# ThomasZiegler/RS-aware-differential-SfM

Measured on AMD Instinct MI355X. Metric: Mpixels/sec RS depth+pose solve, 1280x720 pair, higher is better.
Workload: dtype f64

## Files before the change

### include/rsdsfm.h

```cpp
#ifndef RSDSFM_H
#define RSDSFM_H

#include <stddef.h>
#include <stdint.h>

#ifdef __cplusplus
extern "C" {
#endif

#define RSDSFM_OK 0
#define RSDSFM_ERR_INVALID (-1)
#define RSDSFM_ERR_HIP (-2)
#define RSDSFM_ERR_NO_DEVICE (-3)
#define RSDSFM_ERR_NUMERIC (-4)
#define RSDSFM_ERR_PENDING (-5)
#define RSDSFM_ERR_PEER (-6)

#define RSDSFM_DEPTH_CLOSED_FORM 0
#define RSDSFM_DEPTH_CERES_LM 1

#define RSDSFM_K_COMPAT 0
#define RSDSFM_K_FIXED 1

#define RSDSFM_FLOW_COMPAT_RANK 0
// ... 111 lines not shown
int rsdsfm_flatten_dev(rsdsfm_ctx* ctx, const double* d_flow_img, int32_t rows, int32_t cols, double fx, double fy,
                       double cx, double cy, double gamma, double flow_threshold, double* d_q2n, double* d_u2n,
                       double* d_alpha_n, double* d_alpha_k_n, int64_t* n_out);
int rsdsfm_depth_map_dev(rsdsfm_ctx* ctx, double* d_inliers_3m_inout, int64_t m, double v_inout[3], double fx, double fy,
                         double cx, double cy, int32_t rows, int32_t cols, double* d_depth_map_colmajor,
                         int32_t* d_xs_or_null, int32_t* d_ys_or_null, int* flipped);
int rsdsfm_pose_table_dev(rsdsfm_ctx* ctx, const double v[3], const double w[3], double k, double gamma, int32_t rows,
                          double* d_R_rows9, double* d_t_rows3);
typedef struct rsdsfm_frame_params {
    int32_t ransac_trials;
    int32_t use_acceleration_mode;
    int32_t use_refinement;
    int32_t depth_mode;
    int32_t k_sign_mode;
    int32_t flow_index_mode;
    int32_t use_global_shutter_mode;
    int32_t struct_bytes;
    double ransac_tol;
    double flow_threshold;
    uint64_t seed;
} rsdsfm_frame_params;

void rsdsfm_frame_params_init(rsdsfm_frame_params* params);

typedef struct rsdsfm_frame_result {
    int64_t n_points, num_inliers;
    int32_t best_trial, flipped;
    double ransac_w[3], ransac_v[3], ransac_k;
    double w[3], v[3], k;
    rsdsfm_lm_summary refine_summary;
    const double* d_inliers;
    const int64_t* d_inlier_idx;
    const int32_t* d_scanline;
} rsdsfm_frame_result;

int rsdsfm_solve_frame_dev(rsdsfm_ctx* ctx, const double* d_flow_img, int32_t rows, int32_t cols, double fx, double fy,
                           double cx, double cy, double gamma, const rsdsfm_frame_params* params,
                           double* d_depth_map_colmajor, double* d_R_rows9_or_null, double* d_t_rows3_or_null,
                           rsdsfm_frame_result* result);
typedef struct rsdsfm_frame_job {
    const double* d_flow_img;
    int32_t rows, cols;
    double fx, fy, cx, cy, gamma;
    double* d_depth_map_colmajor;
    double* d_R_rows9_or_null;
    double* d_t_rows3_or_null;
    uint64_t seed;
} rsdsfm_frame_job;
int rsdsfm_solve_frames_dev(rsdsfm_ctx* ctx, const rsdsfm_frame_job* jobs, int32_t count, const rsdsfm_frame_params* params,
                            rsdsfm_frame_result* results);
int rsdsfm_set_sequence_lanes(rsdsfm_ctx* ctx, int32_t lanes);
int rsdsfm_set_frame_side_flatten(rsdsfm_ctx* ctx, int mode);
int rsdsfm_set_frame_tail(rsdsfm_ctx* ctx, int mode);
int rsdsfm_ransac_dev(rsdsfm_ctx* ctx, const double* d_q2n, const double* d_u2n, const double* d_alpha_n,
                      const double* d_alpha_k_n, int64_t n, int use_alpha_k, int32_t iterations, double tolerance,
                      const int32_t* samples_9xT_or_null, uint64_t seed, int depth_mode, int k_sign_mode,
                      rsdsfm_ransac_out* out);
int rsdsfm_refine_dev(rsdsfm_ctx* ctx, const double* d_flow2n, int64_t n_flow, int64_t m, const double* d_inliers_3m,
                      const double* d_alpha_m, const double* d_alpha_k_m, const int64_t* d_inlier_idx_or_null,
                      const double v_in[3], const double w_in[3], double k_in, int const_acceleration,
                      int flow_index_mode, double* d_inliers_out_3m, double v_out[3], double w_out[3], double* k_out,
                      rsdsfm_lm_summary* summary_or_null);
int rsdsfm_estimate_inverse_depths_batch_dev(rsdsfm_ctx* const* ctxs, int32_t count, const double* const* d_q2n,
                                             const double* const* d_u2n, const int64_t* n, const double* v_count_x3,
                                             const double* w_count_x3, const double* k_count, const double* const* d_alpha_n,
                                             const double* const* d_alpha_k_n, double* const* d_inv_depth_n);
int rsdsfm_depth_lm_batch_launch_dev(rsdsfm_ctx* const* ctxs, int32_t count, const double* const* d_q2n, const double* const* d_u2n,
                                     const int64_t* n, const double* v_count_x3, const double* w_count_x3, const double* k_count,
                                     const double* const* d_alpha_n, const double* const* d_alpha_k_n, double* const* d_inv_depth_n);
int rsdsfm_depth_lm_launch_dev(rsdsfm_ctx* ctx, const double* d_q2n, const double* d_u2n, int64_t n,
                               const double v[3], const double w[3], double k, const double* d_alpha_n,
                               const double* d_alpha_k_n, double* d_inv_depth_n, int launch_id);
int rsdsfm_depth_lm_sums_row_size(void);
int rsdsfm_depth_lm_reduce_dev(rsdsfm_ctx* ctx, int64_t n_shard, double* d_row_out);
int rsdsfm_depth_lm_decide_rows_dev(rsdsfm_ctx* ctx, const double* d_rows, int32_t nrows, int64_t n_total, int launch_id);
int rsdsfm_depth_lm_state(rsdsfm_ctx* ctx, int32_t* status, int32_t* next_launch, rsdsfm_lm_summary* summary_or_null);
int rsdsfm_depth_finish_dev(rsdsfm_ctx* ctx, const double* d_q2n, const double* d_u2n, int64_t n,
                            const double v[3], const double w[3], double k, const double* d_alpha_n,
                            const double* d_alpha_k_n, double* d_inv_depth_n, rsdsfm_lm_summary* summary_or_null,
                            int32_t* extra_launches);

int rsdsfm_flatten_slab_dev(rsdsfm_ctx* ctx, const double* d_img_slab, int32_t rows, int32_t slab_cols, int32_t col0,
                            double fx, double fy, double cx, double cy, double gamma, double thr, double* d_q2n,
                            double* d_u2n, double* d_alpha_n, double* d_alpha_k_n, int64_t* n_out);
int rsdsfm_sample_indices(int64_t n, int32_t iterations, uint64_t seed, int32_t* samples);
int rsdsfm_minimal9_dev(rsdsfm_ctx* ctx, const double* d_q9, const double* d_u9, const double* d_alpha9,
                        const double* d_alpha_k9, int32_t count, int use_alpha_k, int k_sign_mode, double* d_hyp);
int rsdsfm_minimal9_probe_dev(rsdsfm_ctx* ctx, const double* d_q9, const double* d_u9, const double* d_alpha9, const double* d_alpha_k9,
                              int32_t count, int use_alpha_k, int k_sign_mode, int use_cores, double* d_hyp, double* d_probe4);
size_t rsdsfm_tile_lm_state_bytes(void);
size_t rsdsfm_tile_best_bytes(void);
int32_t rsdsfm_tile_ransac_row_size(void);
int32_t rsdsfm_tile_ransac_batch(void);
int rsdsfm_tile_ransac_lm_rows_dev(rsdsfm_ctx* ctx, const double* d_q2n, const double* d_u2n, const double* d_alpha_n,
                                   const double* d_alpha_k_n, int64_t n_shard, const double* d_hyp, int32_t count,
                                   const void* d_states, int32_t round, double tolerance, double* d_rows);
int rsdsfm_tile_ransac_decide_dev(rsdsfm_ctx* ctx, const double* d_rows_all, int32_t nranks, int32_t count, void* d_states,
                                  int64_t n_total, int32_t round, int32_t* d_flags, int32_t* d_scored, double* d_trial_count,
                                  double* d_trial_err);
int rsdsfm_tile_ransac_score_rows_dev(rsdsfm_ctx* ctx, const double* d_q2n, const double* d_u2n, const double* d_alpha_n,
                                      const double* d_alpha_k_n, int64_t n_shard, const double* d_hyp, int32_t count,
                                      const void* d_states, int depth_mode, double tolerance, const int32_t* d_scored_or_null,
                                      double* d_rows);
int rsdsfm_tile_ransac_score_merge_dev(rsdsfm_ctx* ctx, const double* d_rows_all, int32_t nranks, int32_t count,
                                       const int32_t* d_scored_or_null, double* d_trial_count, double* d_trial_err);
int rsdsfm_tile_ransac_pick_dev(rsdsfm_ctx* ctx, const double* d_trial_count, const double* d_trial_err, int32_t iterations,
// ... 105 lines not shown
```

### rs-aware-differential-sfm_amd/__init__.py

```python
import ctypes as C
import os
import sys

import numpy as np

from . import dist, pipeline, synth

_HERE = os.path.dirname(os.path.abspath(__file__))
LIB_PATH = os.environ.get("RSDSFM_LIB") or os.path.join(_HERE, "librsdsfm_hip.so")
LIB_PATH_FUSED = os.path.join(_HERE, "librsdsfm_hip_fused.so")
HEADER_PATH = os.path.join(os.path.dirname(_HERE), "include", "rsdsfm.h")

OK = 0
ERR_PENDING = -5
DEPTH_CLOSED_FORM, DEPTH_CERES_LM = 0, 1
K_COMPAT, K_FIXED = 0, 1
FLOW_COMPAT_RANK, FLOW_GATHERED = 0, 1
REFINE_TRACE_COLS = 8
TRACE_REJECTED, TRACE_ACCEPTED, TRACE_INVALID, TRACE_PARAMETER_TOL, TRACE_FUNCTION_TOL, TRACE_ACCEPTED_GRADIENT_TOL = 0.0, 1.0, 2.0, 3.0, 4.0, 5.0
TERMINATION = {0: "gradient", 1: "parameter", 2: "function", 3: "max_iter", 4: "failure", 5: "min_radius"}

_libs = {}


# ... 442 lines not shown
                          int(flow_index_mode), int(use_global_shutter_mode), 0, float(tol), float(flow_threshold), int(seed))
        res, info = FrameResult(), TiledInfo()
        d = C.c_double
        self._check(self.lib.rsdsfm_solve_frame_tiled_dev(self._ctx, _dp(d_img_slab) if d_img_slab else None, C.c_int32(rows), C.c_int32(cols), d(K[0]), d(K[1]),
                                                          d(K[2]), d(K[3]), d(gamma), C.byref(prm), _dp(d_depth_map), _dp(d_R) if d_R else None,
                                                          _dp(d_t) if d_t else None, C.byref(res), C.byref(info)), "rsdsfm_solve_frame_tiled_dev")
        return dict(n=int(res.n_points), num_inliers=int(res.num_inliers), best_trial=int(res.best_trial), flipped=bool(res.flipped),
                    ransac_w=np.array(res.ransac_w[:]), ransac_v=np.array(res.ransac_v[:]), ransac_k=float(res.ransac_k),
                    w=np.array(res.w[:]), v=np.array(res.v[:]), k=float(res.k), refine_summary=res.refine_summary.as_dict(),
                    d_inliers=res.d_inliers, d_inlier_idx=res.d_inlier_idx, d_scanline=res.d_scanline, flow_index_mode=int(flow_index_mode),
                    info={k2: int(getattr(info, k2)) for k2, _ in TiledInfo._fields_ if k2 != "_pad"})

    def estimate_inverse_depths_tiled_dev(self, d_q_shard, d_u_shard, n_total, v, w, k, d_alpha_shard, d_alpha_k_shard, d_inv_depth,
                                          mode=DEPTH_CERES_LM):
        sm, info = LmSummary(), TiledInfo()
        opt = lambda p_: _dp(p_) if p_ else None
        self._check(self.lib.rsdsfm_estimate_inverse_depths_tiled_dev(self._ctx, opt(d_q_shard), opt(d_u_shard), C.c_int64(n_total), _v3(v), _v3(w),
                                                                      C.c_double(k), opt(d_alpha_shard), opt(d_alpha_k_shard), C.c_int(int(mode)),
                                                                      opt(d_inv_depth), C.byref(sm), C.byref(info)),
                    "rsdsfm_estimate_inverse_depths_tiled_dev")
        return (sm.as_dict() if int(mode) == DEPTH_CERES_LM else None,
                {k2: int(getattr(info, k2)) for k2, _ in TiledInfo._fields_ if k2 != "_pad"})

    def prepared_frame_solve(self, d_flow_img, rows, cols, K, gamma, d_depth_map, d_R=None, d_t=None, trials=50, tol=0.05,
                             use_acceleration_mode=False, use_refinement=True, depth_mode=DEPTH_CERES_LM, k_sign_mode=K_COMPAT,
                             flow_threshold=1e-10, flow_index_mode=FLOW_COMPAT_RANK, use_global_shutter_mode=False):
        prm = FrameParams(int(trials), int(use_acceleration_mode), int(use_refinement), int(depth_mode), int(k_sign_mode),
                          int(flow_index_mode), int(use_global_shutter_mode), 0, float(tol), float(flow_threshold), 0)
        res = FrameResult()
        d = C.c_double
        fn = self.lib.rsdsfm_solve_frame_dev
        args = (self._ctx, _dp(d_flow_img), C.c_int32(rows), C.c_int32(cols), d(K[0]), d(K[1]), d(K[2]), d(K[3]), d(gamma), C.byref(prm),
                _dp(d_depth_map), _dp(d_R) if d_R else None, _dp(d_t) if d_t else None, C.byref(res))
        check = self._check

        def call(seed):
            prm.seed = seed
            rc = fn(*args)
            if rc != OK:
                check(rc, "rsdsfm_solve_frame_dev")
            return res

        return call

    def set_sequence_lanes(self, lanes):
        self._check(self.lib.rsdsfm_set_sequence_lanes(self._ctx, C.c_int32(int(lanes))), "rsdsfm_set_sequence_lanes")

    def set_frame_side_flatten(self, on):
        self._check(self.lib.rsdsfm_set_frame_side_flatten(self._ctx, int(on)), "rsdsfm_set_frame_side_flatten")

    def set_frame_tail(self, mode):
        self._check(self.lib.rsdsfm_set_frame_tail(self._ctx, int(mode)), "rsdsfm_set_frame_tail")

    def prepared_frames_solve(self, jobs, trials=50, tol=0.05, use_acceleration_mode=False, use_refinement=True, depth_mode=DEPTH_CERES_LM,
                              k_sign_mode=K_COMPAT, flow_threshold=1e-10, flow_index_mode=FLOW_COMPAT_RANK, use_global_shutter_mode=False):
        n = len(jobs)
        arr = (FrameJob * n)()
        for a, j in zip(arr, jobs):
            K = j["K"]
            a.d_flow_img, a.rows, a.cols = int(j["d_flow_img"]), int(j["rows"]), int(j["cols"])
            a.fx, a.fy, a.cx, a.cy, a.gamma = float(K[0]), float(K[1]), float(K[2]), float(K[3]), float(j["gamma"])
            a.d_depth_map, a.d_R, a.d_t = int(j["d_depth_map"]), int(j.get("d_R") or 0) or None, int(j.get("d_t") or 0) or None
        prm = FrameParams(int(trials), int(use_acceleration_mode), int(use_refinement), int(depth_mode), int(k_sign_mode),
                          int(flow_index_mode), int(use_global_shutter_mode), 0, float(tol), float(flow_threshold), 0)
        res = (FrameResult * n)()
        fn, ctx, check = self.lib.rsdsfm_solve_frames_dev, self._ctx, self._check

        def call(seeds):
            for a, sd in zip(arr, seeds):
                a.seed = int(sd)
            rc = fn(ctx, arr, C.c_int32(n), C.byref(prm), res)
            if rc != OK:
                check(rc, "rsdsfm_solve_frames_dev")
            return res

        return call

    def solve_frames_dev(self, jobs, seeds, **kw):
        res = self.prepared_frames_solve(jobs, **kw)(seeds)
        return [dict(n=int(r.n_points), num_inliers=int(r.num_inliers), best_trial=int(r.best_trial), flipped=bool(r.flipped),
                     ransac_w=np.array(r.ransac_w[:]), ransac_v=np.array(r.ransac_v[:]), ransac_k=float(r.ransac_k),
                     w=np.array(r.w[:]), v=np.array(r.v[:]), k=float(r.k), refine_summary=r.refine_summary.as_dict(),
                     d_inliers=r.d_inliers, d_inlier_idx=r.d_inlier_idx, d_scanline=r.d_scanline) for r in res]

    def depth_lm_reduce_dev(self, n_shard, d_row):
        self._check(self.lib.rsdsfm_depth_lm_reduce_dev(self._ctx, C.c_int64(n_shard), _dp(d_row)), "rsdsfm_depth_lm_reduce_dev")

    def depth_lm_decide_rows_dev(self, d_rows, nrows, n_total, launch_id):
        self._check(self.lib.rsdsfm_depth_lm_decide_rows_dev(self._ctx, _dp(d_rows), C.c_int32(nrows), C.c_int64(n_total), int(launch_id)), "rsdsfm_depth_lm_decide_rows_dev")

    def depth_lm_state(self):
        status, nxt, sm = C.c_int32(), C.c_int32(), LmSummary()
        self._check(self.lib.rsdsfm_depth_lm_state(self._ctx, C.byref(status), C.byref(nxt), C.byref(sm)), "rsdsfm_depth_lm_state")
        return status.value, nxt.value, sm.as_dict()

    def depth_finish_dev(self, d_q, d_u, n, v, w, k, d_alpha, d_alpha_k, d_rho):
        sm = LmSummary()
        extra = C.c_int32()
        self._check(self.lib.rsdsfm_depth_finish_dev(self._ctx, _dp(d_q), _dp(d_u), C.c_int64(n), _v3(v), _v3(w), C.c_double(k), _dp(d_alpha), _dp(d_alpha_k), _dp(d_rho), C.byref(sm), C.byref(extra)), "rsdsfm_depth_finish_dev")
        return sm.as_dict(), extra.value


def _np0(ptr):
    return _dp(ptr) if ptr else None


# ... 386 lines not shown
```

### rs-aware-differential-sfm_amd/build.py

```python
import concurrent.futures
import glob
import os
import subprocess

HERE = os.path.dirname(os.path.abspath(__file__))
SO = os.path.join(HERE, "librsdsfm_hip.so")
SO_FUSED = os.path.join(HERE, "librsdsfm_hip_fused.so")
OBJ_DIR = os.path.join(HERE, "build")
CFLAGS = ["--offload-arch=gfx950", "-O3", "-std=c++17", "-ffp-contract=off", "-fPIC", "-Wall", "-Wno-unused-function"]
LDFLAGS = ["--offload-arch=gfx950", "-shared", "-fPIC", "-ldl"]
FUSED_UNITS = ("depth_kernels", "ransac_kernels", "ransac_lma_kernels", "depth_lma_kernels", "gtflow_kernels", "capi")


def sources():
    return sorted(glob.glob(os.path.join(HERE, "csrc", "*.hip")))


def _deps():
    return glob.glob(os.path.join(HERE, "csrc", "*.hpp")) + [os.path.join(HERE, "..", "include", "rsdsfm.h")]


def _stale(target, deps):
    return not os.path.exists(target) or os.path.getmtime(target) < max(os.path.getmtime(d) for d in deps)


def needs_build():
    return _stale(SO, sources() + _deps()) or _stale(SO_FUSED, sources() + _deps())


def _compile(job):
    src, obj, extra, verbose = job
    hipcc = os.environ.get("HIPCC", "/opt/rocm/bin/hipcc")
    cmd = [hipcc] + CFLAGS + extra + ["-c", src, "-o", obj]
    if verbose:
        print(" ".join(cmd), flush=True)
    subprocess.check_call(cmd)
    return obj


def build(force=False, verbose=False, jobs=None):
    if not force and not needs_build():
        return SO
    os.makedirs(OBJ_DIR, exist_ok=True)
    hdrs = _deps()
    todo, objs, objs_fused = [], [], []
    for src in sources():
        stem = os.path.splitext(os.path.basename(src))[0]
        obj = os.path.join(OBJ_DIR, stem + ".o")
        objs.append(obj)
        if force or _stale(obj, [src] + hdrs):
            todo.append((src, obj, [], verbose))
        if stem in FUSED_UNITS:
            objf = os.path.join(OBJ_DIR, stem + ".fused.o")
            objs_fused.append(objf)
            if force or _stale(objf, [src] + hdrs):
                todo.append((src, objf, ["-DRSDSFM_FUSED=1"], verbose))
        else:
            objs_fused.append(obj)
    jobs = jobs or max(1, min(len(todo), (os.cpu_count() or 4)))
    if todo:
        with concurrent.futures.ThreadPoolExecutor(max_workers=jobs) as ex:
            list(ex.map(_compile, todo))
    hipcc = os.environ.get("HIPCC", "/opt/rocm/bin/hipcc")
    for so, oo in ((SO, objs), (SO_FUSED, objs_fused)):
# ... 14 lines not shown
```

### rs-aware-differential-sfm_amd/csrc/frame_host.hip

```cpp
#include <stdlib.h>
#include <string.h>

#include <atomic>

#include <algorithm>
#include <new>

#include "rsdsfm_internal.hpp"

namespace rsdsfm {

static std::atomic<int> g_frames_in_flight[64];
int frames_in_flight(const Ctx* c) { return g_frames_in_flight[c->device & 63].load(std::memory_order_relaxed); }

int alpha_ones_launch(Ctx* c, double* d_alpha, int64_t n);
int flatten_device(Ctx* c, const double* d_img, int32_t rows, int32_t cols, int32_t col0, double fx, double fy, double cx, double cy, double gamma,
                   double thr, double* d_q, double* d_u, double* d_alpha, double* d_alpha_k, int64_t* n_out);

struct FrameRun {
    rsdsfm_frame_job job;
    rsdsfm_frame_params prm;
    size_t N = 0;
    int64_t n = 0;
    double *d_q = nullptr, *d_u = nullptr, *d_a = nullptr, *d_ak = nullptr, *d_in_a = nullptr, *d_in_ak = nullptr, *d_inl = nullptr, *d_inl_ref = nullptr;
    int64_t* d_idx = nullptr;
    uint8_t* d_mask = nullptr;
    int32_t* d_ys = nullptr;
    double *d_zpartials = nullptr, *d_zheader = nullptr;
    char* d_refine_ws = nullptr;
    rsdsfm_ransac_out ro;
    RansacRun ransac;
    RefineRun refine;
    Minimal9Direct direct;
    DenseFlatten dense;
    bool refinement_enqueued = false, ahead = false, side_flatten = false, dense_in_launch = false, open = false;
    bool counted = false;
    int rc_begin = RSDSFM_OK;
    int64_t m_known = -1;
    RefineTail tail;
    FinishClaim claim;
    RansacSpecTail spec_tail;
    std::function<int()> join;
};

namespace {

inline double* header_host(Ctx* c) { return reinterpret_cast<double*>(static_cast<char*>(c->h_pinned) + c->pinned_bytes - 64); }
inline RefineState* state_host(Ctx* c) { return reinterpret_cast<RefineState*>(static_cast<char*>(c->h_pinned) + c->pinned_bytes - kPinnedTail); }
inline int64_t* count_host(Ctx* c) { return reinterpret_cast<int64_t*>(static_cast<char*>(c->h_pinned) + c->pinned_bytes - kPinnedTail / 2); }
static_assert(sizeof(RefineState) + sizeof(int) <= kPinnedTail / 2, "reserved tail: state read-back | point count ... depth-map header");

struct StreamSwap {
    Ctx* c;
    hipStream_t main;
    StreamSwap(Ctx* ctx, hipStream_t other) : c(ctx), main(ctx->stream) { c->stream = other; }
    ~StreamSwap() { c->stream = main; }
};

int ensure_side_stream(Ctx* c) {
    if (c->aux_stream) return RSDSFM_OK;
    RSDSFM_HIP_CHECK(c, hipStreamCreateWithFlags(&c->aux_stream, hipStreamNonBlocking));
    RSDSFM_HIP_CHECK(c, hipEventCreateWithFlags(&c->ev_fork, hipEventDisableTiming));
    RSDSFM_HIP_CHECK(c, hipEventCreateWithFlags(&c->ev_join, hipEventDisableTiming));
    return RSDSFM_OK;
}

static void frame_uncount(const Ctx* c, FrameRun* F) {
    if (F && F->counted) {
        F->counted = false;
        g_frames_in_flight[c->device & 63].fetch_sub(1, std::memory_order_relaxed);
    }
}
struct FrameInFlightEnd {
    const Ctx* c;
    FrameRun* F;
    ~FrameInFlightEnd() { frame_uncount(c, F); }
};

int frame_begin(Ctx* c, FrameRun* F) {
    const rsdsfm_frame_job& J = F->job;
    const rsdsfm_frame_params* prm = &F->prm;
    frame_uncount(c, F);
    F->open = false;
    F->rc_begin = RSDSFM_OK;
    if (J.rows <= 0 || J.cols <= 0 || !J.d_flow_img || !J.d_depth_map_colmajor) return fail(c, RSDSFM_ERR_INVALID, "bad arguments");
    if (prm->flow_index_mode != RSDSFM_FLOW_COMPAT_RANK && prm->flow_index_mode != RSDSFM_FLOW_GATHERED) return fail(c, RSDSFM_ERR_INVALID, "unknown flow_index_mode");
    if (prm->struct_bytes != 0 && prm->struct_bytes != (int32_t)sizeof(rsdsfm_frame_params))
        return fail(c, RSDSFM_ERR_INVALID, "rsdsfm_frame_params: struct_bytes is neither 0 nor sizeof(rsdsfm_frame_params) -- caller built against another header (use rsdsfm_frame_params_init)");
// ... 74 lines not shown
                StreamSwap on_side(c, c->aux_stream);
                rc = flatten_launch(c, J.d_flow_img, rows, cols, 0, fx, fy, cx, cy, gamma, prm->flow_threshold, F->d_q, F->d_u, F->d_a, F->d_ak,
                                    d_flat_counts, d_flat_offsets, count_host(c), nullptr);
                if (rc == RSDSFM_OK && prm->use_global_shutter_mode) rc = alpha_ones_launch(c, F->d_a, n);
            }
            if (rc != RSDSFM_OK) return rc;
            RSDSFM_HIP_CHECK(c, hipEventRecord(c->ev_join, c->aux_stream));
            F->join = [c]() -> int {
                RSDSFM_HIP_CHECK(c, hipStreamWaitEvent(c->stream, c->ev_join, 0));
                return RSDSFM_OK;
            };
        } else {
            rc = flatten_enqueue(c, J.d_flow_img, rows, cols, fx, fy, cx, cy, gamma, prm->flow_threshold, F->d_q, F->d_u, F->d_a, F->d_ak, count_host(c));
            if (rc != RSDSFM_OK) return rc;
        }
    } else {
        rc = flatten_device(c, J.d_flow_img, rows, cols, 0, fx, fy, cx, cy, gamma, prm->flow_threshold, F->d_q, F->d_u, F->d_a, F->d_ak, &n);
        if (rc != RSDSFM_OK) return rc;
        *count_host(c) = n;
    }
    if (prm->use_global_shutter_mode && !F->side_flatten) {
        rc = alpha_ones_launch(c, F->d_a, n);
        if (rc != RSDSFM_OK) return rc;
    }
    F->n = n;
    memset(&F->ro, 0, sizeof(F->ro));
    F->ro.inlier_idx = F->d_idx;
    F->ro.inliers = F->d_inl;
    F->ro.alpha = F->d_in_a;
    F->ro.alpha_k = F->d_in_ak;
    F->ro.mask = F->d_mask;
    F->m_known = -1;
    F->tail = [c, F](const RefineBuffers& B) -> int {
        const rsdsfm_frame_job& J2 = F->job;
        const RefineState* st = B.state;
        const int64_t m_arg = F->m_known >= 0 ? F->m_known : F->n;
        const int64_t* m_dev = F->m_known >= 0 ? nullptr : &st->m;
        PoseTableOut pt;
        if (J2.d_R_rows9_or_null && J2.d_t_rows3_or_null)
            pt.R = J2.d_R_rows9_or_null, pt.t = J2.d_t_rows3_or_null, pt.rows = J2.rows, pt.gamma = J2.gamma, pt.wk_dev = st->p + 3;
        if (B.claim.on)
            return depth_map_decided_launch(c, F->d_inl_ref, m_arg, F->d_zpartials, refine_finish_grid(c, B), B, J2.d_depth_map_colmajor, F->d_zheader,
                                            header_host(c), st->p, m_dev, &pt);
        return depth_map_slab_launch(c, F->d_inl_ref, m_arg, F->d_zpartials, refine_finish_grid(c, B), m_arg, nullptr, J2.fx, J2.fy, J2.cx, J2.cy, J2.rows,
                                     0, J2.cols, J2.d_depth_map_colmajor, nullptr, F->d_ys, F->d_zheader, header_host(c), st->p, m_dev, &pt);
    };
    F->claim = FinishClaim();
    if (c->frame_tail == 0) {
        F->claim.on = true;
        F->claim.fx = J.fx, F->claim.fy = J.fy, F->claim.cx = J.cx, F->claim.cy = J.cy;
        F->claim.rows = rows, F->claim.cols = cols;
        F->claim.ys = F->d_ys;
    }
    F->spec_tail = [c, F](const RansacBest* d_best) -> int {
        return refine_begin(c, F->d_u, F->n, F->n, F->d_inl, F->d_in_a, F->d_in_ak, F->d_idx, nullptr, nullptr, 0.0, F->prm.use_acceleration_mode,
                            F->prm.flow_index_mode, F->d_inl_ref, &F->tail, d_best, F->d_refine_ws, &F->refine, state_host(c), F->d_zpartials, false,
                            &F->claim);
    };
    F->refinement_enqueued = false;
    F->ahead = prm->use_refinement && c->ransac_spec_miss < 2;
    F->open = true;
    g_frames_in_flight[c->device & 63].fetch_add(1, std::memory_order_relaxed);
    F->counted = true;
    F->rc_begin = ransac_begin(c, F->d_q, F->d_u, F->d_a, F->d_ak, n, prm->use_acceleration_mode, prm->ransac_trials, prm->ransac_tol, nullptr, J.seed,
                               prm->depth_mode, prm->k_sign_mode, &F->ro, prm->use_refinement ? &F->spec_tail : nullptr, &F->refinement_enqueued, &F->ransac,
                               F->side_flatten ? &F->direct : nullptr, F->side_flatten && !F->dense_in_launch ? &F->join : nullptr,
                               F->dense_in_launch ? &F->dense : nullptr, F->ahead, true,
                               F->claim.on && prm->use_refinement ? refine_flag_words(F->d_refine_ws) : nullptr);
    return RSDSFM_OK;
}

int frame_finish(Ctx* c, FrameRun* F, rsdsfm_frame_result* res) {
    if (!F->open) return fail(c, RSDSFM_ERR_INVALID, "no frame solve in flight");
    F->open = false;
    FrameInFlightEnd in_flight_end_{c, F};
    const rsdsfm_frame_job& J = F->job;
    const rsdsfm_frame_params* prm = &F->prm;
    memset(res, 0, sizeof(*res));
    int rc = F->rc_begin;
    if (rc == RSDSFM_OK) rc = ransac_finish(c, &F->ransac);
    if (rc != RSDSFM_OK) RSDSFM_HIP_CHECK(c, hipStreamSynchronize(c->stream));
    if (F->side_flatten && c->aux_stream) RSDSFM_HIP_CHECK(c, hipStreamSynchronize(c->aux_stream));
    int64_t n = F->n;
    if (*count_host(c) < 0) {
        c->frame_dense_hint = 1;
        return rc != RSDSFM_OK ? rc : fail(c, RSDSFM_ERR_NUMERIC, "frame solve: the point count did not arrive");
    }
    bool counted = true;
    if (*count_host(c) != n) {
        if (F->dense_in_launch) {
            int64_t n_real = 0;
            rc = flatten_device(c, J.d_flow_img, J.rows, J.cols, 0, J.fx, J.fy, J.cx, J.cy, J.gamma, prm->flow_threshold, F->d_q, F->d_u, F->d_a, F->d_ak, &n_real);
            if (rc == RSDSFM_OK && prm->use_global_shutter_mode) rc = alpha_ones_launch(c, F->d_a, n_real);
            if (rc != RSDSFM_OK) return rc;
            *count_host(c) = n_real;
        }
        n = *count_host(c);
        F->n = n;
        F->refinement_enqueued = false;
        counted = false;
        rc = ransac_begin(c, F->d_q, F->d_u, F->d_a, F->d_ak, n, prm->use_acceleration_mode, prm->ransac_trials, prm->ransac_tol, nullptr, J.seed,
                          prm->depth_mode, prm->k_sign_mode, &F->ro, prm->use_refinement ? &F->spec_tail : nullptr, &F->refinement_enqueued, &F->ransac, nullptr, nullptr,
                          nullptr, F->ahead, true,
                               F->claim.on && prm->use_refinement ? refine_flag_words(F->d_refine_ws) : nullptr);
        if (rc == RSDSFM_OK) rc = ransac_finish(c, &F->ransac);
        counted = rc == RSDSFM_OK;
    }
    c->frame_dense_hint = n == (int64_t)F->N ? 1 : 0;
    if (rc != RSDSFM_OK) return rc;
    if (counted) ransac_commit_hints(c, F->ransac);
    const rsdsfm_ransac_out& ro = F->ro;
    res->n_points = n;
    res->num_inliers = ro.num_inliers;
    res->best_trial = ro.best_trial;
    memcpy(res->ransac_w, ro.w, sizeof(ro.w));
    memcpy(res->ransac_v, ro.v, sizeof(ro.v));
    res->ransac_k = ro.k;
    double v[3], w[3], k = ro.k;
    for (int i = 0; i < 3; ++i) v[i] = ro.v[i], w[i] = ro.w[i];
    double* d_final = F->d_inl;
    int flipped = 0;
    F->m_known = ro.num_inliers;
    if (prm->use_refinement) {
        bool exact = false;
        if (F->refinement_enqueued) {
            rc = refine_poll(c, &F->refine, v, w, &k, &res->refine_summary);
            exact = rc == kRcRefineRestartExact;
        }
        if (!F->refinement_enqueued || exact)
            rc = refine_device(c, F->d_u, n, ro.num_inliers, F->d_inl, F->d_in_a, F->d_in_ak, F->d_idx, v, w, k, prm->use_acceleration_mode,
                               prm->flow_index_mode, F->d_inl_ref, v, w, &k, &res->refine_summary, &F->tail, F->d_zpartials, exact, &F->claim);
        if (rc != RSDSFM_OK) return rc;
        d_final = F->d_inl_ref;
        const double* h_header = header_host(c);
        flipped = h_header[0] != 0.0;
        v[0] = h_header[1], v[1] = h_header[2], v[2] = h_header[3];
    } else {
        rc = depth_map_device(c, d_final, ro.num_inliers, v, J.fx, J.fy, J.cx, J.cy, J.rows, J.cols, J.d_depth_map_colmajor, nullptr, F->d_ys, &flipped, w,
                              k, J.gamma, J.d_R_rows9_or_null, J.d_t_rows3_or_null);
        if (rc != RSDSFM_OK) return rc;
    }
    res->flipped = flipped;
    memcpy(res->v, v, sizeof(v));
    memcpy(res->w, w, sizeof(w));
    res->k = k;
    res->d_inliers = d_final;
    res->d_inlier_idx = F->d_idx;
    res->d_scanline = F->d_ys;
    return RSDSFM_OK;
}

FrameRun* frame_run_of(Ctx* c) {
    if (!c->frame_run) c->frame_run = new (std::nothrow) FrameRun();
    return static_cast<FrameRun*>(c->frame_run);
}

}

void frame_release(Ctx* c) {
    frame_uncount(c, static_cast<FrameRun*>(c->frame_run));
    delete static_cast<FrameRun*>(c->frame_run);
    c->frame_run = nullptr;
    for (rsdsfm_ctx* lane : c->lanes) rsdsfm_destroy(lane);
    c->lanes.clear();
    if (c->ev_fork) (void)hipEventDestroy(c->ev_fork);
    if (c->ev_join) (void)hipEventDestroy(c->ev_join);
    if (c->ev_seq) (void)hipEventDestroy(c->ev_seq);
    if (c->aux_stream) (void)hipStreamDestroy(c->aux_stream);
    if (c->d_flat_counters) (void)hipFree(c->d_flat_counters);
    c->d_flat_counters = nullptr;
    c->ev_fork = c->ev_join = c->ev_seq = nullptr;
    c->aux_stream = nullptr;
}

}

using namespace rsdsfm;

extern "C" {

void rsdsfm_frame_params_init(rsdsfm_frame_params* p) {
    if (!p) return;
    memset(p, 0, sizeof(*p));
    p->ransac_trials = 5;
    p->use_acceleration_mode = 0;
    p->use_refinement = 1;
    p->depth_mode = RSDSFM_DEPTH_CERES_LM;
    p->k_sign_mode = RSDSFM_K_COMPAT;
    p->flow_index_mode = RSDSFM_FLOW_COMPAT_RANK;
    p->use_global_shutter_mode = 0;
    p->struct_bytes = (int32_t)sizeof(rsdsfm_frame_params);
    p->ransac_tol = 0.05;
    p->flow_threshold = 1e-10;
    p->seed = 1;
}

int rsdsfm_solve_frame_dev(rsdsfm_ctx* ctx, const double* d_flow_img, int32_t rows, int32_t cols, double fx, double fy, double cx,
                           double cy, double gamma, const rsdsfm_frame_params* prm, double* d_depth_map, double* d_R_rows9,
                           double* d_t_rows3, rsdsfm_frame_result* res) {
    if (!ctx) return RSDSFM_ERR_INVALID;
    Ctx* c = &ctx->c;
    DeviceGuard device_guard_(c);
    if (!prm || !res) return fail(c, RSDSFM_ERR_INVALID, "bad arguments");
    FrameRun* F = frame_run_of(c);
    if (!F) return fail(c, RSDSFM_ERR_INVALID, "out of host memory");
    F->prm = *prm;
    F->job = rsdsfm_frame_job{d_flow_img, rows, cols, fx, fy, cx, cy, gamma, d_depth_map, d_R_rows9, d_t_rows3, prm->seed};
    int rc = frame_begin(c, F);
    if (rc != RSDSFM_OK) return rc;
    return frame_finish(c, F, res);
}

int rsdsfm_set_sequence_lanes(rsdsfm_ctx* ctx, int32_t lanes) {
    if (!ctx) return RSDSFM_ERR_INVALID;
    Ctx* c = &ctx->c;
    DeviceGuard device_guard_(c);
    if (lanes < 0 || lanes > 16) return fail(c, RSDSFM_ERR_INVALID, "lanes must be 0 (default) .. 16");
    c->seq_lanes = lanes;
    return RSDSFM_OK;
}

int rsdsfm_set_frame_tail(rsdsfm_ctx* ctx, int mode) {
    if (!ctx) return RSDSFM_ERR_INVALID;
    if (mode < 0 || mode > 1) return fail(&ctx->c, RSDSFM_ERR_INVALID, "mode must be 0 (short launch tail) or 1 (stage-by-stage launches)");
    ctx->c.frame_tail = mode;
    return RSDSFM_OK;
}

int rsdsfm_set_frame_side_flatten(rsdsfm_ctx* ctx, int mode) {
    if (!ctx) return RSDSFM_ERR_INVALID;
    if (mode < 0 || mode > 3) return fail(&ctx->c, RSDSFM_ERR_INVALID, "mode must be 0 (flatten first), 1 (flatten on a second stream), 2 (flatten behind the minimal solver) or 3 (flatten inside the solver's launch)");
    ctx->c.frame_side_flatten = mode;
    return RSDSFM_OK;
}

int rsdsfm_solve_frames_dev(rsdsfm_ctx* ctx, const rsdsfm_frame_job* jobs, int32_t count, const rsdsfm_frame_params* prm, rsdsfm_frame_result* results) {
    if (!ctx) return RSDSFM_ERR_INVALID;
    Ctx* c = &ctx->c;
    DeviceGuard device_guard_(c);
    if (count < 0 || !prm || (count > 0 && (!jobs || !results))) return fail(c, RSDSFM_ERR_INVALID, "bad arguments");
    if (count == 0) return RSDSFM_OK;
    const int L = std::max(1, std::min<int>(count, c->seq_lanes > 0 ? c->seq_lanes : kSequenceLanesDefault));
    while ((int)c->lanes.size() < L - 1) {
        rsdsfm_ctx* lane = nullptr;
        int rc = rsdsfm_create(&lane, c->device, nullptr);
        if (rc != RSDSFM_OK) return fail(c, rc, "could not create a sequence lane");
        c->lanes.push_back(lane);
    }
    auto lane_ctx = [&](int l) -> Ctx* { return l == 0 ? c : &c->lanes[(size_t)l - 1]->c; };
    if (L > 1) {
        if (!c->ev_seq) RSDSFM_HIP_CHECK(c, hipEventCreateWithFlags(&c->ev_seq, hipEventDisableTiming));
        RSDSFM_HIP_CHECK(c, hipEventRecord(c->ev_seq, c->stream));
    }
    for (int l = 1; l < L; ++l) {
        Ctx* lc = lane_ctx(l);
        RSDSFM_HIP_CHECK(c, hipStreamWaitEvent(lc->stream, c->ev_seq, 0));
        lc->ransac_k0 = c->ransac_k0;
        lc->ransac_math_mode = c->ransac_math_mode;
        lc->lm_arithmetic = c->lm_arithmetic;
        lc->refine_arithmetic = c->refine_arithmetic;
        lc->lma_count_only_force = c->lma_count_only_force;
        lc->frame_side_flatten = c->frame_side_flatten;
        lc->frame_tail = c->frame_tail;
        lc->refine_stage_mode = c->refine_stage_mode;
    }
    for (int l = 0; l < L; ++l) lane_ctx(l)->refine_stage_separate = L > 1;
    int first_error = RSDSFM_OK;
    int in_flight[16];
    for (int l = 0; l < 16; ++l) in_flight[l] = -1;
    auto finish_lane = [&](int l) {
        const int i = in_flight[l];
        if (i < 0) return;
        in_flight[l] = -1;
        Ctx* lc = lane_ctx(l);
        int rc = frame_finish(lc, static_cast<FrameRun*>(lc->frame_run), &results[i]);
        if (rc != RSDSFM_OK && first_error == RSDSFM_OK) {
            first_error = rc;
            if (lc != c) c->err = "pair " + std::to_string(i) + ": " + lc->err;
        }
    };
    for (int i = 0; i < count && first_error == RSDSFM_OK; ++i) {
        const int l = i % L;
        finish_lane(l);
        if (first_error != RSDSFM_OK) break;
        Ctx* lc = lane_ctx(l);
        FrameRun* F = frame_run_of(lc);
        if (!F) {
            first_error = fail(c, RSDSFM_ERR_INVALID, "out of host memory");
            break;
        }
        F->prm = *prm;
        F->job = jobs[i];
        int rc = frame_begin(lc, F);
        if (rc != RSDSFM_OK) {
            first_error = rc;
            if (lc != c) c->err = "pair " + std::to_string(i) + ": " + lc->err;
            break;
        }
        in_flight[l] = i;
    }
    for (;;) {
        int best = -1;
        for (int l = 0; l < L; ++l)
            if (in_flight[l] >= 0 && (best < 0 || in_flight[l] < in_flight[best])) best = l;
        if (best < 0) break;
        finish_lane(best);
    }
    for (int l = 0; l < L; ++l) lane_ctx(l)->refine_stage_separate = false;
    return first_error;
}

int rsdsfm_set_refine_stage(rsdsfm_ctx* ctx, int mode) {
    if (!ctx) return RSDSFM_ERR_INVALID;
    Ctx* c = &ctx->c;
    if (mode < 0 || mode > 2) return fail(c, RSDSFM_ERR_INVALID, "refine stage: 0 (automatic), 1 (in the next pass's prologue) or 2 (a launch of its own)");
    c->refine_stage_mode = mode;
// ... 5 lines not shown
```

### rs-aware-differential-sfm_amd/csrc/lm_common.hpp

```cpp
#pragma once

#include "device_math.hpp"
#include "rsdsfm_internal.hpp"

namespace rsdsfm {

__device__ __forceinline__ double closed_form_rho(double x, double y, double ux, double uy, double al, double ak,
                                                  const Pose& pose, double two_over) {
    PixelModel m;
    m.init(x, y, ux, uy, al, ak, pose, two_over);
    double r0, r1;
    m.residual(1.0, r0, r1);
    double h = m.J0 * m.J0 + m.J1 * m.J1;
    double g = m.J0 * r0 + m.J1 * r1;
    return (h > 0.0) ? 1.0 - g / h : 1.0;
}


__device__ __forceinline__ void lm_advance(LmScal& st, double* hist, const double* sums, int64_t n, int first, int used_K,
                                           int used_write, int launch_id) {
    if (first) {
        st.status = 0;
        st.restart = 0;
        st.n_hist = 0;
// ... 61 lines not shown
        if (rel > kMinRelDecrease) {
            hist[st.n_hist] = st.radius;
            st.n_hist += 1;
            accepted_in_batch = j + 1;
            cost = ccost;
            x_norm = sqrt(s[3]);
            st.radius = radius_accept(st.radius, rel);
            st.decrease_factor = 2.0;
            st.num_successful += 1;
            if (s[4] <= kGradientTol) {
                st.termination = RSDSFM_TERM_GRADIENT;
                break;
            }
        } else {
            st.num_unsuccessful += 1;
            st.radius = st.radius / st.decrease_factor;
            st.decrease_factor *= 2.0;
            break;
        }
    }
    st.cost = cost;
    if (used_write <= accepted_in_batch) st.rho_holds = base_hist + used_write;
    else st.rho_holds = -1;
    if (st.termination < 0 && st.iteration >= kMaxIter) st.termination = RSDSFM_TERM_MAX_ITER;
    if (st.termination < 0 && st.radius <= kMinRadius) st.termination = RSDSFM_TERM_MIN_RADIUS;
    st.next_launch = launch_id + 1;
    if (st.termination >= 0) {
        st.predict = st.n_hist < KMAX ? st.n_hist : KMAX;
        if (st.rho_holds == st.n_hist) {
            st.status = 1;
        } else {
            st.status = 2;
            st.K = 0;
            st.write_which = 0;
        }
    } else {
        st.status = 0;
        st.K = KMAX;
        st.write_which = 0;
        double r = st.radius;
#pragma unroll
        for (int j = 0; j < KMAX; ++j) {
            st.cand[j] = r;
            r = radius_accept(r, 1.0);
        }
    }
}

struct LmPlanLds {
    int n_hist, K, write_which;
    double inv_hist[kMaxIter];
    double inv_cand[KMAX];
    __device__ __forceinline__ double inv_hist_at(int h) const { return inv_hist[h]; }
};

struct LmPlanReg {
    int n_hist, K, write_which;
    double inv_cand[KMAX];
    double h0, h1, h2, h3;
    const double* hist_lds;
    __device__ __forceinline__ double inv_hist_at(int h) const {
        return h == 0 ? h0 : (h == 1 ? h1 : (h == 2 ? h2 : (h == 3 ? h3 : hist_lds[h])));
    }
};

template <int K0>
struct LmPlanFirstK {
    static constexpr int n_hist = 0;
    static constexpr int K = K0;
    int write_which;
    double inv_cand[KMAX];
    __device__ __forceinline__ double inv_hist_at(int) const { return 0.0; }
    __device__ __forceinline__ void load(const LmPlanLds& l) {
        write_which = l.write_which;
#pragma unroll
        for (int j = 0; j < KMAX; ++j) inv_cand[j] = l.inv_cand[j];
    }
};
using LmPlanFirst = LmPlanFirstK<KMAX>;

template <int NH>
struct LmPlanReplay {
    static constexpr int n_hist = NH;
    static constexpr int K = 0;
    static constexpr int write_which = 0;
    double ih[NH > 0 ? NH : 1];
    double inv_cand[KMAX];
    __device__ __forceinline__ double inv_hist_at(int h) const { return ih[h]; }
};

__device__ __forceinline__ double lm_denominator(double ht, double diag, double inv_radius) {
#if RSDSFM_FUSED
    return __builtin_fma(diag, inv_radius, ht);
#else
    const double lam = diag * inv_radius;
    return ht + lam;
#endif
}

struct NoHook {
    __device__ __forceinline__ void operator()(int, double, const PixelModel&) const {}
};

template <bool CORE, class Plan, class Hook = NoHook>
__device__ __forceinline__ double lm_pixel_t(double x, double y, double ux, double uy, double al, double ak,
                                             const Pose& pose, double two_over, const Plan& plan,
// ... 9 lines not shown
        s = 1.0 / (1.0 + sqrt(dot2(m.J0, m.J0, m.J1, m.J1)));
    }
    const double jt0 = m.J0 * s, jt1 = m.J1 * s;
    const double ht = dot2(jt0, jt0, jt1, jt1);
    const double diag = clampd(ht, kMinLmDiag, kMaxLmDiag);
    double rho = 1.0;
    double r0, r1;
    m.residual(rho, r0, r1);
    for (int h = 0; h < plan.n_hist; ++h) {
        const double gt = dot2(jt0, r0, jt1, r1);
        const double step = -(gt / lm_denominator(ht, diag, plan.inv_hist_at(h)));
        rho = mad(step, s, rho);
        m.residual(rho, r0, r1);
    }
    double out = rho;
    if (plan.K > 0) {
        acc[0] = acc_sq2(acc[0], r0, r1);
        acc[1] = acc_sq(acc[1], rho);
        acc[2] = fmax(acc[2], fabs(dot2(m.J0, r0, m.J1, r1)));
    }
#pragma unroll
    for (int j = 0; j < KMAX; ++j) {
        if (j < plan.K) {
            const double gt = dot2(jt0, r0, jt1, r1);
            const double step = -(gt / lm_denominator(ht, diag, plan.inv_cand[j]));
            const double m0 = jt0 * step, m1 = jt1 * step;
#if RSDSFM_FUSED
            acc[3 + 5 * j + 1] = __builtin_fma(-m0, __builtin_fma(m0, 0.5, r0), __builtin_fma(-m1, __builtin_fma(m1, 0.5, r1), acc[3 + 5 * j + 1]));
#else
            acc[3 + 5 * j + 1] -= m0 * (r0 + m0 / 2.0) + m1 * (r1 + m1 / 2.0);
#endif
            const double cand = mad(step, s, rho);
            const double dx = rho - cand;
            acc[3 + 5 * j + 2] = acc_sq(acc[3 + 5 * j + 2], dx);
            m.residual(cand, r0, r1);
            acc[3 + 5 * j + 0] = acc_sq2(acc[3 + 5 * j + 0], r0, r1);
            acc[3 + 5 * j + 3] = acc_sq(acc[3 + 5 * j + 3], cand);
            acc[3 + 5 * j + 4] = fmax(acc[3 + 5 * j + 4], fabs(dot2(m.J0, r0, m.J1, r1)));
            rho = cand;
            hook(j, cand, m);
            if (plan.write_which == j + 1) out = cand;
        }
    }
    return out;
}

template <class Plan, class Hook = NoHook>
__device__ __forceinline__ double lm_pixel(double x, double y, double ux, double uy, double al, double ak,
                                           const Pose& pose, double two_over, const Plan& plan,
                                           double (&acc)[NS], const Hook& hook = Hook(), PixelModel* model_out = nullptr) {
    return lm_pixel_t<false>(x, y, ux, uy, al, ak, pose, two_over, plan, acc, hook, model_out);
}

__device__ __forceinline__ bool is_max_slot(int s) { return s == 2 || (s >= 3 && ((s - 3) % 5) == 4); }


}
```

### rs-aware-differential-sfm_amd/csrc/ransac_host.hip

```cpp
#include <stdio.h>
#include <stdlib.h>
#include <string.h>

#include <algorithm>
#include <vector>

#include "rsdsfm_internal.hpp"

namespace rsdsfm {

namespace {


inline uint64_t splitmix64(uint64_t& state) {
    uint64_t z = (state += 0x9E3779B97F4A7C15ULL);
    z = (z ^ (z >> 30)) * 0xBF58476D1CE4E5B9ULL;
    z = (z ^ (z >> 27)) * 0x94D049BB133111EBULL;
    return z ^ (z >> 31);
}

void sample_indices(int64_t n, int T, uint64_t seed, std::vector<int32_t>& out) {
    struct Slot {
        int64_t key;
        int32_t val;
// ... 105 lines not shown
                    }
                }
                R.b0 = 0;
                R.pc = kPcBatchBegin;
                break;
            }
            case kPcBatchBegin: {
                if (R.b0 >= T) {
                    R.pc = kPcFinal;
                    break;
                }
                R.B = std::min(batch, T - R.b0);
                R.need_score = true;
                if (depth_mode == RSDSFM_DEPTH_CERES_LM) {
                    if (R.b0 > 0)
                        RSDSFM_HIP_CHECK(c, hipMemsetAsync(R.d_flags, 0, (size_t)(reinterpret_cast<char*>(R.d_irr_count + R.batch) - reinterpret_cast<char*>(R.d_flags)), c->stream));
                    R.round = 0;
                    R.pc = kPcRoundEnqueue;
                } else {
                    R.pc = kPcScore;
                }
                break;
            }
            case kPcRoundEnqueue: {
                const int b0 = R.b0, B = R.B, round = R.round;
                bool flags_via_pick = false;
                if (round > 4 * kMaxIter) return fail(c, RSDSFM_ERR_NUMERIC, "LM state machines did not terminate");
                if (R.analytic && round == 0) {
                    rc = ransac_lma_launch(c, R.d_q, R.d_u, R.d_a, R.d_ak, n, R.d_hyp + (size_t)b0 * 8, B, R.d_states + b0, R.d_partials, R.d_flags,
                                           R.d_scored + b0, R.d_tcount + b0, R.d_terr + b0, tol, R.lma_cand, 2, R.d_irr_count, R.d_irr_list, R.d_unscored,
                                           nullptr, R.core_epoch ? c->d_core_flag : nullptr, R.core_epoch, R.count_only);
                } else {
                    rc = ransac_lm_round_launch(c, R.d_q, R.d_u, R.d_a, R.d_ak, n, R.d_hyp + (size_t)b0 * 8, B, R.d_states + b0, R.d_partials, R.d_flags,
                                                R.d_scored + b0, R.d_tcount + b0, R.d_terr + b0, round, tol, R.k0, R.fused_base, R.core_math,
                                                R.core_epoch ? c->d_core_flag : nullptr, R.core_epoch, R.d_unscored);
                }
                if (rc != RSDSFM_OK) return rc;
                if (round == 0 && B == T) {
                    const PickLazy lazy = R.count_only ? PickLazy{R.d_scored, R.d_unscored, R.d_flags + 1} : PickLazy();
                    if (c->ransac_score_idle < kScoreIdleLimit) {
                        if (R.count_only) {
                            rc = ransac_pick_launch(c, R.d_tcount, R.d_terr, T, R.d_hyp, R.d_best, nullptr, R.d_flags, nullptr, 0, nullptr, 0, 0, nullptr, 0.0, lazy);
                            if (rc != RSDSFM_OK) return rc;
                        }
                        rc = ransac_score_launch(c, R.d_q, R.d_u, R.d_a, R.d_ak, n, R.d_hyp, T, R.d_states, depth_mode, tol, R.d_scored, R.d_partials,
                                                 R.d_tcount, R.d_terr, R.d_unscored, R.d_flags + 1);
                        if (rc != RSDSFM_OK) return rc;
                        R.spec_scored = true;
                    }
                    rc = ransac_pick_launch(c, R.d_tcount, R.d_terr, T, R.d_hyp, R.d_best, R.h_best, R.d_flags, R.h_running, R.spec_scored ? 1 : 0,
                                            nullptr, 0, 0, nullptr, R.tie_margin, lazy);
                    if (rc != RSDSFM_OK) return rc;
                    flags_via_pick = true;
                    rc = ransac_final_launch(c, R.d_q, R.d_u, R.d_a, R.d_ak, n, R.d_best, R.d_states, depth_mode, tol, R.d_rho, R.d_mask, R.d_bcounts,
                                             R.d_boffs, out->inlier_idx, out->inliers, out->alpha, out->alpha_k, R.h_best, R.refine_flag_words);
                    if (rc != RSDSFM_OK) return rc;
                    R.final_done = true;
                    R.spec_final = true;
                    if (R.spec_tail && R.tail_ahead) {
                        rc = (*R.spec_tail)(R.d_best);
                        if (rc != RSDSFM_OK) return rc;
                        R.tail_enqueued = true;
                    }
                }
                if (!flags_via_pick) RSDSFM_HIP_CHECK(c, hipMemcpyAsync(R.h_running, R.d_flags, sizeof(int) * 8, hipMemcpyDeviceToHost, c->stream));
                R.pc = kPcRoundWait;
                if (yield_at_wait) return RSDSFM_OK;
                break;
            }
            case kPcRoundWait: {
                yield_at_wait = false;
                if (int rcs = sync_stream(c, "ransac_finish line 244")) return rcs;
                const int* h_running = R.h_running;
                if (R.round == 0 && R.analytic && (h_running[3] & 16) != 0) R.lma_guard |= h_running[3] >> 8;
                if (R.round == 0 && R.analytic && (h_running[3] & 6) != 0 && !((h_running[3] & 1) && R.core_math)) {
                    rc = lma_start_over(c, R, (h_running[3] >> 8) | ((h_running[3] & 4) ? (1 << 7) : 0));
                    if (rc != RSDSFM_OK) return rc;
                    break;
                }
                if (R.round == 0 && R.core_math && (h_running[3] & 1) != 0) {
                    R.core_math = false;
                    R.restarted = true;
                    R.not_one_step = 0;
                    R.final_done = R.spec_scored = R.tail_enqueued = R.spec_final = false;
                    R.dense = nullptr;
                    R.after_minimal9 = nullptr;
                    R.pc = kPcStart;
                    break;
                }
                if (R.round == 0) {
                    R.not_one_step += h_running[2];
                    if (R.b0 == 0) {
                        int best = 0;
                        for (int a2 = 1; a2 <= 3; ++a2)
                            if (h_running[4 + a2] > (best ? h_running[4 + best] : 0)) best = a2;
                        if (best) R.fused_base_next = best;
                        int second = 0;
                        for (int a2 = 1; a2 <= 3; ++a2)
                            if (a2 != best && h_running[4 + a2] > (second ? h_running[4 + second] : 0)) second = a2;
                        if (best) {
                            R.lma_cand_next[0] = best;
                            R.lma_cand_next[1] = second ? second : (best > 1 ? best - 1 : 2);
                        }
                    }
                }
                if (h_running[0] == 0) {
                    R.pc = kPcAfterRounds;
                } else {
                    R.final_done = false;
                    R.round += 1;
                    R.pc = kPcRoundEnqueue;
                }
                break;
            }
            case kPcAfterRounds: {
                R.need_score = R.h_running[1] > 0;
                if (R.B == T) R.score_hint_next = R.need_score ? 1 : 0;
                if (R.need_score && R.final_done && R.spec_scored && !R.h_best->lazy_pending) R.need_score = false;
                if (R.need_score) R.final_done = false;
                R.pc = kPcScore;
                break;
            }
            case kPcScore: {
                if (R.need_score) {
                    rc = ransac_score_launch(c, R.d_q, R.d_u, R.d_a, R.d_ak, n, R.d_hyp + (size_t)R.b0 * 8, R.B, R.d_states + R.b0, depth_mode, tol,
                                             depth_mode == RSDSFM_DEPTH_CERES_LM ? R.d_scored + R.b0 : nullptr, R.d_partials, R.d_tcount + R.b0,
                                             R.d_terr + R.b0, depth_mode == RSDSFM_DEPTH_CERES_LM ? R.d_unscored : nullptr, R.d_flags + 1);
                    if (rc != RSDSFM_OK) return rc;
                }
                R.b0 += batch;
                R.pc = kPcBatchBegin;
                break;
            }
            case kPcFinal: {
                if (!R.final_done) {
                    R.tail_enqueued = false;
                    R.spec_final = false;
                    rc = ransac_pick_launch(c, R.d_tcount, R.d_terr, T, R.d_hyp, R.d_best, R.h_best, nullptr, nullptr, 0, nullptr, 0, 0, nullptr, R.tie_margin,
                                            R.count_only ? PickLazy{R.d_scored, R.d_unscored, R.d_flags + 1} : PickLazy());
                    if (rc != RSDSFM_OK) return rc;
                    rc = ransac_final_launch(c, R.d_q, R.d_u, R.d_a, R.d_ak, n, R.d_best, R.d_states, depth_mode, tol, R.d_rho, R.d_mask, R.d_bcounts,
                                             R.d_boffs, out->inlier_idx, out->inliers, out->alpha, out->alpha_k, R.h_best, R.refine_flag_words);
                    if (rc != RSDSFM_OK) return rc;
                }
                if (R.spec_tail && !R.tail_enqueued) {
                    rc = (*R.spec_tail)(R.d_best);
                    if (rc != RSDSFM_OK) return rc;
                    R.tail_enqueued = true;
                }
                if (T > 0 && out->trial_count) RSDSFM_HIP_CHECK(c, hipMemcpyAsync(R.h_tcount, R.d_tcount, sizeof(double) * T, hipMemcpyDeviceToHost, c->stream));
                if (T > 0 && out->trial_err) RSDSFM_HIP_CHECK(c, hipMemcpyAsync(R.h_terr, R.d_terr, sizeof(double) * T, hipMemcpyDeviceToHost, c->stream));
                if (T > 0 && out->trial_vel) RSDSFM_HIP_CHECK(c, hipMemcpyAsync(R.h_hyp, R.d_hyp, sizeof(double) * 8 * T, hipMemcpyDeviceToHost, c->stream));
                if (T > 0 && out->trial_steps && depth_mode == RSDSFM_DEPTH_CERES_LM)
                    RSDSFM_HIP_CHECK(c, hipMemcpyAsync(R.h_states, R.d_states, sizeof(LmState) * T, hipMemcpyDeviceToHost, c->stream));
                R.pc = kPcFinalWait;
                if (yield_at_wait) return RSDSFM_OK;
                break;
            }
            case kPcFinalWait: {
                if (int rcs = sync_stream(c, "ransac_finish line 345")) return rcs;
                const RansacBest* h_best = R.h_best;
#ifdef RSDSFM_DEBUG_HOOKS
                if (getenv("RSDSFM_RANSAC_DEBUG")) fprintf(stderr, "[ransac] final wait: lazy_pending %d undecided %d flags %d %d %d %d hist %d %d %d %d spec_scored %d spec_final %d tail %d idle %d\n", h_best->lazy_pending, h_best->undecided, R.h_running[0], R.h_running[1], R.h_running[2], R.h_running[3], R.h_running[4], R.h_running[5], R.h_running[6], R.h_running[7], (int)R.spec_scored, (int)R.spec_final, (int)R.tail_enqueued, c->ransac_score_idle);
#endif
                if (R.count_only && h_best->lazy_pending) {
                    if (++R.lazy_rounds > T + 2) return fail(c, RSDSFM_ERR_NUMERIC, "lazy error sums did not settle");
                    R.final_done = R.tail_enqueued = R.spec_final = false;
                    R.need_score = true;
                    R.score_hint_next = 1;
                    R.b0 = 0;
                    R.B = T;
                    R.pc = kPcScore;
                    break;
                }
                if (R.analytic && h_best->lma_tie) {
                    rc = lma_start_over(c, R, 1 << 7);
                    if (rc != RSDSFM_OK) return rc;
                    break;
                }
                R.lma_tie_seen = h_best->lma_tie != 0;
                R.shared_best = h_best->shared_best;
                if (h_best->num_inliers != h_best->num_inliers_scan) {
                    if (R.analytic) {
                        rc = lma_start_over(c, R, 1 << 10);
                        if (rc != RSDSFM_OK) return rc;
                        break;
                    }
                    return fail(c, RSDSFM_ERR_NUMERIC, "inlier count mismatch between scoring and compaction");
                }
                out->num_inliers = h_best->num_inliers;
                out->best_trial = h_best->best_trial;
                memcpy(out->w, &h_best->hyp[0], 3 * sizeof(double));
                memcpy(out->v, &h_best->hyp[3], 3 * sizeof(double));
                out->k = h_best->hyp[6];
                out->inlier_error = h_best->inlier_error;
                for (int t = 0; t < T; ++t) {
                    if (out->trial_count) out->trial_count[t] = (int64_t)R.h_tcount[t];
                    if (out->trial_err) out->trial_err[t] = R.h_terr[t];
                    if (out->trial_vel) memcpy(out->trial_vel + (size_t)7 * t, R.h_hyp + (size_t)8 * t, 7 * sizeof(double));
                    if (out->trial_steps) out->trial_steps[t] = depth_mode == RSDSFM_DEPTH_CERES_LM ? R.h_states[t].num_successful : 1;
                }
                if (R.spec_tail_held) *R.spec_tail_held = R.tail_enqueued;
                R.hints_ready = true;
                R.pc = kPcDone;
                (void)Tn;
                return RSDSFM_OK;
            }
            default:
                return RSDSFM_OK;
        }
    }
}

}

void ransac_commit_hints(Ctx* c, const RansacRun& R) {
    if (!R.hints_ready || R.depth_mode != RSDSFM_DEPTH_CERES_LM || R.T <= 0) return;
    if (R.fused_base_next) c->ransac_fused_base = R.fused_base_next;
    if (R.score_hint_next >= 0) c->ransac_score_idle = R.score_hint_next ? 0 : std::min(c->ransac_score_idle + 1, kScoreIdleLimit);
    c->ransac_not_one_step = R.not_one_step;
    c->ransac_spec_miss = R.spec_final ? 0 : std::min(c->ransac_spec_miss + 1, 2);
    if (R.count_only) c->lma_count_only_runs += 1, c->lma_lazy_runs += (R.lazy_rounds > 0 || R.shared_best > 1) ? 1 : 0;
    if (R.lazy_rounds > 0 || R.shared_best > 1) c->lma_unique_run = 0;
    else if (R.shared_best == 1) c->lma_unique_run = std::min(c->lma_unique_run + 1, 2);
    if (R.lma_guard) c->lma_last_guard = R.lma_guard, c->lma_handed_over += 1;
    if (R.lma_restarted) {
        c->lma_hold = 16;
        c->lma_restarts += 1;
        c->lma_last_guard = R.lma_guard;
    } else if (c->lma_hold > 0 && !R.analytic) {
        c->lma_hold = R.lma_tie_seen ? 16 : c->lma_hold - 1;
    }
    if (R.restarted) {
        c->ransac_standard_math = 16;
        c->ransac_restarts += 1;
    } else if (c->ransac_standard_math > 0) {
        c->ransac_standard_math -= 1;
    }
}

int ransac_begin(Ctx* c, const double* d_q, const double* d_u, const double* d_a, const double* d_ak, int64_t n, int use_alpha_k, int T,
                 double tol, const int32_t* h_samples, uint64_t seed, int depth_mode, int k_sign_mode, rsdsfm_ransac_out* out,
                 const RansacSpecTail* spec_tail, bool* spec_tail_held, RansacRun* run, const Minimal9Direct* direct,
                 const std::function<int()>* after_minimal9, const DenseFlatten* dense, bool tail_ahead, bool count_only, int* refine_flag_words) {
    RansacRun& R = *run;
    R = RansacRun();
    R.tail_ahead = tail_ahead;
    R.core_math = c->ransac_math_mode == 0 && c->ransac_standard_math == 0;
    R.analytic = depth_mode == RSDSFM_DEPTH_CERES_LM && T > 0 && c->lm_arithmetic == 0 && c->lma_hold == 0;
    R.tie_margin = depth_mode != RSDSFM_DEPTH_CERES_LM || c->lm_arithmetic != 0 ? 0.0 : (R.analytic ? kLmaTie : -kLmaTie);
    R.lma_cand[0] = c->lma_cand[0], R.lma_cand[1] = c->lma_cand[1];
    R.count_only = count_only && R.analytic && T <= kRansacBatch && (c->lma_unique_run >= 2 || c->lma_count_only_force);
    if (R.count_only) R.tie_margin = 0.0;
    R.refine_flag_words = refine_flag_words;
    if (spec_tail_held) *spec_tail_held = false;
    if (!out) return fail(c, RSDSFM_ERR_INVALID, "null out");
    if (n < 9) return fail(c, RSDSFM_ERR_INVALID, "ransac needs at least 9 points (the reference would compute rand() % 0)");
    if (T < 0) return fail(c, RSDSFM_ERR_INVALID, "negative iterations");
    if (depth_mode != RSDSFM_DEPTH_CLOSED_FORM && depth_mode != RSDSFM_DEPTH_CERES_LM) return fail(c, RSDSFM_ERR_INVALID, "unknown depth_mode");
    if (n > (int64_t)INT32_MAX) return fail(c, RSDSFM_ERR_INVALID, "n exceeds the int32 sample index range");
    if (T > 0) {
        if (h_samples) {
            R.samples.assign(h_samples, h_samples + (size_t)T * 9);
            for (int32_t s : R.samples)
                if (s < 0 || s >= n) return fail(c, RSDSFM_ERR_INVALID, "sample index out of range");
        } else {
            sample_indices(n, T, seed, R.samples);
        }
    }
    const int Tn = std::max(T, 1);
    const int batch = std::min(Tn, kRansacBatch);
    const size_t partials_doubles = std::max<size_t>((size_t)ransac_lm_partials_doubles(c, n, batch), (size_t)ransac_lma_partials_doubles(c, n, batch));
    size_t need = Arena::need(sizeof(double) * Tn * 8) + Arena::need(sizeof(int) * batch) + Arena::need(sizeof(int) * ransac_lma_list_ints(batch)) +
                  Arena::need(sizeof(LmState) * Tn) + Arena::need(sizeof(double) * partials_doubles) +
                  Arena::need(sizeof(int) * 8) + 2 * Arena::need(sizeof(int) * Tn) + 2 * Arena::need(sizeof(double) * Tn) + Arena::need(sizeof(RansacBest)) +
                  2 * Arena::need(sizeof(int64_t) * 2048) + Arena::need(sizeof(double) * (size_t)n) + Arena::need((size_t)n) + 4096;
    int rc = ensure_ws(c, need);
    if (rc != RSDSFM_OK) return rc;
    Arena ws(c->d_ws);
    R.d_hyp = ws.take<double>((size_t)Tn * 8);
    R.zero_begin = ws.base + ws.off;
    R.d_states = ws.take<LmState>(Tn);
    R.d_scored = ws.take<int>(Tn);
    R.d_flags = ws.take<int>(8);
    R.d_irr_count = ws.take<int>(batch);
    R.zero_bytes = (size_t)((ws.base + ws.off) - R.zero_begin);
    R.d_irr_list = ws.take<int>(ransac_lma_list_ints(batch));
    R.d_unscored = ws.take<int>(batch);
    R.d_partials = ws.take<double>(partials_doubles);
    R.d_tcount = ws.take<double>(Tn);
    R.d_terr = ws.take<double>(Tn);
    R.d_best = ws.take<RansacBest>(1);
    R.d_bcounts = ws.take<int64_t>(2048);
    R.d_boffs = ws.take<int64_t>(2048);
    R.d_rho = out->inv_depth ? out->inv_depth : ws.take<double>((size_t)n);
    R.d_mask = out->mask ? out->mask : ws.take<uint8_t>((size_t)n);

    rc = ensure_pinned(c, ransac_pinned_bytes(T));
    if (rc != RSDSFM_OK) return rc;
    if (!c->d_core_flag) {
        RSDSFM_HIP_CHECK(c, hipMalloc(reinterpret_cast<void**>(&c->d_core_flag), 64));
        RSDSFM_HIP_CHECK(c, hipMemsetAsync(c->d_core_flag, 0, 64, c->stream));
    }
    char* hp = static_cast<char*>(c->h_pinned);
    R.h_best = reinterpret_cast<RansacBest*>(hp);
    R.h_running = reinterpret_cast<int*>(hp + sizeof(RansacBest));
    R.h_tcount = reinterpret_cast<double*>(hp + sizeof(RansacBest) + 32);
    R.h_terr = R.h_tcount + Tn;
    R.h_hyp = R.h_terr + Tn;
    R.h_states = reinterpret_cast<LmState*>(R.h_hyp + (size_t)8 * Tn);
    R.h_samples_pinned = reinterpret_cast<int32_t*>(R.h_states + Tn);

    R.d_q = d_q, R.d_u = d_u, R.d_a = d_a, R.d_ak = d_ak;
    R.n = n, R.T = T, R.Tn = Tn, R.batch = batch, R.tol = tol, R.depth_mode = depth_mode, R.use_alpha_k = use_alpha_k, R.k_sign_mode = k_sign_mode;
    R.out = out, R.spec_tail = spec_tail, R.spec_tail_held = spec_tail_held;
    R.direct = direct, R.after_minimal9 = after_minimal9, R.dense = dense;
    R.k0 = c->ransac_k0 != 0 ? c->ransac_k0 : (c->ransac_not_one_step == 0 ? 2 : (int)KMAX);
    R.fused_base = R.k0 == 2 ? 1 : std::min(std::max(c->ransac_fused_base, 1), (int)KMAX);
    R.pc = kPcStart;
    return ransac_advance(c, R, true);
}

int ransac_finish(Ctx* c, RansacRun* run) { return ransac_advance(c, *run, false); }

int ransac_device(Ctx* c, const double* d_q, const double* d_u, const double* d_a, const double* d_ak, int64_t n,
                  int use_alpha_k, int T, double tol, const int32_t* h_samples, uint64_t seed, int depth_mode,
                  int k_sign_mode, rsdsfm_ransac_out* out, const RansacSpecTail* spec_tail, bool* spec_tail_held) {
    RansacRun run;
    int rc = ransac_begin(c, d_q, d_u, d_a, d_ak, n, use_alpha_k, T, tol, h_samples, seed, depth_mode, k_sign_mode, out, spec_tail, spec_tail_held,
                          &run, nullptr, nullptr);
    if (rc == RSDSFM_OK) rc = ransac_finish(c, &run);
    if (rc == RSDSFM_OK) ransac_commit_hints(c, run);
    return rc;
}

}

using namespace rsdsfm;

extern "C" {

int rsdsfm_calculate_velocities(rsdsfm_ctx* ctx, const double* q, const double* u, const double* alpha, const double* alpha_k,
                                int32_t count, int use_alpha_k, int k_sign_mode, double* w, double* v, double* k) {
    if (!ctx) return RSDSFM_ERR_INVALID;
    Ctx* c = &ctx->c;
    DeviceGuard device_guard_(c);
    if (count < 0 || (count > 0 && (!q || !u || !alpha || !alpha_k || !w || !v || !k))) return fail(c, RSDSFM_ERR_INVALID, "bad arguments");
    if (count == 0) return RSDSFM_OK;
    const size_t T = (size_t)count;
    int rc = ensure_stage(c, 2 * Arena::need(144 * T) + 2 * Arena::need(72 * T) + Arena::need(64 * T));
    if (rc != RSDSFM_OK) return rc;
    Arena sa(c->d_stage);
    double* d_q = sa.take<double>(18 * T);
    double* d_u = sa.take<double>(18 * T);
    double* d_a = sa.take<double>(9 * T);
    double* d_ak = sa.take<double>(9 * T);
    double* d_h = sa.take<double>(8 * T);
    RSDSFM_HIP_CHECK(c, hipMemcpyAsync(d_q, q, 144 * T, hipMemcpyHostToDevice, c->stream));
    RSDSFM_HIP_CHECK(c, hipMemcpyAsync(d_u, u, 144 * T, hipMemcpyHostToDevice, c->stream));
    RSDSFM_HIP_CHECK(c, hipMemcpyAsync(d_a, alpha, 72 * T, hipMemcpyHostToDevice, c->stream));
    RSDSFM_HIP_CHECK(c, hipMemcpyAsync(d_ak, alpha_k, 72 * T, hipMemcpyHostToDevice, c->stream));
    rc = minimal9_launch(c, d_q, d_u, d_a, d_ak, nullptr, count, use_alpha_k, k_sign_mode, d_h);
    if (rc != RSDSFM_OK) return rc;
    std::vector<double> h(8 * T);
    RSDSFM_HIP_CHECK(c, hipMemcpyAsync(h.data(), d_h, 64 * T, hipMemcpyDeviceToHost, c->stream));
    RSDSFM_HIP_CHECK(c, hipStreamSynchronize(c->stream));
    int worst = 0;
    for (size_t t = 0; t < T; ++t) {
        memcpy(w + 3 * t, &h[8 * t], 3 * sizeof(double));
        memcpy(v + 3 * t, &h[8 * t + 3], 3 * sizeof(double));
        k[t] = h[8 * t + 6];
        if (h[8 * t + 7] != 0.0) worst = (int)h[8 * t + 7];
    }
    if (worst != 0) return fail(c, RSDSFM_ERR_NUMERIC, worst == -1 ? "no real eigenvalue k for at least one hypothesis" : "singular system in the k estimation");
    return RSDSFM_OK;
}
// ... 79 lines not shown
```

### rs-aware-differential-sfm_amd/csrc/ransac_kernels.hip

```cpp
#include <algorithm>

#include "device_math.hpp"
#include "lm_common.hpp"
#include "rsdsfm_internal.hpp"

namespace rsdsfm {

namespace {

constexpr int kRB = 256;
constexpr int kRP = RSDSFM_FUSED ? 5 : 6;
constexpr int kFused = 1;
constexpr int kTiledFusedBase = 2;
constexpr int NSR = NS + 2 * kFused;
constexpr int kNSum = NSR - (KMAX + 1);
constexpr int kTStride = 65;

template <int K0>
struct R0Shape {
    static constexpr int NSk = 3 + 5 * K0;
    static constexpr int F = kFused;
    static constexpr int nsum = NSk - (K0 + 1) + 2 * F;
};
static_assert(R0Shape<KMAX>::nsum == kNSum, "full shape uses every sum slot");
// ... 287 lines not shown
    if (core_flags && t == 0 && threadIdx.x < 2) rows[(int64_t)T * NSR + threadIdx.x] = (threadIdx.x == 0 && core_flags[3] != 0) ? 1.0 : 0.0;
    const LmState* state = states + t;
    if (round > 0 && (state->status != 0 || state->next_launch != round)) {
        if (threadIdx.x < NSR) rows[(int64_t)t * NSR + threadIdx.x] = 0.0;
        return;
    }
    reduce_hyp_sums(partials, nblocks, T, t, true, s_red, s_sums);
    if (threadIdx.x < NSR) rows[(int64_t)t * NSR + threadIdx.x] = s_sums[threadIdx.x];
}

__global__ __launch_bounds__(256) void ransac_decide_kernel(const double* __restrict__ partials, int nblocks, int T, int hyp_major,
                                                           LmState* states, int64_t n, int round, int k0, int* flags, int* pred_flag,
                                                           int* __restrict__ scored, double* __restrict__ trial_count,
                                                           double* __restrict__ trial_err, int fused_base, int* steps_hist,
                                                           int* __restrict__ unscored_list, int rank_stride2 = 0,
                                                           double* __restrict__ cnt_rt = nullptr, int cnt_stride = 0) {
    __shared__ double s_red[4][NSR];
    __shared__ double s_sums[NSR];
    __shared__ int s_fused_score;
    const int t = blockIdx.x;
    const int tid = threadIdx.x;
    LmState* state = states + t;
    if (tid == 0) s_fused_score = 0;
    if (rank_stride2 && t == 0 && tid < nblocks) {
        if (partials[(int64_t)tid * rank_stride2 * 2 + (int64_t)T * NSR] != 0.0) flags[3] = 1;
    }
    if (round > 0 && (state->status != 0 || state->next_launch != round)) return;
    reduce_hyp_sums(partials, nblocks, T, t, hyp_major != 0, s_red, s_sums, rank_stride2);
    if (tid == 0) {
        LmScal st = *static_cast<const LmScal*>(state);
        const bool first = round == 0 || st.launches == 0;
        const int used_K = (round == 0) ? k0 : st.K;
        lm_advance(st, state->hist, s_sums, n, first, used_K, 0, round);
        if (pred_flag && round == 0 && (st.status == 0 || st.n_hist >= 2)) atomicAdd(pred_flag, 1);
        if (steps_hist && round == 0) atomicAdd(&steps_hist[st.status == 0 ? 3 : (st.n_hist < 1 ? 0 : (st.n_hist > 3 ? 3 : st.n_hist))], 1);
        if (st.status == 0) {
            atomicAdd(&flags[0], 1);
        } else if (round == 0 && st.n_hist == fused_base) {
            trial_count[t] = s_sums[NS];
            trial_err[t] = s_sums[NS + 1];
            scored[t] = 1;
            s_fused_score = 1;
        } else {
            const int pos = atomicAdd(&flags[1], 1);
            if (unscored_list) unscored_list[pos] = t;
        }
        *static_cast<LmScal*>(state) = st;
    }
    if (cnt_rt) {
        __syncthreads();
        if (s_fused_score && tid < nblocks)
            cnt_rt[(int64_t)tid * cnt_stride + t] = partials[((int64_t)tid * (rank_stride2 ? rank_stride2 : T * (NSR / 2)) + (int64_t)t * (NSR / 2)) * 2 + NS];
    }
}

__device__ __forceinline__ double hyp_rho(double x, double y, double ux, double uy, double al, double ak, const Pose& pose,
                                          double two_over, int depth_mode, const LmPlanLds& plan) {
    if (depth_mode == RSDSFM_DEPTH_CLOSED_FORM) return closed_form_rho(x, y, ux, uy, al, ak, pose, two_over);
    double dummy[NS];
    return lm_pixel(x, y, ux, uy, al, ak, pose, two_over, plan, dummy);
}

__device__ __forceinline__ double score_error(const PixelModel& m, double x, double y, double ux, double uy, double al, double ak,
                                              const Pose& pose, double two_over, double rho) {
#if RSDSFM_FUSED
    (void)m;
    return point_error(x, y, ux, uy, al, ak, pose, two_over, rho);
#else
    (void)x, (void)y, (void)ux, (void)uy, (void)al, (void)ak, (void)pose, (void)two_over;
    return point_error_from_model(m, rho);
#endif
}

template <int NH>
__device__ __forceinline__ void score_pixels(const Tile& px, bool full_tile, const Pose& pose, double two_over, const LmState& st, double tol,
                                             double& cnt, double& es) {
    LmPlanReplay<NH> plan;
#pragma unroll
    for (int h = 0; h < NH; ++h) plan.ih[h] = 1.0 / st.hist[h];
    double dummy[NS];
#pragma unroll
    for (int j = 0; j < kRP; ++j) {
        if (full_tile || px.ok[j]) {
            PixelModel m;
            const double rho = lm_pixel(px.x[j], px.y[j], px.ux[j], px.uy[j], px.al[j], px.ak[j], pose, two_over, plan, dummy, NoHook(), &m);
            const double err = score_error(m, px.x[j], px.y[j], px.ux[j], px.uy[j], px.al[j], px.ak[j], pose, two_over, rho);
            if (err < tol) {
                cnt += 1.0;
                es += err;
            }
        }
    }
}

__device__ __forceinline__ void tile_group_of_block(int bid, int ntile_blocks, int ngroups, int& tb, int& grp) {
    const int tiles8 = ((ntile_blocks + 7) / 8) * 8;
    const int nfull = ngroups - 1;
    if (nfull > 0 && bid < tiles8 * nfull) {
        const int window = 8 * nfull;
        tb = (bid / window) * 8 + (bid % 8);
        grp = (bid % window) / 8;
    } else {
        tb = bid - tiles8 * nfull;
        grp = nfull;
    }
}

__global__ __launch_bounds__(kRB) void ransac_score_kernel(const double2* __restrict__ q, const double2* __restrict__ u,
                                                          const double* __restrict__ alpha,
                                                          const double* __restrict__ alpha_k, int64_t n,
                                                          const double* __restrict__ hyp, int T,
                                                          const LmState* __restrict__ states, int depth_mode, double tol,
                                                          const int* __restrict__ scored, double* __restrict__ partials, int ntile_blocks,
// ... 229 lines not shown
            ns += __builtin_popcountll(__builtin_amdgcn_ballot_w64(hit));
            nco += __builtin_popcountll(__builtin_amdgcn_ballot_w64(hit && lazy.scored && lazy.scored[t] == 2));
        }
        if (ns > 1 && nco > 0) {
            int base = 0;
            for (int t0 = 0; t0 < T; t0 += 64) {
                const int t = t0 + lane;
                const bool co = t < T && trial_count[t] == best_count && lazy.scored[t] == 2;
                const unsigned long long mk = __builtin_amdgcn_ballot_w64(co);
                if (co) {
                    lazy.list[base + __builtin_popcountll(mk & ((1ull << lane) - 1ull))] = t;
                    lazy.scored[t] = 0;
                }
                base += __builtin_popcountll(mk);
            }
            if (lane == 0) *lazy.list_count = nco;
            pending = 1;
            list_n = nco;
            undecided = 1;
        }
    }
    if (flags_host && lane < 8) flags_host[lane] = (lane == 1 && pending) ? list_n : (flags[lane] | ((lane == 3 && tie && tie_margin > 0.0) ? 4 : 0));
    if (m_all)
        for (int r = lane; r < nranks; r += 64) m_all[r] = bi >= 0 ? (int64_t)cnt_rt[(int64_t)r * cnt_stride + bi] : 0;
    const double h = (lane < 8 && bi >= 0) ? hyp[(int64_t)bi * 8 + lane] : 0.0;
    if (lane < 8) best->hyp[lane] = h;
    if (lane < 8 && best_host) best_host->hyp[lane] = h;
    if (lane == 0) {
        best->best_trial = bi;
        best->undecided = undecided;
        best->lma_tie = tie;
        best->lazy_pending = pending;
        best->shared_best = ns;
        best->num_inliers = bi >= 0 ? (int64_t)best_count : 0;
        best->inlier_error = best_err;
        if (best_host) {
            best_host->best_trial = bi;
            best_host->undecided = undecided;
            best_host->lma_tie = tie;
            best_host->lazy_pending = pending;
            best_host->shared_best = ns;
            best_host->num_inliers = bi >= 0 ? (int64_t)best_count : 0;
            best_host->inlier_error = best_err;
        }
    }
}

__global__ __launch_bounds__(kRB) void ransac_final_kernel(const double2* __restrict__ q, const double2* __restrict__ u,
                                                          const double* __restrict__ alpha,
                                                          const double* __restrict__ alpha_k, int64_t n, int64_t chunk,
                                                          const RansacBest* __restrict__ best,
                                                          const LmState* __restrict__ states, int depth_mode, double tol,
                                                          double* __restrict__ rho_out, uint8_t* __restrict__ mask_out,
                                                          int64_t* __restrict__ block_counts) {
    __shared__ LmPlanLds plan;
    __shared__ int s_cnt[kRB / 64];
    const int tid = threadIdx.x, lane = tid & 63, wv = tid >> 6;
    if (best->undecided) return;
    const int bt = best->best_trial;
    Pose pose;
    pose.w[0] = best->hyp[0], pose.w[1] = best->hyp[1], pose.w[2] = best->hyp[2];
    pose.v[0] = best->hyp[3], pose.v[1] = best->hyp[4], pose.v[2] = best->hyp[5];
    pose.k = best->hyp[6];
    if (depth_mode == RSDSFM_DEPTH_CERES_LM && bt >= 0) {
        if (tid == 0) {
            plan.n_hist = states[bt].n_hist;
            plan.K = 0;
            plan.write_which = 0;
        }
        if (tid < kMaxIter) plan.inv_hist[tid] = 1.0 / states[bt].hist[tid];
    }
    __syncthreads();
    const double two_over = 2.0 / (2.0 + pose.k);
    const int64_t i0 = (int64_t)blockIdx.x * chunk;
    const int64_t i1 = (i0 + chunk < n) ? i0 + chunk : n;
    int count = 0;
    for (int64_t i = i0 + tid; i < i1; i += kRB) {
        double2 qq = q[i], uu = u[i];
        const double al = alpha[i], ak = alpha_k[i];
        bool in = false;
        double rho = 0.0;
        if (bt >= 0) {
            rho = hyp_rho(qq.x, qq.y, uu.x, uu.y, al, ak, pose, two_over, depth_mode, plan);
            in = point_error(qq.x, qq.y, uu.x, uu.y, al, ak, pose, two_over, rho) < tol;
        }
        rho_out[i] = rho;
        mask_out[i] = in ? 1 : 0;
        count += in ? 1 : 0;
    }
    for (int off = 32; off >= 1; off >>= 1) count += __shfl_xor(count, off, 64);
    if (lane == 0) s_cnt[wv] = count;
    __syncthreads();
    if (tid == 0) {
        int c = 0;
        for (int w2 = 0; w2 < kRB / 64; ++w2) c += s_cnt[w2];
        block_counts[blockIdx.x] = c;
    }
}

__global__ __launch_bounds__(256) void ransac_scan_kernel(const int64_t* __restrict__ block_counts, int nblocks,
                                                         int64_t* __restrict__ block_offsets, RansacBest* best, RansacBest* best_host) {
    __shared__ int64_t s_part[256];
    const int tid = threadIdx.x;
    const int per = (nblocks + 255) / 256;
    int64_t sum = 0;
    for (int j = 0; j < per; ++j) {
        const int b = tid * per + j;
        if (b < nblocks) sum += block_counts[b];
    }
    s_part[tid] = sum;
    __syncthreads();
    if (tid == 0) {
        int64_t run = 0;
        for (int i = 0; i < 256; ++i) {
            int64_t v = s_part[i];
            s_part[i] = run;
            run += v;
        }
        best->num_inliers_scan = run;
        if (best_host) best_host->num_inliers_scan = run;
    }
    __syncthreads();
    int64_t run = s_part[tid];
    for (int j = 0; j < per; ++j) {
        const int b = tid * per + j;
        if (b < nblocks) {
            block_offsets[b] = run;
            run += block_counts[b];
        }
    }
}

__global__ __launch_bounds__(kRB) void ransac_scatter_kernel(const double2* __restrict__ q, const double* __restrict__ alpha,
                                                            const double* __restrict__ alpha_k, int64_t n, int64_t chunk,
                                                            const double* __restrict__ rho, const uint8_t* __restrict__ mask,
                                                            const int64_t* __restrict__ block_counts, RansacBest* best,
                                                            RansacBest* best_host, int64_t* __restrict__ inlier_idx, double* __restrict__ inliers,
                                                            double* __restrict__ out_alpha, double* __restrict__ out_alpha_k,
                                                            int* __restrict__ zero_words = nullptr) {
    __shared__ int s_wave[kRB / 64];
    __shared__ int64_t s_base;
    if (zero_words && blockIdx.x == 0 && threadIdx.x < (int)(kRefineStateBlockTail / sizeof(int))) zero_words[threadIdx.x] = 0;
    __shared__ int64_t s_pre[kRB / 64], s_all[kRB / 64];
    const int tid = threadIdx.x, lane = tid & 63, wv = tid >> 6;
    const int undecided = best->undecided;
    const int64_t i0 = (int64_t)blockIdx.x * chunk;
    const int64_t i1 = (i0 + chunk < n) ? i0 + chunk : n;
    {
        int64_t pre = 0, all = 0;
        for (int b = tid; b < (int)gridDim.x; b += kRB) {
            const int64_t cnt = block_counts[b];
            all += cnt;
            if (b < (int)blockIdx.x) pre += cnt;
        }
#pragma unroll
        for (int off = 32; off > 0; off >>= 1) {
            pre += __shfl_down(pre, off);
            all += __shfl_down(all, off);
        }
        if (lane == 0) s_pre[wv] = pre, s_all[wv] = all;
        __syncthreads();
        if (tid == 0) {
            int64_t p2 = 0, a2 = 0;
            for (int w2 = 0; w2 < kRB / 64; ++w2) p2 += s_pre[w2], a2 += s_all[w2];
            s_base = p2;
            if (blockIdx.x == 0 && !undecided) {
                best->num_inliers_scan = a2;
                if (best_host) best_host->num_inliers_scan = a2;
            }
        }
    }
    if (undecided) return;
    __syncthreads();
    for (int64_t start = i0; start < i1; start += kRB) {
        const int64_t i = start + tid;
        const bool in = (i < i1) && mask[i] != 0;
        const unsigned long long bal = __ballot(in);
        const int prefix = __popcll(bal & ((1ull << lane) - 1ull));
        if (lane == 0) s_wave[wv] = __popcll(bal);
        __syncthreads();
        int woff = 0, total = 0;
#pragma unroll
        for (int w2 = 0; w2 < kRB / 64; ++w2) {
            const int c = s_wave[w2];
            if (w2 < wv) woff += c;
            total += c;
        }
        if (in) {
            const int64_t o = s_base + woff + prefix;
            double2 qq = q[i];
            if (inlier_idx) inlier_idx[o] = i;
            if (inliers) {
                inliers[3 * o + 0] = qq.x;
                inliers[3 * o + 1] = qq.y;
                inliers[3 * o + 2] = 1.0 / rho[i];
// ... 119 lines not shown
    return RSDSFM_OK;
}

int ransac_rows_payload_doubles(int T, bool core_trailer) { return T * NSR + (core_trailer ? 2 : 0); }

int ransac_decide_rows_launch(Ctx* c, const double* rows_all, int nranks, int T, LmState* states, int64_t n_total, int round,
                              int* flags, int* scored, double* trial_count, double* trial_err, bool core_trailer, double* cnt_rt, int cnt_stride) {
    if (cnt_rt && nranks > 256) return fail(c, RSDSFM_ERR_INVALID, "more than 256 ranks");
    RSDSFM_HIP_CHECK(c, hipMemsetAsync(flags, 0, sizeof(int), c->stream));
    hipLaunchKernelGGL(ransac_decide_kernel, dim3(T), dim3(256), 0, c->stream, rows_all, nranks, T, 0, states, n_total, round, (int)KMAX, flags,
                       static_cast<int*>(nullptr), scored, trial_count, trial_err, kTiledFusedBase, static_cast<int*>(nullptr),
                       static_cast<int*>(nullptr), core_trailer ? T * NSR / 2 + 1 : 0, cnt_rt, cnt_stride);
    RSDSFM_HIP_CHECK(c, hipGetLastError());
    return RSDSFM_OK;
}

int ransac_score_rows_launch(Ctx* c, const double* q, const double* u, const double* a, const double* ak, int64_t n,
                             const double* hyp, int T, const LmState* states, int depth_mode, double tol, const int* scored,
                             double* partials, double* rows) {
    const int grid = ransac_pixel_grid(c, n);
    const int groups = ransac_lm_groups(c, grid, T);
    hipLaunchKernelGGL(ransac_score_kernel, dim3(((grid + 7) / 8) * 8 * groups), dim3(kRB), sizeof(double) * T * 2, c->stream,
                       reinterpret_cast<const double2*>(q), reinterpret_cast<const double2*>(u), a, ak, n, hyp, T, states,
                       depth_mode, tol, scored, partials, grid, groups, static_cast<const int*>(nullptr), static_cast<const int*>(nullptr));
    RSDSFM_HIP_CHECK(c, hipGetLastError());
    hipLaunchKernelGGL(ransac_score_rows_kernel, dim3(T), dim3(256), 0, c->stream, partials, grid, T, scored, rows);
    RSDSFM_HIP_CHECK(c, hipGetLastError());
    return RSDSFM_OK;
}

int ransac_score_merge_launch(Ctx* c, const double* rows_all, int nranks, int T, const int* scored, double* trial_count,
                              double* trial_err, double* cnt_rt, int cnt_stride) {
    if (cnt_rt && nranks > 256) return fail(c, RSDSFM_ERR_INVALID, "more than 256 ranks");
    hipLaunchKernelGGL(ransac_reduce_scores_kernel, dim3(T), dim3(256), 0, c->stream, rows_all, nranks, T, scored, trial_count,
                       trial_err, cnt_rt, cnt_stride);
    RSDSFM_HIP_CHECK(c, hipGetLastError());
    return RSDSFM_OK;
}

int ransac_rows_doubles() { return NSR; }

int ransac_pick_launch(Ctx* c, const double* trial_count, const double* trial_err, int T, const double* hyp, RansacBest* best,
                       RansacBest* best_host, const int* d_flags, int* h_flags, int scored_ahead, const double* cnt_rt, int cnt_stride,
                       int nranks, int64_t* m_all, double tie_margin, PickLazy lazy) {
    hipLaunchKernelGGL(ransac_pick_kernel, dim3(1), dim3(64), 0, c->stream, trial_count, trial_err, T, hyp, best, best_host, d_flags, h_flags, scored_ahead,
                       cnt_rt, cnt_stride, nranks, m_all, tie_margin, lazy);
    RSDSFM_HIP_CHECK(c, hipGetLastError());
    return RSDSFM_OK;
}

int ransac_final_launch(Ctx* c, const double* q, const double* u, const double* a, const double* ak, int64_t n,
                        RansacBest* best, const LmState* states, int depth_mode, double tol, double* rho, uint8_t* mask,
                        int64_t* block_counts, int64_t* block_offsets, int64_t* inlier_idx, double* inliers,
                        double* out_alpha, double* out_alpha_k, RansacBest* best_host, int* zero_words) {
    int64_t blocks = (n + kRB - 1) / kRB;
    if (blocks < 1) blocks = 1;
    const int64_t cap = 2048;
    int64_t chunk = kRB;
    if (blocks > cap) {
        chunk = ((blocks + cap - 1) / cap) * kRB;
        blocks = (n + chunk - 1) / chunk;
    }
    hipLaunchKernelGGL(ransac_final_kernel, dim3((int)blocks), dim3(kRB), 0, c->stream, reinterpret_cast<const double2*>(q),
                       reinterpret_cast<const double2*>(u), a, ak, n, chunk, best, states, depth_mode, tol, rho, mask,
                       block_counts);
    RSDSFM_HIP_CHECK(c, hipGetLastError());
    if (inlier_idx || inliers || out_alpha || out_alpha_k) {
        hipLaunchKernelGGL(ransac_scatter_kernel, dim3((int)blocks), dim3(kRB), 0, c->stream, reinterpret_cast<const double2*>(q),
                           a, ak, n, chunk, rho, mask, block_counts, best, best_host, inlier_idx, inliers, out_alpha, out_alpha_k, zero_words);
    } else {
        if (zero_words) RSDSFM_HIP_CHECK(c, hipMemsetAsync(zero_words, 0, kRefineStateBlockTail, c->stream));
        hipLaunchKernelGGL(ransac_scan_kernel, dim3(1), dim3(256), 0, c->stream, block_counts, (int)blocks, block_offsets, best, best_host);
    }
    RSDSFM_HIP_CHECK(c, hipGetLastError());
    return RSDSFM_OK;
}

}
```

### rs-aware-differential-sfm_amd/csrc/refine_host.hip

```cpp
#include <string.h>

#include <algorithm>

#include "rsdsfm_internal.hpp"

namespace rsdsfm {

int refine_begin(Ctx* c, const double* d_flow, int64_t n_flow, int64_t m, const double* d_inl, const double* d_alpha,
                 const double* d_alpha_k, const int64_t* d_inlier_idx, const double v_in[3], const double w_in[3], double k_in,
                 int const_acceleration, int flow_index_mode, double* d_inl_out, const RefineTail* tail, const RansacBest* d_best,
                 void* ws_base, RefineRun* run, RefineState* hs_prefetch, double* d_zpartials, bool exact, const FinishClaim* claim) {
    if (m < 0 || n_flow < 0 || (!d_best && (!v_in || !w_in))) return fail(c, RSDSFM_ERR_INVALID, "bad arguments");
    if (flow_index_mode != RSDSFM_FLOW_COMPAT_RANK && flow_index_mode != RSDSFM_FLOW_GATHERED) return fail(c, RSDSFM_ERR_INVALID, "unknown flow_index_mode");
    if (flow_index_mode == RSDSFM_FLOW_GATHERED && m > 0 && !d_inlier_idx) return fail(c, RSDSFM_ERR_INVALID, "gathered mode needs inlier_idx");
    if (m > 0 && (!d_flow || !d_inl || !d_alpha || !d_alpha_k || !d_inl_out)) return fail(c, RSDSFM_ERR_INVALID, "null device pointer");
    const int np = const_acceleration ? 7 : 6;
    const size_t M = (size_t)std::max<int64_t>(m, 1);
    const size_t npart = (size_t)(d_best ? refine_partials_doubles_cap(c) : refine_partials_doubles(c, m));
    int rc = RSDSFM_OK;
    if (!ws_base) {
        rc = ensure_ws(c, refine_workspace_bytes(c, m, d_best != nullptr));
        if (rc != RSDSFM_OK) return rc;
        ws_base = c->d_ws;
    }
    rc = ensure_pinned(c, sizeof(RefineState) + 64);
    if (rc != RSDSFM_OK) return rc;
    Arena ws(ws_base);
    RefineBuffers& B = run->B;
    B = RefineBuffers();
    B.flow = d_flow;
    B.n_flow = n_flow;
    B.m = m;
    B.m_on_device = d_best != nullptr;
    B.inl = d_inl;
    B.alpha = d_alpha;
    B.alpha_k = d_alpha_k;
    B.inlier_idx = d_inlier_idx;
    B.flow_index_mode = flow_index_mode;
    static_assert(sizeof(RefineState) % sizeof(int) == 0, "flag follows the state");
    char* state_block = ws.take<char>(sizeof(RefineState) + 64);
    B.state = reinterpret_cast<RefineState*>(state_block);
    B.uu = ws.take<double>(4 * M);
    B.beta = ws.take<double>(M);
    B.rho_a = ws.take<double>(M);
    B.rho_b = ws.take<double>(M);
    B.srho = ws.take<double>(M);
    B.partials = ws.take<double>(npart);
    B.bad_index = reinterpret_cast<int*>(state_block + sizeof(RefineState));
    B.zpartials = d_zpartials;
    if (claim && claim->on && d_zpartials) B.claim = *claim;
    run->np = np;
    run->rf = !exact && c->lm_arithmetic == 0 && c->refine_arithmetic == 0;
    if (run->rf) c->refine_rf_runs += 1;
    run->d_inl_out = d_inl_out;
    run->tail = tail;
    run->launched = 0;
    run->hint_prev = c->refine_iters_hint;
    run->hs = hs_prefetch ? hs_prefetch : static_cast<RefineState*>(c->h_pinned);
    run->prefetch = hs_prefetch != nullptr;
    run->prefetched = false;
    B.state_host = hs_prefetch;
    if (d_best && claim && claim->on && run->rf && !c->refine_stage_separate) {
        B.best_dev = d_best;
    } else if (d_best) {
        rc = refine_state_from_best_launch(c, d_best, B, np);
        if (rc != RSDSFM_OK) return rc;
    } else {
        RefineState* hs = static_cast<RefineState*>(c->h_pinned);
        int* h_bad = reinterpret_cast<int*>(static_cast<char*>(c->h_pinned) + sizeof(RefineState));
        memset(hs, 0, sizeof(RefineState));
        hs->np = np;
        for (int i = 0; i < 3; ++i) {
            hs->p[i] = v_in[i];
            hs->p[3 + i] = w_in[i];
        }
        hs->p[6] = k_in;
        hs->termination = -1;
        hs->radius = kInitialRadius;
        hs->need_schur = 1;
        memset(h_bad, 0, kRefineStateBlockTail);
        RSDSFM_HIP_CHECK(c, hipMemcpyAsync(B.state, hs, sizeof(RefineState) + kRefineStateBlockTail, hipMemcpyHostToDevice, c->stream));
    }
    rc = refine_trace_reset(c);
    if (rc != RSDSFM_OK) return rc;
    if (!run->rf) {
        rc = refine_init_launch(c, B, np);
        if (rc != RSDSFM_OK) return rc;
    }
    const int hp = run->hint_prev;
    run->chunk = (hp >= 0 && hp <= 3) ? hp + 1 : (hp > 8 ? std::min(hp + 1, 28) : 7);
    return refine_enqueue_chunk(c, run);
}

int refine_enqueue_chunk(Ctx* c, RefineRun* run) {
    static const bool watch = getenv("RSDSFM_SYNC_WATCHDOG_S") != nullptr;
    if (watch) {
        const RefineBuffers B = run->B;
        const int launched = run->launched, chunk = run->chunk, rf = run->rf ? 1 : 0;
        set_sync_dumper([B, launched, chunk, rf](Ctx* cc) {
            fprintf(stderr, "[rsdsfm] last refinement chunk enqueued: slots [%d, %d), radius-factorised %d\n", launched, launched + chunk, rf);
            refine_rf_debug_dump(cc, B);
        });
    }
    if (run->rf) {
        for (int i = 0; i <= run->chunk; ++i) {
            const int g = run->launched + i;
// ... 204 lines not shown
```

### rs-aware-differential-sfm_amd/csrc/refine_kernels.hip

```cpp
#include "refine_common.hpp"

namespace rsdsfm {


template <int NP>
__global__ __launch_bounds__(kFB) void refine_init_kernel(const double2* __restrict__ flow, int64_t n_flow, int64_t m,
                                                         const double* __restrict__ inl, const double* __restrict__ alpha,
                                                         const double* __restrict__ alpha_k,
                                                         const int64_t* __restrict__ inlier_idx, int flow_index_mode,
                                                         const RefineState* __restrict__ st, double4* __restrict__ xyuv,
                                                         double* __restrict__ beta_out, double* __restrict__ rho0,
                                                         double* __restrict__ srho, double* __restrict__ partials,
                                                         int* __restrict__ bad_index, int want_zsum) {
    using CT = Counts<NP>;
    __shared__ double s_red[kFB / 64][CT::NINIT];
    const PassShape ps = pass_shape(st, m);
    if (!ps.live) return;
    m = ps.m;
    double p[7];
#pragma unroll
    for (int c = 0; c < 7; ++c) p[c] = st->p[c];
    double acc[CT::NINIT];
#pragma unroll
    for (int s = 0; s < CT::NINIT; ++s) acc[s] = 0.0;
// ... 386 lines not shown
template <int NP>
__global__ __launch_bounds__(kFB) void refine_decide_kernel(const double* __restrict__ partials, int nblocks,
                                                           RefineState* st, double* __restrict__ trace, int trace_rows) {
    using CT = Counts<NP>;
    __shared__ double s_red[kFB / 64][CT::NBACK];
    __shared__ double s[CT::NBACK];
    if (st->termination >= 0) return;
    const int solve_ok = st->solve_ok;
    if (solve_ok) reduce_partials<CT::NBACK>(partials, nblocks >= 0 ? nblocks : st->grid, CT::BACK_MAX, s_red, s);
    if (threadIdx.x != 0) return;
    (void)decide_serial<NP>(st, s, solve_ok, trace, trace_rows);
}

__global__ __launch_bounds__(kFB) void refine_finish_kernel(int64_t m, const double* __restrict__ inl,
                                                           const double* __restrict__ rho_a, const double* __restrict__ rho_b,
                                                           const RefineState* __restrict__ st, double* __restrict__ inl_out,
                                                           double* __restrict__ zpartials, RefineState* __restrict__ state_host,
                                                           const int* __restrict__ bad_index) {
    __shared__ double s_red[kFB / 64];
    if (state_host && blockIdx.x == 0) {
        static_assert(sizeof(RefineState) % 8 == 0, "copied as 8-byte words");
        for (int i = threadIdx.x; i < (int)(sizeof(RefineState) / 8); i += kFB)
            reinterpret_cast<double*>(state_host)[i] = reinterpret_cast<const double*>(st)[i];
        if (threadIdx.x == 0) *reinterpret_cast<int*>(reinterpret_cast<char*>(state_host) + sizeof(RefineState)) = *bad_index;
    }
    const double* __restrict__ rho = st->cur ? rho_b : rho_a;
    if (m < 0) m = st->m;
    const int64_t stride = (int64_t)gridDim.x * kFB;
    double acc = 0.0;
    for (int64_t i = (int64_t)blockIdx.x * kFB + threadIdx.x; i < m; i += stride) {
        inl_out[3 * i] = inl[3 * i];
        inl_out[3 * i + 1] = inl[3 * i + 1];
        const double z = 1.0 / rho[i];
        inl_out[3 * i + 2] = z;
        acc += z;
    }
    if (zpartials) {
        const double r = wave_sum(acc);
        if ((threadIdx.x & 63) == 0) s_red[threadIdx.x >> 6] = r;
        __syncthreads();
        if (threadIdx.x == 0) {
            double t = s_red[0];
            for (int w2 = 1; w2 < kFB / 64; ++w2) t += s_red[w2];
            zpartials[blockIdx.x] = t;
        }
    }
}

__global__ __launch_bounds__(kFB) void refine_finish_claim_kernel(int64_t m, const double* __restrict__ inl, const double* __restrict__ rho_a,
                                                                 const double* __restrict__ rho_b, const RefineState* __restrict__ st,
                                                                 double* __restrict__ inl_out, double* __restrict__ zpartials,
                                                                 RefineState* __restrict__ state_host, const int* __restrict__ bad_index,
                                                                 double fx, double fy, double cx, double cy, int rows, int ncols,
                                                                 unsigned* __restrict__ owner, unsigned tag, int32_t* __restrict__ ys) {
    __shared__ double s_red[kFB / 64];
    if (state_host && blockIdx.x == 0) {
        for (int i = threadIdx.x; i < (int)(sizeof(RefineState) / 8); i += kFB)
            reinterpret_cast<double*>(state_host)[i] = reinterpret_cast<const double*>(st)[i];
        if (threadIdx.x == 0) *reinterpret_cast<int*>(reinterpret_cast<char*>(state_host) + sizeof(RefineState)) = *bad_index;
    }
    const double* __restrict__ rho = st->cur ? rho_b : rho_a;
    if (m < 0) m = st->m;
    const int64_t stride = (int64_t)gridDim.x * kFB;
    double acc = 0.0;
    for (int64_t i = (int64_t)blockIdx.x * kFB + threadIdx.x; i < m; i += stride) {
        const double xn = inl[3 * i], yn = inl[3 * i + 1];
        inl_out[3 * i] = xn;
        inl_out[3 * i + 1] = yn;
        const double z = 1.0 / rho[i];
        inl_out[3 * i + 2] = z;
        acc += z;
        const int x = (int)(fx * xn + cx + 0.5);
        const int y = (int)(fy * yn + cy + 0.5);
        ys[i] = y;
        if (x >= 0 && x < ncols && y >= 0 && y < rows) atomicMax(&owner[(int64_t)x * rows + y], tag | (unsigned)i);
    }
    const double r = wave_sum(acc);
    if ((threadIdx.x & 63) == 0) s_red[threadIdx.x >> 6] = r;
    __syncthreads();
    if (threadIdx.x == 0) {
        double t = s_red[0];
        for (int w2 = 1; w2 < kFB / 64; ++w2) t += s_red[w2];
        zpartials[blockIdx.x] = t;
    }
}

__global__ void refine_state_from_best_kernel(const RansacBest* __restrict__ best, RefineState* __restrict__ st, int np, int cap,
                                              int* __restrict__ bad_index) {
    if (threadIdx.x != 0 || blockIdx.x != 0) return;
    RefineState z;
    memset(&z, 0, sizeof(z));
    z.np = np;
    for (int i = 0; i < 3; ++i) {
        z.p[i] = best->hyp[3 + i];
        z.p[3 + i] = best->hyp[i];
    }
    z.p[6] = best->hyp[6];
    z.termination = -1;
    z.radius = kInitialRadius;
    z.need_schur = 1;
    const int64_t m = best->undecided ? 0 : best->num_inliers_scan;
    z.m = m;
    int64_t b = (m + kFB - 1) / kFB;
    if (b < 1) b = 1;
    if (b > cap) {
        const int64_t iters = (b + cap - 1) / cap;
        b = (b + iters - 1) / iters;
    }
    z.grid = (int)b;
    *st = z;
    bad_index[0] = 0;
    bad_index[4] = bad_index[5] = bad_index[6] = 0;
}

static inline int refine_grid_cap(const Ctx* c) { return c->num_cus * kWorkgroupsPerCu; }
static inline int refine_grid(const Ctx* c, int64_t m) {
    int64_t b = (m + kFB - 1) / kFB;
    const int64_t cap = (int64_t)c->num_cus * kWorkgroupsPerCu;
    if (b < 1) b = 1;
    if (b > cap) {
        const int64_t iters = (b + cap - 1) / cap;
        b = (b + iters - 1) / iters;
    }
    return (int)b;
}

static inline int refine_partials_half(const Ctx* c) { return refine_grid_cap(c) * SlotRow<7>::NW; }
constexpr int kStateDoubles = (int)((sizeof(RefineState) + 63) / 64 * 8);
int refine_partials_doubles_cap(const Ctx* c) { return 2 * refine_partials_half(c) + 2 * kStateDoubles + 8 + refine_rf_extra_doubles(); }
int refine_partials_half_doubles(const Ctx* c) { return refine_partials_half(c); }
int refine_state_doubles() { return kStateDoubles; }
int refine_partials_doubles(const Ctx* c, int64_t m) { (void)m; return refine_partials_doubles_cap(c); }
static inline double* rows_buffer(const Ctx* c, const RefineBuffers& B, int which) { return B.partials + (size_t)(which & 1) * refine_partials_half(c); }
static inline RefineState* chunk_state(const Ctx* c, const RefineBuffers& B, int which) {
    return reinterpret_cast<RefineState*>(B.partials + 2 * (size_t)refine_partials_half(c) + (size_t)(which & 1) * kStateDoubles);
}
static inline const RefineState* slot_state_in(const Ctx* c, const RefineBuffers& B, int j) { return j == 0 ? B.state : chunk_state(c, B, j - 1); }

int refine_state_from_best_launch(Ctx* c, const RansacBest* d_best, const RefineBuffers& B, int np) {
    hipLaunchKernelGGL(refine_state_from_best_kernel, dim3(1), dim3(64), 0, c->stream, d_best, B.state, np, refine_grid_cap(c), B.bad_index);
    RSDSFM_HIP_CHECK(c, hipGetLastError());
    return RSDSFM_OK;
}

template <int NP>
static int refine_init_t(Ctx* c, const RefineBuffers& B) {
    const int grid = B.m_on_device ? refine_grid_cap(c) : refine_grid(c, B.m);
    const int64_t m_arg = B.m_on_device ? -1 : B.m;
    hipLaunchKernelGGL(refine_init_kernel<NP>, dim3(grid), dim3(kFB), 0, c->stream, reinterpret_cast<const double2*>(B.flow), B.n_flow,
                       m_arg, B.inl, B.alpha, B.alpha_k, B.inlier_idx, B.flow_index_mode, B.state, reinterpret_cast<double4*>(B.uu),
                       B.beta, B.rho_a, B.srho, B.partials, B.bad_index, B.want_zsum ? 1 : 0);
    RSDSFM_HIP_CHECK(c, hipGetLastError());
    hipLaunchKernelGGL(refine_init_decide_kernel<NP>, dim3(1), dim3(kFB), 0, c->stream, B.partials, B.m_on_device ? -1 : grid, B.state, m_arg);
    RSDSFM_HIP_CHECK(c, hipGetLastError());
    return RSDSFM_OK;
}

template <int NV>
__global__ __launch_bounds__(kFB) void refine_row_kernel(const double* __restrict__ partials, int nblocks, int max_slot,
                                                        double* __restrict__ row, const RefineState* __restrict__ st = nullptr) {
    __shared__ double s_red[kFB / 64][NV];
    __shared__ double s[NV];
    if (nblocks < 0) nblocks = st->grid;
    reduce_partials<NV>(partials, nblocks, max_slot, s_red, s);
    if (threadIdx.x < NV) row[threadIdx.x] = s[threadIdx.x];
}

template <int NP>
static int refine_stage_rows_t(Ctx* c, const RefineBuffers& B, int stage, double* row) {
    using CT = Counts<NP>;
    const int grid = B.m_on_device ? refine_grid_cap(c) : refine_grid(c, B.m);
    if (stage == 0) {
        hipLaunchKernelGGL(refine_init_kernel<NP>, dim3(grid), dim3(kFB), 0, c->stream, reinterpret_cast<const double2*>(B.flow),
                           B.n_flow, B.m_on_device ? (int64_t)-1 : B.m, B.inl, B.alpha, B.alpha_k, B.inlier_idx, B.flow_index_mode, B.state,
                           reinterpret_cast<double4*>(B.uu), B.beta, B.rho_a, B.srho, B.partials, B.bad_index, B.want_zsum ? 1 : 0);
        RSDSFM_HIP_CHECK(c, hipGetLastError());
        hipLaunchKernelGGL(refine_row_kernel<CT::NINIT>, dim3(1), dim3(kFB), 0, c->stream, B.partials, B.m_on_device ? -1 : grid, CT::INIT_MAX, row,
                           static_cast<const RefineState*>(B.state));
    } else if (B.m_on_device) {
        return fail(c, RSDSFM_ERR_INVALID, "two-stage refinement protocol: the inlier count must be known on the host");
    } else if (stage == 1) {
        hipLaunchKernelGGL(refine_schur_kernel<NP>, dim3(grid), dim3(kFB), 0, c->stream, B.m,
                           reinterpret_cast<const double4*>(B.uu), B.beta, B.alpha, B.alpha_k, B.rho_a, B.rho_b, B.srho, B.state, B.partials);
        RSDSFM_HIP_CHECK(c, hipGetLastError());
        hipLaunchKernelGGL(refine_row_kernel<CT::NSCHUR>, dim3(1), dim3(kFB), 0, c->stream, B.partials, grid, -1, row);
    } else {
        hipLaunchKernelGGL(refine_backsub_kernel<NP>, dim3(grid), dim3(kFB), 0, c->stream, B.m,
                           reinterpret_cast<const double4*>(B.uu), B.beta, B.alpha, B.alpha_k, B.rho_a, B.rho_b, B.srho, B.state, B.partials, B.want_zsum ? 1 : 0);
        RSDSFM_HIP_CHECK(c, hipGetLastError());
        hipLaunchKernelGGL(refine_row_kernel<CT::NBACK>, dim3(1), dim3(kFB), 0, c->stream, B.partials, grid, CT::BACK_MAX, row);
    }
    RSDSFM_HIP_CHECK(c, hipGetLastError());
    return RSDSFM_OK;
// ... 243 lines not shown
    return RSDSFM_OK;
}

template <int NP>
static int refine_slot_rows_t(Ctx* c, const RefineBuffers& B, double* row, int j, const double* rows_all_prev, int nranks) {
    const int grid = B.m_on_device ? refine_grid_cap(c) : refine_grid(c, B.m);
    hipLaunchKernelGGL(refine_slot_pass_kernel<NP>, dim3(grid), dim3(kFB), 0, c->stream, B.m_on_device ? (int64_t)-1 : B.m, reinterpret_cast<const double4*>(B.uu), B.beta, B.alpha,
                       B.alpha_k, B.rho_a, B.rho_b, B.srho, slot_state_in(c, B, j), chunk_state(c, B, j), rows_all_prev, nranks, rows_buffer(c, B, 0),
                       B.want_zsum ? 1 : 0, c->d_refine_trace, c->refine_trace_rows);
    RSDSFM_HIP_CHECK(c, hipGetLastError());
    hipLaunchKernelGGL(refine_slot_row_kernel<NP>, dim3(1), dim3(kFB), 0, c->stream, rows_buffer(c, B, 0), B.m_on_device ? -1 : grid, row,
                       static_cast<const RefineState*>(B.state));
    RSDSFM_HIP_CHECK(c, hipGetLastError());
    return RSDSFM_OK;
}
int refine_slot_row_doubles(int np) { return np == 7 ? SlotRow<7>::NW : SlotRow<6>::NW; }
int refine_slot_partials_doubles(const Ctx* c, int64_t m) { return refine_partials_doubles(c, m); }
int refine_slot_rows_launch(Ctx* c, const RefineBuffers& B, int np, double* row, int j, const double* rows_all_prev, int nranks) {
    return np == 7 ? refine_slot_rows_t<7>(c, B, row, j, rows_all_prev, nranks) : refine_slot_rows_t<6>(c, B, row, j, rows_all_prev, nranks);
}
int refine_slot_apply_launch(Ctx* c, const RefineBuffers& B, int np, const double* rows_all, int nranks, int chunk) {
    if (np == 7)
        hipLaunchKernelGGL(refine_slot_apply_kernel<7>, dim3(1), dim3(kFB), 0, c->stream, rows_all, nranks, chunk_state(c, B, chunk - 1), B.state,
                           c->d_refine_trace, c->refine_trace_rows);
    else
        hipLaunchKernelGGL(refine_slot_apply_kernel<6>, dim3(1), dim3(kFB), 0, c->stream, rows_all, nranks, chunk_state(c, B, chunk - 1), B.state,
                           c->d_refine_trace, c->refine_trace_rows);
    RSDSFM_HIP_CHECK(c, hipGetLastError());
    return RSDSFM_OK;
}

int refine_stage_row_doubles(int np, int stage) {
    if (np == 7) return stage == 0 ? Counts<7>::NINIT : stage == 1 ? Counts<7>::NSCHUR : Counts<7>::NBACK;
    return stage == 0 ? Counts<6>::NINIT : stage == 1 ? Counts<6>::NSCHUR : Counts<6>::NBACK;
}
int refine_stage_rows_launch(Ctx* c, const RefineBuffers& B, int np, int stage, double* row) {
    return np == 7 ? refine_stage_rows_t<7>(c, B, stage, row) : refine_stage_rows_t<6>(c, B, stage, row);
}
int refine_stage_apply_launch(Ctx* c, const RefineBuffers& B, int np, int stage, const double* rows_all, int nranks, int64_t m_total, const int64_t* m_total_dev) {
    return np == 7 ? refine_stage_apply_t<7>(c, B, stage, rows_all, nranks, m_total, m_total_dev)
                   : refine_stage_apply_t<6>(c, B, stage, rows_all, nranks, m_total, m_total_dev);
}

int refine_init_launch(Ctx* c, const RefineBuffers& B, int np) { return np == 7 ? refine_init_t<7>(c, B) : refine_init_t<6>(c, B); }
int refine_iter_launch(Ctx* c, const RefineBuffers& B, int np, int j, int chunk) { return np == 7 ? refine_iter_t<7>(c, B, j, chunk) : refine_iter_t<6>(c, B, j, chunk); }

int refine_finish_grid(const Ctx* c, const RefineBuffers& B) { return B.m_on_device ? refine_grid_cap(c) : refine_grid(c, B.m); }

int refine_finish_launch(Ctx* c, const RefineBuffers& B, double* inl_out) {
    if (!B.m_on_device && B.m == 0 && !B.zpartials && !B.state_host) return RSDSFM_OK;
    if (B.claim.on) {
        hipLaunchKernelGGL(refine_finish_claim_kernel, dim3(refine_finish_grid(c, B)), dim3(kFB), 0, c->stream, B.m_on_device ? (int64_t)-1 : B.m, B.inl,
                           B.rho_a, B.rho_b, B.state, inl_out, B.zpartials, B.state_host, B.bad_index, B.claim.fx, B.claim.fy, B.claim.cx, B.claim.cy,
                           B.claim.rows, B.claim.cols, B.claim.owner, B.claim.tag, B.claim.ys);
        RSDSFM_HIP_CHECK(c, hipGetLastError());
        return RSDSFM_OK;
    }
    hipLaunchKernelGGL(refine_finish_kernel, dim3(refine_finish_grid(c, B)), dim3(kFB), 0, c->stream,
                       B.m_on_device ? (int64_t)-1 : B.m, B.inl, B.rho_a, B.rho_b, B.state, inl_out, B.zpartials, B.state_host, B.bad_index);
    RSDSFM_HIP_CHECK(c, hipGetLastError());
    return RSDSFM_OK;
}

}
```

### rs-aware-differential-sfm_amd/csrc/refine_rf_kernels.hip

```cpp
#include "refine_common.hpp"

#ifndef RF_LOADS_ONLY
#define RF_LOADS_ONLY 0
#endif
#ifndef RF_NP7_PREFETCH
#define RF_NP7_PREFETCH 0
#endif

namespace rsdsfm {

namespace {

constexpr int kRfListCap = 64;
constexpr int kRfEntry = 8;

template <int NP>
struct RfRow {
    static constexpr int TRI = NP * (NP + 1) / 2;
    static constexpr int OFF_JTJ = 0, OFF_B = TRI, OFF_JTB = 2 * TRI, OFF_C = 2 * TRI + NP;
    static constexpr int NSCHUR = 2 * TRI + 2 * NP;
    static constexpr int MODEL = NSCHUR, STEPSQ = NSCHUR + 1, COST2 = NSCHUR + 2, XSQ = NSCHUR + 3, ZSUM = NSCHUR + 4, GMAX = NSCHUR + 5;
    static constexpr int NW = NSCHUR + 6;
    static constexpr int NF = TRI + NP;
    static_assert(NW % 2 == 0, "rows are read as double2");
};

struct RfExt {
    double sums[RfRow<7>::NSCHUR];
    double nlist;
    double list[kRfListCap * kRfEntry];
};
constexpr int kRfExtDoubles = (int)((sizeof(RfExt) + 63) / 64 * 8);
constexpr int kRfListDoubles = 2 + kRfListCap * kRfEntry;

enum RfGuard : int {
    kRfGuardNonFinite = 1, kRfGuardGradient = 2, kRfGuardModel = 3, kRfGuardParameter = 4, kRfGuardFunction = 5, kRfGuardQuality = 6,
    kRfGuardPivot = 7, kRfGuardList = 8, kRfGuardRadius = 9
};
constexpr double kBandGradient = 1e-4, kBandParameter = 1e-2, kBandFunction = 1e-4, kBandQuality = 1e-4, kBandModel = 1e-12, kBandPivot = 1e-9;

struct RfPoint {
    double v0, v1, v2, w0, w1, w2, k, c1, c2;
};
__device__ __forceinline__ RfPoint rf_point(const double* p) {
    RfPoint P;
    P.v0 = p[0], P.v1 = p[1], P.v2 = p[2], P.w0 = p[3], P.w1 = p[4], P.w2 = p[5], P.k = p[6];
    const double t = 2.0 + p[6];
    P.c1 = 2.0 / t;
    P.c2 = 2.0 / (t * t);
    return P;
}
__device__ __forceinline__ RfPoint rf_point_uniform(const RfPoint& Q) {
    RfPoint P;
    P.v0 = uniform_d(Q.v0), P.v1 = uniform_d(Q.v1), P.v2 = uniform_d(Q.v2), P.w0 = uniform_d(Q.w0), P.w1 = uniform_d(Q.w1), P.w2 = uniform_d(Q.w2);
    P.k = uniform_d(Q.k), P.c1 = uniform_d(Q.c1), P.c2 = uniform_d(Q.c2);
    return P;
}

struct RfGeom {
    double x, y, xy, xx1, yy1;
};
__device__ __forceinline__ RfGeom rf_geom(double x, double y) {
    RfGeom g;
    g.x = x, g.y = y, g.xy = x * y, g.xx1 = __builtin_fma(x, x, 1.0), g.yy1 = __builtin_fma(y, y, 1.0);
    return g;
}
__device__ __forceinline__ void rf_av(const RfGeom& g, double v0, double v1, double v2, double& a0, double& a1) {
    a0 = __builtin_fma(g.x, v2, -v0);
    a1 = __builtin_fma(g.y, v2, -v1);
}
__device__ __forceinline__ void rf_bw(const RfGeom& g, double w0, double w1, double w2, double& b0, double& b1) {
    b0 = __builtin_fma(g.y, w2, __builtin_fma(-g.xx1, w1, g.xy * w0));
    b1 = __builtin_fma(-g.x, w2, __builtin_fma(-g.xy, w1, g.yy1 * w0));
}
template <int NP>
__device__ __forceinline__ void rf_beta(double ab, double ak, const RfPoint& P, double& be, double& dbe) {
    if (NP == 6) {
        be = ab, dbe = 0.0;
    } else {
        be = P.c1 * __builtin_fma(P.k, ak, ab);
        dbe = P.c2 * __builtin_fma(2.0, ak, -ab);
    }
}
__device__ __forceinline__ bool rf_flagged(double h, double h0) { return !(h >= __builtin_fma(2.02e-6, h0, 2.02e-6) && h <= 1e30); }

template <int NP>
struct RfEval {
    double r0, r1, J0, J1, h, in0, in1;
    double P0[NP], P1[NP];
};
// ... 477 lines not shown
        RF_BEAT(21);
        const int again = L.loop;
        __syncthreads();
        if (!again) break;
        resolve = true;
    }
    RF_BEAT(30);
    if (ext_out) {
        if (tid < RR::NSCHUR) ext_out->sums[tid] = L.cur[tid];
        const int n = L.nlist;
        for (int q = tid; q < n * kRfEntry; q += kFB) ext_out->list[q] = L.list[q];
        if (tid == 0) ext_out->nlist = (double)n;
    }
    RF_BEAT(31);
#undef RF_BEAT
}

struct RfPassArgs {
    int64_t m;
    const double4* xyuv_in;
    double4* xyuv_out;
    double* beta;
    const double* alpha;
    const double* alpha_k;
    double* rho_a;
    double* rho_b;
    const RefineState* st_in;
    RefineState* st_out;
    const double* rows_prev;
    int nrows_prev, row_stride;
    RfLists lists_prev;
    int* list_count;
    double* list_entries;
    int* list_count_zero;
    const RfExt* ext_in;
    RfExt* ext_out;
    double* partials;
    double* trace;
    int trace_rows;
    int64_t m_total;
    const int64_t* m_total_dev;
    const double2* flow;
    int64_t n_flow;
    const double* inl;
    const int64_t* inlier_idx;
    int flow_index_mode;
    int* bad_index;
    unsigned long long* beat;
    int slot;
    const RansacBest* best;
    int grid_cap;
    unsigned long long* stamps;
};

struct RfLoad {
    double4 c4;
    double rho, ab, ak;
};
template <int NP>
__device__ __forceinline__ RfLoad rf_load(const RfPassArgs& A, const double* __restrict__ rho, int64_t i, bool live) {
    RfLoad l;
    l.c4 = make_double4(0.0, 0.0, 0.0, 0.0), l.rho = 0.0, l.ab = 0.0, l.ak = 0.0;
    if (live) {
        l.c4 = A.xyuv_in[i];
        l.rho = rho[i];
        if (NP == 6) {
            l.ab = A.beta[i];
        } else {
            l.ab = A.alpha[i], l.ak = A.alpha_k[i];
        }
    }
    return l;
}

}

template <int NP, bool FIRST, bool ZSUM>
__global__ __launch_bounds__(kFB) void refine_rf_pass_kernel(const RfPassArgs A) {
    using RR = RfRow<NP>;
    __shared__ RfStageLds<NP> s_stage;
    __shared__ double s_red[kFB / 64][RR::NW];
    __shared__ RefineState s_state;
    const bool stamp = A.stamps && blockIdx.x == 0 && threadIdx.x == 0;
    if (A.beat && threadIdx.x == 0) {
        if (A.beat[7]) atomicAdd(&A.beat[2], 1ull);
        if (blockIdx.x == 0) A.beat[0] = ((unsigned long long)A.slot << 8) | 1;
        if (blockIdx.x < 512) A.beat[8 + blockIdx.x] = ((unsigned long long)A.slot << 8) | 1;
    }
    __shared__ unsigned long long tk[8];
    if (stamp) {
#pragma unroll
        for (int i = 0; i < 8; ++i) tk[i] = 0;
    }
    if (stamp) tk[0] = wall_clock64();
    if (FIRST && A.best) {
        if (threadIdx.x < sizeof(RefineState) / 8) reinterpret_cast<unsigned long long*>(&s_state)[threadIdx.x] = 0ull;
        __syncthreads();
        if (threadIdx.x == 0) {
            RefineState& z = s_state;
            z.np = NP;
            for (int i = 0; i < 3; ++i) {
                z.p[i] = A.best->hyp[3 + i];
                z.p[3 + i] = A.best->hyp[i];
            }
            z.p[6] = A.best->hyp[6];
            z.termination = -1;
            z.radius = kInitialRadius;
            z.need_schur = 1;
            const int64_t mb = A.best->undecided ? 0 : A.best->num_inliers_scan;
            z.m = mb;
            int64_t b = (mb + kFB - 1) / kFB;
            if (b < 1) b = 1;
            if (b > A.grid_cap) {
                const int64_t iters = (b + A.grid_cap - 1) / A.grid_cap;
                b = (b + iters - 1) / iters;
            }
            z.grid = (int)b;
        }
        __syncthreads();
    } else {
        state_to_lds(&s_state, A.st_in);
    }
    RefineState* st = &s_state;
    if (stamp) tk[1] = wall_clock64();
    if (FIRST) {
        if (threadIdx.x < 7) st->p0[threadIdx.x] = st->p[threadIdx.x];
        if (threadIdx.x == 0) st->rf = 1, st->rf_guard = 0, st->rf_resolves = 0, st->pending_apply = 0;
        __syncthreads();
    } else if (st->termination < 0 && st->pending_apply) {
        int64_t mt = A.m_total_dev ? *A.m_total_dev : (A.m_total >= 0 ? A.m_total : (A.m >= 0 ? A.m : st->m));
        rf_apply_body<NP>(st, s_stage, A.rows_prev, A.nrows_prev >= 0 ? A.nrows_prev : st->grid, A.row_stride, A.lists_prev, A.ext_in,
                          blockIdx.x == 0 ? A.ext_out : nullptr, mt, blockIdx.x == 0 ? A.trace : nullptr, A.trace_rows, stamp ? tk + 4 : nullptr);
        __syncthreads();
    }
    if (threadIdx.x == 0) st->pending_apply = st->termination < 0 ? 1 : 0;
    __syncthreads();
    if (stamp) tk[2] = wall_clock64();
    if (A.beat && threadIdx.x == 0) {
        if (blockIdx.x == 0) A.beat[0] = ((unsigned long long)A.slot << 8) | 2;
        if (blockIdx.x < 512) A.beat[8 + blockIdx.x] = ((unsigned long long)A.slot << 8) | ((st->termination >= 0 || (A.m < 0 && (int)blockIdx.x >= st->grid)) ? 9 : 2);
        if (A.beat[7] && (st->termination >= 0 || (A.m < 0 && (int)blockIdx.x >= st->grid))) atomicAdd(&A.beat[3], 1ull);
    }
    if (blockIdx.x == 0) {
        state_from_lds(A.st_out, st);
        if (threadIdx.x == 0) *A.list_count_zero = 0;
    }
    if (st->termination >= 0) return;
    const PassShape ps = pass_shape(st, A.m);
    if (!ps.live) return;
    const int64_t m = ps.m;
    double acc[RR::NW];
#pragma unroll
    for (int s = 0; s < RR::NW; ++s) acc[s] = 0.0;
    constexpr bool kLdsC = NP == 7 && !FIRST;
    __shared__ double s_cacc[kLdsC ? 3 * NP : 1][kLdsC ? kFB : 1];
    double* const lds_c = kLdsC ? &s_cacc[0][threadIdx.x] : nullptr;
    if (kLdsC) {
#pragma unroll
        for (int a = 0; a < 3 * NP; ++a) lds_c[a * kFB] = 0.0;
    }
    const int64_t stride = (int64_t)ps.grid * kFB;
    const int64_t i0 = (int64_t)blockIdx.x * kFB + threadIdx.x;
    RfPoint P0q = rf_point(st->p0);
    const RfPoint P0 = rf_point_uniform(P0q);
    if (FIRST) {
        RfPoint Pq = rf_point(st->p);
        const RfPoint P = rf_point_uniform(Pq);
        for (int64_t i = i0; i < m; i += stride) {
            int64_t fi = (A.flow_index_mode == RSDSFM_FLOW_GATHERED) ? A.inlier_idx[i] : i;
            if (fi < 0 || fi >= A.n_flow) {
                *A.bad_index = 1;
                fi = 0;
            }
            const double2 f = A.flow[fi];
            const double x = A.inl[3 * i], y = A.inl[3 * i + 1];
            const double rho = 1.0 / A.inl[3 * i + 2];
            const double al = A.alpha[i], ak = A.alpha_k[i];
            A.xyuv_out[i] = make_double4(x, y, f.x, f.y);
            const double ab = NP == 6 ? P.c1 * __builtin_fma(P.k, ak, al) : al;
            if (NP == 6) A.beta[i] = ab;
            A.rho_a[i] = rho;
            const RfGeom g = rf_geom(x, y);
            double be, dbe;
            rf_beta<NP>(ab, ak, P, be, dbe);
            RfEval<NP> o;
            rf_resid<NP>(g, f.x, f.y, be, P, rho, o);
            rf_jac<NP>(g, be, dbe, rho, o);
            acc[RR::COST2] = __builtin_fma(o.r0, o.r0, __builtin_fma(o.r1, o.r1, acc[RR::COST2]));
            acc[RR::GMAX] = fmax(acc[RR::GMAX], fabs(__builtin_fma(o.J0, o.r0, o.J1 * o.r1)));
            acc[RR::XSQ] = __builtin_fma(rho, rho, acc[RR::XSQ]);
            if (ZSUM) acc[RR::ZSUM] += 1.0 / rho;
            const bool flagged = rf_flagged(o.h, o.h);
            const double ihm = flagged ? 0.0 : rcp_core(flagged ? 1.0 : o.h);
            rf_schur_accumulate<NP>(o, ihm, acc);
            if (flagged) rf_list_append(A.list_count, A.list_entries, x, y, f.x, f.y, ab, ak, rho, i);
        }
    } else {
        RfPoint Pq = rf_point(st->p), Pcq = rf_point(st->pc);
        const RfPoint P = rf_point_uniform(Pq), Pc = rf_point_uniform(Pcq);
        double dp[7];
#pragma unroll
        for (int c = 0; c < 7; ++c) dp[c] = uniform_d(st->dp[c]);
        const double inv_radius = uniform_d(1.0 / st->radius);
        const double psi = uniform_d(1.0 / (1.0 + 1.0 / st->radius));
        const double* __restrict__ rho = st->cur ? A.rho_b : A.rho_a;
        double* __restrict__ cand = st->cur ? A.rho_a : A.rho_b;
        auto body = [&](const RfLoad& l0, int64_t i) {
            const double x = l0.c4.x, y = l0.c4.y, ux = l0.c4.z, uy = l0.c4.w, rh = l0.rho;
            const RfGeom g = rf_geom(x, y);
            double be, dbe, bec, dbec, be0, dbe0;
            rf_beta<NP>(l0.ab, l0.ak, P, be, dbe);
            rf_beta<NP>(l0.ab, l0.ak, Pc, bec, dbec);
            rf_beta<NP>(l0.ab, l0.ak, P0, be0, dbe0);
            RfEval<NP> o;
            rf_resid<NP>(g, ux, uy, be, P, rh, o);
            double da0, da1, db0, db1;
            rf_av(g, dp[0], dp[1], dp[2], da0, da1);
            rf_bw(g, dp[3], dp[4], dp[5], db0, db1);
            double t0 = be * __builtin_fma(rh, da0, db0), t1 = be * __builtin_fma(rh, da1, db1);
            if (NP == 7) {
                const double dk = dbe * dp[6];
                t0 = __builtin_fma(dk, o.in0, t0);
                t1 = __builtin_fma(dk, o.in1, t1);
            }
            double a00, a10;
            rf_av(g, P0.v0, P0.v1, P0.v2, a00, a10);
            const double h0 = (be0 * be0) * __builtin_fma(a00, a00, a10 * a10);
            const double gJ = __builtin_fma(o.J0, o.r0, o.J1 * o.r1), tJ = __builtin_fma(o.J0, t0, o.J1 * t1);
            const bool flagged = rf_flagged(o.h, h0);
            double drho = -((psi * (gJ + tJ)) * rcp_core(flagged ? 1.0 : o.h));
            if (__builtin_amdgcn_ballot_w64(flagged) != 0) {
                if (flagged) {
                    asm volatile("; listed inlier: exact e-block inverse" ::: "memory");
                    double sr, E0, E1;
                    const double ete_inv = rf_ete_inv_exact(o.J0, o.J1, h0, inv_radius, sr, E0, E1);
                    drho = -((ete_inv * (sr * (gJ + tJ))) * sr);
                }
            }
            const double m0 = __builtin_fma(o.J0, drho, t0), m1 = __builtin_fma(o.J1, drho, t1);
            acc[RR::MODEL] -= __builtin_fma(m0, __builtin_fma(0.5, m0, o.r0), m1 * __builtin_fma(0.5, m1, o.r1));
            const double cd = rh + drho;
            cand[i] = cd;
            acc[RR::STEPSQ] = __builtin_fma(drho, drho, acc[RR::STEPSQ]);
            RfEval<NP> oc;
            rf_resid<NP>(g, ux, uy, bec, Pc, cd, oc);
            rf_jac<NP>(g, bec, dbec, cd, oc);
            acc[RR::COST2] = __builtin_fma(oc.r0, oc.r0, __builtin_fma(oc.r1, oc.r1, acc[RR::COST2]));
            acc[RR::GMAX] = fmax(acc[RR::GMAX], fabs(__builtin_fma(oc.J0, oc.r0, oc.J1 * oc.r1)));
// ... 13 lines not shown
                const RfLoad l2 = rf_load<NP>(A, rho, i2, i2 <= last);
#if RF_LOADS_ONLY
                acc[0] += l0.c4.x + l0.c4.y + l0.c4.z + l0.c4.w + l0.rho + l0.ab;
                cand[i] = l0.rho;
#else
                body(l0, i);
#endif
                l0 = l1;
                l1 = l2;
            }
        } else {
#if RF_NP7_PREFETCH == 1
            RfLoad l0 = rf_load<NP>(A, rho, i0, i0 <= last);
            for (int64_t i = i0; i < m; i += stride) {
                const RfLoad l1 = rf_load<NP>(A, rho, i + stride, i + stride <= last);
                body(l0, i);
                l0 = l1;
            }
#else
            for (int64_t i = i0; i < m; i += stride) body(rf_load<NP>(A, rho, i, true), i);
#endif
        }
    }
    if (kLdsC) {
        int tri = 0;
#pragma unroll
        for (int a = 0; a < NP; ++a) {
            acc[RR::OFF_C + a] = lds_c[a * kFB];
            tri += NP - 1 - a;
            acc[RR::OFF_JTJ + tri] = lds_c[(NP + a) * kFB];
            acc[RR::OFF_B + tri] = lds_c[(2 * NP + a) * kFB];
            tri += 1;
        }
    }
    if (A.beat && threadIdx.x == 0 && blockIdx.x < 512) A.beat[8 + blockIdx.x] = ((unsigned long long)A.slot << 8) | 3;
    if (A.beat && (threadIdx.x & 63) == 0 && blockIdx.x < 64) A.beat[8 + 256 + blockIdx.x * 4 + 0] |= 1ull << (threadIdx.x >> 6);
    if (A.beat && blockIdx.x == 0 && threadIdx.x == 0) A.beat[0] = ((unsigned long long)A.slot << 8) | 3;
    if (stamp) tk[3] = wall_clock64();
    if (A.stamps && blockIdx.x == 0 && (threadIdx.x & 63) == 0) A.stamps[8 + (threadIdx.x >> 6)] += wall_clock64();
    static_assert(RR::GMAX == RR::NW - 1, "the max slot is the row's last");
    block_reduce_store_halving<RR::NW>(acc, s_red, A.partials + (int64_t)blockIdx.x * RR::NW);
    if (A.beat && threadIdx.x == 0) {
        if (A.beat[7]) atomicAdd(&A.beat[3], 1ull);
        if (blockIdx.x == 0) A.beat[0] = ((unsigned long long)A.slot << 8) | 4;
        if (blockIdx.x < 512) A.beat[8 + blockIdx.x] = ((unsigned long long)A.slot << 8) | 4;
    }
    if (stamp) {
        tk[4] = wall_clock64();
        A.stamps[0] += tk[1] - tk[0], A.stamps[1] += tk[2] - tk[1], A.stamps[2] += tk[3] - tk[2], A.stamps[3] += tk[4] - tk[3], A.stamps[4] += 1;
        if (tk[4 + 0]) A.stamps[5] += tk[4 + 0] - tk[1], A.stamps[6] += tk[4 + 1] - tk[4 + 0], A.stamps[7] += tk[2] - tk[4 + 1];
    }
}

template <int NP>
__global__ __launch_bounds__(kFB) void refine_rf_apply_kernel(const double* __restrict__ rows, int nrows, int row_stride, RfLists lists,
                                                             const RefineState* __restrict__ st_in, RefineState* __restrict__ st_out,
                                                             const RfExt* __restrict__ ext_in, RfExt* __restrict__ ext_out, int64_t m_total,
                                                             const int64_t* __restrict__ m_total_dev, double* __restrict__ trace, int trace_rows,
                                                             unsigned long long* __restrict__ beat, int slot) {
    __shared__ RfStageLds<NP> s_stage;
    __shared__ RefineState s_state;
    if (beat && threadIdx.x == 0) beat[1] = ((unsigned long long)slot << 8) | 1;
    state_to_lds(&s_state, st_in);
    RefineState* st = &s_state;
    if (st->termination < 0 && st->pending_apply) {
        const int64_t mt = m_total_dev ? *m_total_dev : (m_total >= 0 ? m_total : st->m);
        rf_apply_body<NP>(st, s_stage, rows, nrows >= 0 ? nrows : st->grid, row_stride, lists, ext_in, ext_out, mt, trace, trace_rows, nullptr, beat);
    }
    __syncthreads();
    if (beat && threadIdx.x == 0) beat[1] = ((unsigned long long)slot << 8) | 40;
    if (threadIdx.x == 0) st->pending_apply = 0;
    __syncthreads();
    state_from_lds(st_out, st);
}

template <int NP>
__global__ __launch_bounds__(kFB) void refine_rf_row_kernel(const double* __restrict__ partials, int nblocks, const RefineState* __restrict__ st,
                                                           const int* __restrict__ list_count, const double* __restrict__ list_entries,
                                                           double* __restrict__ row) {
    using RR = RfRow<NP>;
    __shared__ double s_grp[ReduceShape<RR::NW>::G][RR::NW];
    __shared__ double s[RR::NW];
    if (nblocks < 0) nblocks = st->grid;
    reduce_partials_groups<RR::NW>(partials, nblocks, RR::GMAX, s_grp, threadIdx.x, RR::NW, 0);
    __syncthreads();
    reduce_partials_slots<RR::NW>(s_grp, RR::GMAX, s, threadIdx.x);
    __syncthreads();
    if (threadIdx.x < RR::NW) row[threadIdx.x] = s[threadIdx.x];
    const int n = *list_count;
    double* lr = row + RR::NW;
    if (threadIdx.x == 0) {
        reinterpret_cast<int*>(lr)[0] = n;
        reinterpret_cast<int*>(lr)[1] = 0;
        lr[1] = 0.0;
    }
    if ((int)threadIdx.x < n && n <= kRfListCap) {
        const double* e = list_entries + (size_t)threadIdx.x * kRfEntry;
        int rank = 0;
        for (int j = 0; j < n; ++j) rank += (list_entries[(size_t)j * kRfEntry + 7] < e[7]) ? 1 : 0;
#pragma unroll
        for (int q = 0; q < kRfEntry; ++q) lr[2 + (size_t)rank * kRfEntry + q] = e[q];
    }
}


int refine_rf_extra_doubles() { return 3 * kRfListCap * kRfEntry + 2 * kRfExtDoubles + 8; }
// ... 29 lines not shown
    Lo.cs[0] = reinterpret_cast<RefineState*>(p), Lo.cs[1] = reinterpret_cast<RefineState*>(p + sd);
    p += 2 * sd + 8;
    for (int i = 0; i < 3; ++i) Lo.list[i] = p + (size_t)i * kRfListCap * kRfEntry;
    p += 3 * kRfListCap * kRfEntry;
    Lo.ext[0] = reinterpret_cast<RfExt*>(p), Lo.ext[1] = reinterpret_cast<RfExt*>(p + kRfExtDoubles);
    return Lo;
}
inline int rf_mod3(int g) { return ((g % 3) + 3) % 3; }
inline int* rf_list_count(const RefineBuffers& B, int g) { return refine_rf_counters(B) + rf_mod3(g); }
inline double* rf_list_entries(const RfLayout& Lo, int g) { return Lo.list[rf_mod3(g)]; }
inline RfLists rf_lists_of(const RfLayout& Lo, const RefineBuffers& B, int g, const double* rows_all, int nranks, int nw) {
    RfLists l;
    if (rows_all) {
        l.counts = reinterpret_cast<const int*>(rows_all + nw), l.count_stride = 2 * (nw + kRfListDoubles);
        l.entries = rows_all + nw + 2, l.entry_stride = nw + kRfListDoubles, l.nlists = nranks;
    } else {
        l.counts = rf_list_count(B, g), l.count_stride = 0, l.entries = rf_list_entries(Lo, g), l.entry_stride = 0, l.nlists = 1;
    }
    return l;
}

struct RfBeat {
    const Ctx* c;
    unsigned long long* words;
};
RfBeat g_beats[32];
int g_nbeats = 0;
unsigned long long* rf_beat(Ctx* c) {
    static const bool on = getenv("RSDSFM_SYNC_WATCHDOG_S") != nullptr && getenv("RSDSFM_NO_BEAT") == nullptr;
    if (!on) return nullptr;
    for (int i = 0; i < g_nbeats; ++i)
        if (g_beats[i].c == c) return g_beats[i].words;
    if (g_nbeats >= 32) return nullptr;
    unsigned long long* w = nullptr;
    if (hipHostMalloc((void**)&w, 64 + 8 * 512, hipHostMallocDefault) != hipSuccess) return nullptr;
    for (int i = 0; i < 8 + 512; ++i) w[i] = 0;
    w[7] = getenv("RSDSFM_BEAT_COUNT_WORKGROUPS") ? 1 : 0;
    g_beats[g_nbeats].c = c, g_beats[g_nbeats].words = w;
    ++g_nbeats;
    return w;
}
unsigned long long* rf_stamps(Ctx* c) {
    static int on = -1;
    static unsigned long long* buf = nullptr;
    if (on < 0) {
        const char* e = getenv("RSDSFM_RF_STAMPS");
        on = (e && e[0] == '1') ? 1 : 0;
        if (on && (hipMalloc(&buf, 128) != hipSuccess || hipMemset(buf, 0, 128) != hipSuccess)) buf = nullptr;
    }
    (void)c;
    return buf;
}
template <int NP, bool ZSUM>
void rf_pass_launch_t(Ctx* c, const RfPassArgs& A, bool first, int grid) {
    if (first)
        hipLaunchKernelGGL((refine_rf_pass_kernel<NP, true, ZSUM>), dim3(grid), dim3(kFB), 0, c->stream, A);
    else
        hipLaunchKernelGGL((refine_rf_pass_kernel<NP, false, ZSUM>), dim3(grid), dim3(kFB), 0, c->stream, A);
}
}

int refine_rf_pass_launch(Ctx* c, const RefineBuffers& B, int np, int g, int g_first, const double* rows_all_prev, int nranks, int64_t m_total,
                          const int64_t* m_total_dev, bool publish) {
    const RfLayout Lo = rf_layout(c, B);
    const int grid = B.m_on_device ? rf_grid_cap(c) : rf_grid(c, B.m);
    const int nw = np == 7 ? RfRow<7>::NW : RfRow<6>::NW;
    RfPassArgs A = {};
    A.m = B.m_on_device ? -1 : B.m;
    A.xyuv_in = reinterpret_cast<const double4*>(B.uu);
    A.xyuv_out = reinterpret_cast<double4*>(B.uu);
    A.beta = B.beta;
    A.alpha = B.alpha;
    A.alpha_k = B.alpha_k;
    A.rho_a = B.rho_a;
    A.rho_b = B.rho_b;
    A.st_in = g == g_first ? B.state : Lo.cs[(g - 1) & 1];
    A.st_out = publish ? B.state : Lo.cs[g & 1];
    if (rows_all_prev)
        A.rows_prev = rows_all_prev, A.nrows_prev = nranks, A.row_stride = nw + kRfListDoubles;
    else
        A.rows_prev = Lo.rows[(g - 1) & 1], A.nrows_prev = B.m_on_device ? -1 : grid, A.row_stride = nw;
    A.lists_prev = rf_lists_of(Lo, B, g - 1, rows_all_prev, nranks, nw);
    A.list_count = rf_list_count(B, g);
    A.list_entries = rf_list_entries(Lo, g);
    A.list_count_zero = rf_list_count(B, g + 1);
    A.ext_in = Lo.ext[(g - 1) & 1];
    A.ext_out = Lo.ext[g & 1];
    A.partials = Lo.rows[g & 1];
    A.trace = c->d_refine_trace;
    A.trace_rows = c->refine_trace_rows;
    A.m_total = m_total;
    A.m_total_dev = m_total_dev;
    A.flow = reinterpret_cast<const double2*>(B.flow);
    A.n_flow = B.n_flow;
    A.inl = B.inl;
    A.inlier_idx = B.inlier_idx;
    A.flow_index_mode = B.flow_index_mode;
    A.bad_index = B.bad_index;
    A.best = g == 0 ? B.best_dev : nullptr;
    A.grid_cap = rf_grid_cap(c);
    A.stamps = rf_stamps(c);
    A.beat = rf_beat(c);
    A.slot = g;
    const bool first = g == 0;
    if (np == 7) {
        if (B.want_zsum) rf_pass_launch_t<7, true>(c, A, first, grid); else rf_pass_launch_t<7, false>(c, A, first, grid);
    } else {
        if (B.want_zsum) rf_pass_launch_t<6, true>(c, A, first, grid); else rf_pass_launch_t<6, false>(c, A, first, grid);
    }
    RSDSFM_HIP_CHECK(c, hipGetLastError());
    return RSDSFM_OK;
}

int refine_rf_apply_launch(Ctx* c, const RefineBuffers& B, int np, int g, bool to_published, const double* rows_all, int nranks, int64_t m_total,
                           const int64_t* m_total_dev) {
    const RfLayout Lo = rf_layout(c, B);
    const int grid = B.m_on_device ? rf_grid_cap(c) : rf_grid(c, B.m);
    const int nw = np == 7 ? RfRow<7>::NW : RfRow<6>::NW;
    const double* rows = rows_all ? rows_all : Lo.rows[g & 1];
    const int nrows = rows_all ? nranks : (B.m_on_device ? -1 : grid);
    const int stride = rows_all ? nw + kRfListDoubles : nw;
    const RfLists lists = rf_lists_of(Lo, B, g, rows_all, nranks, nw);
    RefineState* st_io = Lo.cs[g & 1];
    if (np == 7)
        hipLaunchKernelGGL(refine_rf_apply_kernel<7>, dim3(1), dim3(kFB), 0, c->stream, rows, nrows, stride, lists, st_io, to_published ? B.state : st_io,
                           Lo.ext[g & 1], Lo.ext[(g + 1) & 1], m_total, m_total_dev, c->d_refine_trace, c->refine_trace_rows, rf_beat(c), g);
    else
        hipLaunchKernelGGL(refine_rf_apply_kernel<6>, dim3(1), dim3(kFB), 0, c->stream, rows, nrows, stride, lists, st_io, to_published ? B.state : st_io,
                           Lo.ext[g & 1], Lo.ext[(g + 1) & 1], m_total, m_total_dev, c->d_refine_trace, c->refine_trace_rows, rf_beat(c), g);
    RSDSFM_HIP_CHECK(c, hipGetLastError());
    return RSDSFM_OK;
}

int refine_rf_row_launch(Ctx* c, const RefineBuffers& B, int np, int g, double* row) {
    const RfLayout Lo = rf_layout(c, B);
    const int grid = B.m_on_device ? rf_grid_cap(c) : rf_grid(c, B.m);
    if (np == 7)
        hipLaunchKernelGGL(refine_rf_row_kernel<7>, dim3(1), dim3(kFB), 0, c->stream, Lo.rows[g & 1], B.m_on_device ? -1 : grid, static_cast<const RefineState*>(Lo.cs[g & 1]),
                           rf_list_count(B, g), rf_list_entries(Lo, g), row);
    else
        hipLaunchKernelGGL(refine_rf_row_kernel<6>, dim3(1), dim3(kFB), 0, c->stream, Lo.rows[g & 1], B.m_on_device ? -1 : grid, static_cast<const RefineState*>(Lo.cs[g & 1]),
                           rf_list_count(B, g), rf_list_entries(Lo, g), row);
    RSDSFM_HIP_CHECK(c, hipGetLastError());
    return RSDSFM_OK;
}

void refine_rf_debug_dump(Ctx* c, const RefineBuffers& B) {
    const RfLayout Lo = rf_layout(c, B);
    hipStream_t s2 = nullptr;
    if (hipStreamCreateWithFlags(&s2, hipStreamNonBlocking) != hipSuccess) return;
    RefineState h[3];
    int cnt[8] = {0, 0, 0, 0, 0, 0, 0, 0};
    const RefineState* src[3] = {B.state, Lo.cs[0], Lo.cs[1]};
    for (int i = 0; i < 3; ++i) (void)hipMemcpyAsync(&h[i], src[i], sizeof(RefineState), hipMemcpyDeviceToHost, s2);
    (void)hipMemcpyAsync(cnt, B.bad_index, sizeof(int) * 8, hipMemcpyDeviceToHost, s2);
    if (hipStreamSynchronize(s2) != hipSuccess) {
        fprintf(stderr, "[rsdsfm] refinement dump: the copies did not complete either\n");
        return;
    }
    const char* names[3] = {"published", "chunk state 0", "chunk state 1"};
    for (int i = 0; i < 3; ++i)
// ... 34 lines not shown
```

### rs-aware-differential-sfm_amd/csrc/rsdsfm_internal.hpp

```cpp
#pragma once

#include <hip/hip_runtime.h>
#include <stdint.h>

#include <functional>
#include <string>
#include <vector>

#include "../../include/rsdsfm.h"

namespace rsdsfm {

constexpr int kMaxIter = 50;
constexpr int kRefineTraceCols = RSDSFM_REFINE_TRACE_COLS;
constexpr double kInitialRadius = 1e4;
constexpr double kMaxRadius = 1e16;
constexpr double kMinRadius = 1e-32;
constexpr double kMinRelDecrease = 1e-3;
constexpr double kMinLmDiag = 1e-6;
constexpr double kMaxLmDiag = 1e32;
constexpr double kFunctionTol = 1e-6;
constexpr double kGradientTol = 1e-10;
static_assert(kGradientTol < 1.0, "the indicator encoding of the gradient-maximum slots needs kGradientTol < 1");
constexpr double kParameterTol = 1e-8;
constexpr int kMaxInvalid = 5;
constexpr double kLmaTie = 1e-11;

constexpr int KMAX = 3;
constexpr int NS = 3 + 5 * KMAX;

struct Pose {
    double v[3];
    double w[3];
    double k;
};

struct LmScal {
    int32_t status;
    int32_t n_hist;
    int32_t K;
    int32_t write_which;
    int32_t iteration;
    int32_t num_successful;
    int32_t num_unsuccessful;
    int32_t invalid_run;
    int32_t termination;
    int32_t rho_holds;
    int32_t launches;
    int32_t next_launch;
    int32_t predict;
    int32_t restart;
    double radius;
    double decrease_factor;
    double cost;
    double initial_cost;
    double cand[KMAX];
};
struct LmState : LmScal {
    double hist[kMaxIter];
};

constexpr size_t kRefineStateBlockTail = 32;
struct RansacBest {
    int32_t best_trial;
    int32_t undecided;
    int64_t num_inliers;
    int64_t num_inliers_scan;
    double inlier_error;
    double hyp[8];
    int32_t lma_tie;
    int32_t shared_best;
    int32_t _pad_shared;
    int32_t lazy_pending;
};
struct PickLazy {
    int* scored = nullptr;
    int* list = nullptr;
    int* list_count = nullptr;
};

constexpr int kScoreIdleLimit = 4;
constexpr int kRansacBatch = 128;

struct Ctx {
    int device = 0;
    hipStream_t stream = nullptr;
    bool own_stream = false;
    std::string err;
    double* d_partials = nullptr;
    unsigned* d_tickets = nullptr;
    LmState* d_lm = nullptr;
    LmState* h_lm = nullptr;
    int lm_issued_k = 0;
    int true_flow_exhaustive = 0;
    int ransac_fused_base = 2;
    int ransac_score_idle = kScoreIdleLimit;
    int refine_iters_hint = -1;
    int ransac_standard_math = 0;
    int* d_core_flag = nullptr;
    int core_epoch = 0;
    int ransac_math_mode = 0;
    int64_t ransac_restarts = 0;
    int lm_arithmetic = 0;
    int lma_hold = 0;
    bool lma_count_only_force = false;
    int64_t lma_count_only_runs = 0, lma_lazy_runs = 0;
    int lma_unique_run = 0;
    int64_t lma_restarts = 0;
    int64_t lma_handed_over = 0;
    int lma_last_guard = 0;
    int* d_lma_list = nullptr;
    int depth_lma_parity = 0;
    int lma_cand[2] = {2, 1};
    int ransac_spec_miss = 0;
    int frame_dense_hint = 1;
    int lm_issued_d = 0;
    int depth_epoch = 0;
    int depth_standard_math = 0;
    int64_t depth_restarts = 0;
    int depth_core_launch = 0;
    int prof_what = 0;
    void* d_stage = nullptr;
    size_t stage_bytes = 0;
    void* d_ws = nullptr;
    size_t ws_bytes = 0;
    void* d_frame = nullptr;
    size_t frame_bytes = 0;
    void* h_pinned = nullptr;
    hipEvent_t ev_ready = nullptr;
    size_t pinned_bytes = 0;
    int num_cus = 256;
    int ransac_k0 = 0;
    int ransac_not_one_step = -1;
    bool profile = false;
    hipEvent_t ev_prof[2] = {nullptr, nullptr};
    unsigned long long* d_clk_probe = nullptr;
    bool prof_pending = false;
    double* d_refine_trace = nullptr;
    int refine_trace_rows = 0;
    int depth_variant = 0;
    void* d_tile = nullptr;
    size_t tile_bytes = 0;
    void* tile_session = nullptr;
    int tile_np = 0;
    void* flow_pair = nullptr;
    void* flow_clip = nullptr;
    int flow_batch = 0;
    unsigned* d_claim[3] = {nullptr, nullptr, nullptr};
    size_t claim_words[3] = {0, 0, 0};
    unsigned claim_epoch[3] = {0, 0, 0};
    void* dist = nullptr;
    void* frame_run = nullptr;
    hipStream_t aux_stream = nullptr;
    hipEvent_t ev_fork = nullptr, ev_join = nullptr, ev_seq = nullptr;
    int frame_side_flatten = 3;
    int frame_tail = 0;
    unsigned long long* d_flat_counters = nullptr;
    int seq_lanes = 0;
    int refine_stage_mode = 0;
    bool refine_stage_separate = false;
    int refine_arithmetic = 0;
    int64_t refine_rf_runs = 0, refine_rf_restarts = 0, refine_rf_resolves = 0;
    int refine_rf_last_guard = 0;
    struct RansacCache {
        uint64_t tag = 0, stage_gen = 0;
        const double *d_u = nullptr, *d_inl = nullptr, *d_alpha = nullptr, *d_alpha_k = nullptr;
        const int64_t* d_idx = nullptr;
        int64_t n = 0, m = 0;
        const void* h_u = nullptr;
        double u_probe[16] = {0};
        double inl_probe[16] = {0};
    } ransac_cache;
    uint64_t stage_gen = 0, ransac_tag_counter = 0;
    int64_t refine_cache_hits = 0;
    std::vector<rsdsfm_ctx*> lanes;
};
constexpr int kSequenceLanesDefault = 3;
void dist_release(Ctx* c);
void dist_reset_hold(Ctx* c);
void frame_release(Ctx* c);
void flow_release(Ctx* c);

constexpr int kDepthBlock = 256;
constexpr int kDepthMaxBlocks = 512;
constexpr int kDecideBlock = 256;
constexpr int kDepthBatchMax = 8;

#define RSDSFM_HIP_CHECK(ctx, expr)                                                            \
    do {                                                                                       \
        hipError_t _e = (expr);                                                                \
        if (_e != hipSuccess) {                                                                \
            (ctx)->err = std::string(#expr) + ": " + hipGetErrorString(_e);                    \
            return RSDSFM_ERR_HIP;                                                             \
        }                                                                                      \
    } while (0)

struct DeviceGuard {
    int prev = -1;
    bool switched = false;
    explicit DeviceGuard(const Ctx* c) {
        if (hipGetDevice(&prev) == hipSuccess && prev != c->device) switched = hipSetDevice(c->device) == hipSuccess;
    }
    ~DeviceGuard() {
        if (switched) (void)hipSetDevice(prev);
    }
    DeviceGuard(const DeviceGuard&) = delete;
    DeviceGuard& operator=(const DeviceGuard&) = delete;
};

// ... 82 lines not shown
int depth_map_launch(Ctx* c, double* d_inl, int64_t m, const double v[3], double fx, double fy, double cx, double cy, int rows,
                     int cols, double* d_depth_map, int32_t* d_xs, int32_t* d_ys, double* d_header, double* d_partials,
                     double* h_header = nullptr, const double* v_dev = nullptr, const int64_t* m_dev = nullptr,
                     const PoseTableOut* pt = nullptr);
int depth_map_slab_launch(Ctx* c, double* d_inl, int64_t m, const double* d_zsums, int nz, int64_t m_total, const double v[3],
                          double fx, double fy, double cx, double cy, int rows, int col0, int ncols, double* d_depth_map,
                          int32_t* d_xs, int32_t* d_ys, double* d_header, double* h_header = nullptr, const double* v_dev = nullptr,
                          const int64_t* m_dev = nullptr, const PoseTableOut* pt = nullptr);
int claim_map_acquire(Ctx* c, int which, size_t npix, unsigned** map, unsigned* tag, unsigned* mask);
int claim_map_reserve(Ctx* c, int which, size_t words);
int zsum_row_launch(Ctx* c, const double* d_inl, int64_t m, double* d_partials, double* d_out);
}

namespace rsdsfm {
struct Minimal9Direct {
    const double* img = nullptr;
    int rows = 0, cols = 0, alpha_ones = 0;
    double fx = 0, fy = 0, cx = 0, cy = 0, gamma = 0;
    int* core_flag = nullptr;
    int core_epoch = 0;
    double* probe = nullptr;
};
int minimal9_launch(Ctx* c, const double* q, const double* u, const double* alpha, const double* alpha_k,
                    const int32_t* samples, int T, int use_alpha_k, int k_sign_mode, double* hyp_out, void* zero_begin = nullptr,
                    size_t zero_bytes = 0, const Minimal9Direct* direct = nullptr);
struct DenseFlatten {
    double thr = 0.0;
    double *d_q = nullptr, *d_u = nullptr, *d_alpha = nullptr, *d_alpha_k = nullptr;
    unsigned long long* d_counters = nullptr;
    int64_t* total_out = nullptr;
};
int minimal9_flatten_launch(Ctx* c, const int32_t* samples, int T, int use_alpha_k, int k_sign_mode, double* hyp_out, void* zero_begin, size_t zero_bytes,
                            const Minimal9Direct& direct, double thr, double* d_q, double* d_u, double* d_alpha, double* d_alpha_k,
                            unsigned long long* d_counters, int64_t* total_out);
}

namespace rsdsfm {
int ransac_pixel_grid(const Ctx* c, int64_t n);
int ransac_lm_partials_doubles(const Ctx* c, int64_t n, int batch);
int ransac_lm_round_launch(Ctx* c, const double* q, const double* u, const double* a, const double* ak, int64_t n,
                           const double* hyp, int T, LmState* states, double* partials, int* flags, int* scored,
                           double* trial_count, double* trial_err, int round, double tol, int k0, int fused_base, bool core_math,
                           const int* m9_core_flag = nullptr, int m9_core_epoch = 0, int* unscored_list = nullptr);
int ransac_score_launch(Ctx* c, const double* q, const double* u, const double* a, const double* ak, int64_t n,
                        const double* hyp, int T, const LmState* states, int depth_mode, double tol, const int* scored,
                        double* partials, double* trial_count, double* trial_err, const int* unscored_list = nullptr, const int* unscored_count = nullptr);
int ransac_pick_launch(Ctx* c, const double* trial_count, const double* trial_err, int T, const double* hyp, RansacBest* best,
                       RansacBest* best_host = nullptr, const int* d_flags = nullptr, int* h_flags = nullptr, int scored_ahead = 0,
                       const double* cnt_rt = nullptr, int cnt_stride = 0, int nranks = 0, int64_t* m_all = nullptr, double tie_margin = 0.0,
                       PickLazy lazy = PickLazy());
int ransac_final_launch(Ctx* c, const double* q, const double* u, const double* a, const double* ak, int64_t n,
                        RansacBest* best, const LmState* states, int depth_mode, double tol, double* rho, uint8_t* mask,
                        int64_t* block_counts, int64_t* block_offsets, int64_t* inlier_idx, double* inliers,
                        double* out_alpha, double* out_alpha_k, RansacBest* best_host = nullptr, int* zero_words = nullptr);
int ransac_rows_doubles();
int ransac_lm_rows_launch(Ctx* c, const double* q, const double* u, const double* a, const double* ak, int64_t n,
                          const double* hyp, int T, const LmState* states, double* partials, int round, double tol, double* rows,
                          int* core_flags = nullptr, const int* m9_flag = nullptr, int m9_epoch = 0);
int ransac_rows_payload_doubles(int T, bool core_trailer);
int ransac_decide_rows_launch(Ctx* c, const double* rows_all, int nranks, int T, LmState* states, int64_t n_total, int round,
                              int* flags, int* scored, double* trial_count, double* trial_err, bool core_trailer = false,
                              double* cnt_rt = nullptr, int cnt_stride = 0);
int ransac_score_rows_launch(Ctx* c, const double* q, const double* u, const double* a, const double* ak, int64_t n,
                             const double* hyp, int T, const LmState* states, int depth_mode, double tol, const int* scored,
                             double* partials, double* rows);
int ransac_score_merge_launch(Ctx* c, const double* rows_all, int nranks, int T, const int* scored, double* trial_count,
                              double* trial_err, double* cnt_rt = nullptr, int cnt_stride = 0);
void sample_indices(int64_t n, int T, uint64_t seed, int32_t* out);
int64_t ransac_lma_partials_doubles(const Ctx* c, int64_t n, int batch);
size_t ransac_lma_list_ints(int batch);
int ransac_lma_launch(Ctx* c, const double* q, const double* u, const double* a, const double* ak, int64_t n, const double* hyp, int T,
                      LmState* states, double* partials, int* flags, int* scored, double* trial_count, double* trial_err, double tol,
                      const int* cand_steps, int ncand, int* irr_count, int* irr_list, int* unscored_list, int* guard_word,
                      const int* m9_core_flag = nullptr, int m9_core_epoch = 0, bool count_only = false);
int ransac_lma_rows_doubles();
int ransac_lma_rows_launch(Ctx* c, const double* q, const double* u, const double* a, const double* ak, int64_t n, const double* hyp, int T,
                           double* partials, double tol, const int* cand_steps, int ncand, int* irr_count, int* irr_list, double* rows);
int ransac_lma_decide_rows_launch(Ctx* c, const double* rows_all, int nranks, int64_t rank_stride, int T, int64_t n_total, const double* hyp,
                                  LmState* states, int* flags, int* scored, double* trial_count, double* trial_err, double tol, const int* cand_steps,
                                  int ncand, int* unscored_list, int* guard_word, double* cnt_rt, int cnt_stride, const int* m9_core_flag = nullptr,
                                  int m9_core_epoch = 0);
}

namespace rsdsfm {
struct RefineState {
    int32_t np, cur, iteration, invalid_run, num_successful, num_unsuccessful, termination, solve_ok;
    double p[7], pc[7], sp[7], yp[7];
    double radius, decrease_factor, cost, initial_cost, x_norm, gmax, stepsq_p;
    int64_t m;
    int32_t grid;
    int32_t need_schur;
    double zsum;
    int32_t slots;
    int32_t spec_miss_run;
    int32_t pending_apply;
    int32_t rf;
    double dp[7];
    double p0[7];
    int32_t rf_guard, rf_resolves;
};
constexpr int kTermRestartExact = 64;
struct FinishClaim {
    bool on = false;
    double fx = 0.0, fy = 0.0, cx = 0.0, cy = 0.0;
    int rows = 0, cols = 0;
    int32_t* ys = nullptr;
    unsigned* owner = nullptr;
    unsigned tag = 0, mask = 0;
};
struct RefineBuffers {
    const double* flow;
    int64_t n_flow, m;
    bool m_on_device = false;
    const double* inl;
    const double* alpha;
    const double* alpha_k;
    const int64_t* inlier_idx;
    int flow_index_mode;
    RefineState* state;
    double* uu;
    double* beta;
    double* rho_a;
    double* rho_b;
    double* srho;
    double* partials;
    int* bad_index;
    RefineState* state_host = nullptr;
    double* zpartials = nullptr;
    const RansacBest* best_dev = nullptr;
    FinishClaim claim;
    bool want_zsum = false;
};
size_t ransac_pinned_bytes(int T);
typedef std::function<int(const RansacBest*)> RansacSpecTail;
struct RansacRun {
    int pc = 0;
    const double *d_q = nullptr, *d_u = nullptr, *d_a = nullptr, *d_ak = nullptr;
    int64_t n = 0;
    int T = 0, Tn = 1, batch = 1, depth_mode = 0, use_alpha_k = 0, k_sign_mode = 0, k0 = 0, fused_base = 0;
    double tol = 0.0;
    rsdsfm_ransac_out* out = nullptr;
    const RansacSpecTail* spec_tail = nullptr;
    bool* spec_tail_held = nullptr;
    int core_epoch = 0;
    int* d_unscored = nullptr;
    bool core_math = true;
    bool analytic = false;
    bool lma_restarted = false;
    int* refine_flag_words = nullptr;
    bool count_only = false;
    int lazy_rounds = 0;
    int shared_best = 0;
    double tie_margin = 0.0;
    int lma_guard = 0;
    bool lma_tie_seen = false;
    int lma_cand[2] = {2, 1}, lma_cand_next[2] = {0, 0};
    int *d_irr_count = nullptr, *d_irr_list = nullptr;
    bool restarted = false;
    bool tail_ahead = true;
    const Minimal9Direct* direct = nullptr;
    const DenseFlatten* dense = nullptr;
    const std::function<int()>* after_minimal9 = nullptr;
    std::vector<int32_t> samples;
    double *d_hyp = nullptr, *d_partials = nullptr, *d_tcount = nullptr, *d_terr = nullptr, *d_rho = nullptr;
    char* zero_begin = nullptr;
    size_t zero_bytes = 0;
    LmState* d_states = nullptr;
    int *d_scored = nullptr, *d_flags = nullptr;
    RansacBest* d_best = nullptr;
    int64_t *d_bcounts = nullptr, *d_boffs = nullptr;
    uint8_t* d_mask = nullptr;
    RansacBest* h_best = nullptr;
    int* h_running = nullptr;
    double *h_tcount = nullptr, *h_terr = nullptr, *h_hyp = nullptr;
    LmState* h_states = nullptr;
    int32_t* h_samples_pinned = nullptr;
    int b0 = 0, B = 0, round = 0;
    bool need_score = true, final_done = false, spec_scored = false, tail_enqueued = false, spec_final = false;
    int not_one_step = 0, fused_base_next = 0, score_hint_next = -1;
    bool hints_ready = false;
};
int ransac_begin(Ctx* c, const double* d_q, const double* d_u, const double* d_a, const double* d_ak, int64_t n, int use_alpha_k, int T,
                 double tol, const int32_t* h_samples, uint64_t seed, int depth_mode, int k_sign_mode, rsdsfm_ransac_out* out,
                 const RansacSpecTail* spec_tail, bool* spec_tail_held, RansacRun* run, const Minimal9Direct* direct,
                 const std::function<int()>* after_minimal9, const DenseFlatten* dense = nullptr, bool tail_ahead = true, bool count_only = false,
                 int* refine_flag_words = nullptr);
int ransac_finish(Ctx* c, RansacRun* run);
void ransac_commit_hints(Ctx* c, const RansacRun& run);
int flatten_enqueue(Ctx* c, const double* d_img, int32_t rows, int32_t cols, double fx, double fy, double cx, double cy, double gamma,
                    double thr, double* d_q, double* d_u, double* d_alpha, double* d_alpha_k, int64_t* h_total);
typedef std::function<int(const RefineBuffers&)> RefineTail;
int refine_finish_grid(const Ctx* c, const RefineBuffers& B);
int depth_map_decided_launch(Ctx* c, double* d_inl, int64_t m, const double* d_zsums, int nz, const RefineBuffers& B, double* d_depth_map,
                             double* d_header, double* h_header, const double* v_dev, const int64_t* m_dev, const PoseTableOut* pt);
struct RefineRun {
    RefineBuffers B;
    int np = 6, launched = 0, chunk = 5, hint_prev = -1;
    bool rf = false;
    double* d_inl_out = nullptr;
    const RefineTail* tail = nullptr;
    RefineState* hs = nullptr;
    bool prefetch = false, prefetched = false;
    bool tail_done = false;
};
constexpr size_t kPinnedTail = 1024;
size_t refine_workspace_bytes(const Ctx* c, int64_t m, bool m_on_device);
int refine_begin(Ctx* c, const double* d_flow, int64_t n_flow, int64_t m, const double* d_inl, const double* d_alpha,
                 const double* d_alpha_k, const int64_t* d_inlier_idx, const double v_in[3], const double w_in[3], double k_in,
                 int const_acceleration, int flow_index_mode, double* d_inl_out, const RefineTail* tail, const RansacBest* d_best,
                 void* ws_base, RefineRun* run, RefineState* hs_prefetch, double* d_zpartials, bool exact = false,
                 const FinishClaim* claim = nullptr);
constexpr int kRcRefineRestartExact = 1;
int refine_device(Ctx* c, const double* d_flow, int64_t n_flow, int64_t m, const double* d_inl, const double* d_alpha,
                  const double* d_alpha_k, const int64_t* d_inlier_idx, const double v_in[3], const double w_in[3], double k_in,
                  int const_acceleration, int flow_index_mode, double* d_inl_out, double v_out[3], double w_out[3], double* k_out,
                  rsdsfm_lm_summary* summary, const RefineTail* tail, double* d_zpartials, bool exact = false, const FinishClaim* claim = nullptr);
int refine_enqueue_chunk(Ctx* c, RefineRun* run);
int frames_in_flight(const Ctx* c);
int refine_poll(Ctx* c, RefineRun* run, double v_out[3], double w_out[3], double* k_out, rsdsfm_lm_summary* summary);
int refine_partials_doubles(const Ctx* c, int64_t m);
int refine_partials_doubles_cap(const Ctx* c);
int refine_state_from_best_launch(Ctx* c, const RansacBest* d_best, const RefineBuffers& B, int np);
int* refine_flag_words(void* ws_base);
inline int refine_trace_reset(Ctx* c) {
    if (!c->d_refine_trace) return RSDSFM_OK;
    return hipMemsetAsync(c->d_refine_trace, 0xFF, (size_t)c->refine_trace_rows * kRefineTraceCols * sizeof(double), c->stream) == hipSuccess ? RSDSFM_OK : RSDSFM_ERR_HIP;
}
int refine_init_launch(Ctx* c, const RefineBuffers& B, int np);
int refine_rf_pass_launch(Ctx* c, const RefineBuffers& B, int np, int g, int g_first, const double* rows_all_prev, int nranks, int64_t m_total,
                          const int64_t* m_total_dev, bool publish = false);
int refine_rf_apply_launch(Ctx* c, const RefineBuffers& B, int np, int g, bool to_published, const double* rows_all, int nranks, int64_t m_total,
                           const int64_t* m_total_dev);
int refine_rf_row_launch(Ctx* c, const RefineBuffers& B, int np, int g, double* row);
int refine_rf_row_doubles(int np);
void refine_rf_debug_dump(Ctx* c, const RefineBuffers& B);
int refine_rf_read_stamps(Ctx* c, unsigned long long out[16]);
int refine_rf_extra_doubles();
int refine_partials_half_doubles(const Ctx* c);
int refine_state_doubles();
inline int* refine_rf_counters(const RefineBuffers& B) { return B.bad_index + 4; }
int refine_iter_launch(Ctx* c, const RefineBuffers& B, int np, int j, int chunk);
int refine_finish_launch(Ctx* c, const RefineBuffers& B, double* inl_out);
int refine_stage_row_doubles(int np, int stage);
int refine_slot_row_doubles(int np);
int refine_slot_partials_doubles(const Ctx* c, int64_t m);
int refine_slot_rows_launch(Ctx* c, const RefineBuffers& B, int np, double* row, int j, const double* rows_all_prev, int nranks);
int refine_slot_apply_launch(Ctx* c, const RefineBuffers& B, int np, const double* rows_all, int nranks, int chunk);
int refine_stage_rows_launch(Ctx* c, const RefineBuffers& B, int np, int stage, double* row);
int refine_stage_apply_launch(Ctx* c, const RefineBuffers& B, int np, int stage, const double* rows_all, int nranks, int64_t m_total,
                              const int64_t* m_total_dev = nullptr);
}

namespace rsdsfm {
int back_project_launch(Ctx* c, const unsigned char* d_img, const double* d_depth_cm, const double* d_R, const double* d_t, double fx,
                        double fy, double cx, double cy, int rows, int cols, int mode, int q5_mode, unsigned char* d_gs, float* d_c3d);
int interpolate_cracky_launch(Ctx* c, const unsigned char* d_in, int rows, int cols, int offset, unsigned char* d_out);
int rectify_frame_launch(Ctx* c, const double* d_inl, int64_t m, const unsigned char* d_img, const double* d_depth_cm, const double* d_R,
                         const double* d_t, double fx, double fy, double cx, double cy, int rows, int cols, int mode, int q5_mode, int offset,
                         unsigned char* d_preview, unsigned char* d_gs, float* d_c3d, unsigned char* d_fixed, double* d_partials);
int depth_preview_launch(Ctx* c, const double* d_inl, int64_t m, double fx, double fy, double cx, double cy, int rows, int cols,
                         unsigned char* d_out, double* d_partials);
}

struct rsdsfm_ctx {
// ... 3 lines not shown
```

Before: 1752.

## Skip RANSAC final rho/mask and compaction when winner keeps every point

When the winning RANSAC hypothesis counts every point as an inlier, the final rho/mask and compaction kernels exit early. The first refinement pass then recomputes rho for each point from the dense inputs, writes the identity index and alpha arrays, and flags any point that fails the tolerance. If the speculative refinement misses or restarts, the compaction runs late as a fallback. This removes a full pass over the points and the compaction traffic, at the cost of more complex pass kernels and a rerun path.

```diff
diff --git a/include/rsdsfm.h b/include/rsdsfm.h
--- a/include/rsdsfm.h
+++ b/include/rsdsfm.h
@@ -187,6 +187,8 @@
 int rsdsfm_set_sequence_lanes(rsdsfm_ctx* ctx, int32_t lanes);
 int rsdsfm_set_frame_side_flatten(rsdsfm_ctx* ctx, int mode);
 int rsdsfm_set_frame_tail(rsdsfm_ctx* ctx, int mode);
+int rsdsfm_set_frame_dense_winner(rsdsfm_ctx* ctx, int on);
+int rsdsfm_frame_dense_winner_runs(rsdsfm_ctx* ctx, int64_t* runs);
 int rsdsfm_ransac_dev(rsdsfm_ctx* ctx, const double* d_q2n, const double* d_u2n, const double* d_alpha_n,
                       const double* d_alpha_k_n, int64_t n, int use_alpha_k, int32_t iterations, double tolerance,
                       const int32_t* samples_9xT_or_null, uint64_t seed, int depth_mode, int k_sign_mode,
diff --git a/rs-aware-differential-sfm_amd/__init__.py b/rs-aware-differential-sfm_amd/__init__.py
--- a/rs-aware-differential-sfm_amd/__init__.py
+++ b/rs-aware-differential-sfm_amd/__init__.py
@@ -518,6 +518,14 @@
     def set_frame_tail(self, mode):
         self._check(self.lib.rsdsfm_set_frame_tail(self._ctx, int(mode)), "rsdsfm_set_frame_tail")
 
+    def set_frame_dense_winner(self, on):
+        self._check(self.lib.rsdsfm_set_frame_dense_winner(self._ctx, int(on)), "rsdsfm_set_frame_dense_winner")
+
+    def frame_dense_winner_runs(self):
+        n = C.c_int64(0)
+        self._check(self.lib.rsdsfm_frame_dense_winner_runs(self._ctx, C.byref(n)), "rsdsfm_frame_dense_winner_runs")
+        return int(n.value)
+
     def prepared_frames_solve(self, jobs, trials=50, tol=0.05, use_acceleration_mode=False, use_refinement=True, depth_mode=DEPTH_CERES_LM,
                               k_sign_mode=K_COMPAT, flow_threshold=1e-10, flow_index_mode=FLOW_COMPAT_RANK, use_global_shutter_mode=False):
         n = len(jobs)
diff --git a/rs-aware-differential-sfm_amd/build.py b/rs-aware-differential-sfm_amd/build.py
--- a/rs-aware-differential-sfm_amd/build.py
+++ b/rs-aware-differential-sfm_amd/build.py
@@ -9,7 +9,7 @@
 OBJ_DIR = os.path.join(HERE, "build")
 CFLAGS = ["--offload-arch=gfx950", "-O3", "-std=c++17", "-ffp-contract=off", "-fPIC", "-Wall", "-Wno-unused-function"]
 LDFLAGS = ["--offload-arch=gfx950", "-shared", "-fPIC", "-ldl"]
-FUSED_UNITS = ("depth_kernels", "ransac_kernels", "ransac_lma_kernels", "depth_lma_kernels", "gtflow_kernels", "capi")
+FUSED_UNITS = ("depth_kernels", "ransac_kernels", "ransac_lma_kernels", "depth_lma_kernels", "gtflow_kernels", "capi", "refine_rf_kernels")
 
 
 def sources():
diff --git a/rs-aware-differential-sfm_amd/csrc/frame_host.hip b/rs-aware-differential-sfm_amd/csrc/frame_host.hip
--- a/rs-aware-differential-sfm_amd/csrc/frame_host.hip
+++ b/rs-aware-differential-sfm_amd/csrc/frame_host.hip
@@ -34,6 +34,7 @@
     Minimal9Direct direct;
     DenseFlatten dense;
     bool refinement_enqueued = false, ahead = false, side_flatten = false, dense_in_launch = false, open = false;
+    bool dense_winner = false;
     bool counted = false;
     int rc_begin = RSDSFM_OK;
     int64_t m_known = -1;
@@ -214,10 +215,20 @@
         F->claim.rows = rows, F->claim.cols = cols;
         F->claim.ys = F->d_ys;
     }
+    F->dense_winner = c->frame_dense_winner != 0 && prm->use_refinement && c->frame_tail == 0 && c->lm_arithmetic == 0 && c->refine_arithmetic == 0;
     F->spec_tail = [c, F](const RansacBest* d_best) -> int {
+        RefineDense dn;
+        const RansacRun& R = F->ransac;
+        if (R.final_dense) {
+            dn.on = true;
+            dn.q = F->d_q, dn.alpha = F->d_a, dn.alpha_k = F->d_ak;
+            dn.states = R.d_states, dn.best = R.d_best, dn.best_host = R.h_best;
+            dn.n = F->n, dn.depth_mode = F->prm.depth_mode, dn.tol = F->prm.ransac_tol;
+            dn.idx_out = F->d_idx, dn.alpha_out = F->d_in_a, dn.alpha_k_out = F->d_in_ak;
+        }
         return refine_begin(c, F->d_u, F->n, F->n, F->d_inl, F->d_in_a, F->d_in_ak, F->d_idx, nullptr, nullptr, 0.0, F->prm.use_acceleration_mode,
                             F->prm.flow_index_mode, F->d_inl_ref, &F->tail, d_best, F->d_refine_ws, &F->refine, state_host(c), F->d_zpartials, false,
-                            &F->claim);
+                            &F->claim, &dn);
     };
     F->refinement_enqueued = false;
     F->ahead = prm->use_refinement && c->ransac_spec_miss < 2;
@@ -228,7 +239,7 @@
                                prm->depth_mode, prm->k_sign_mode, &F->ro, prm->use_refinement ? &F->spec_tail : nullptr, &F->refinement_enqueued, &F->ransac,
                                F->side_flatten ? &F->direct : nullptr, F->side_flatten && !F->dense_in_launch ? &F->join : nullptr,
                                F->dense_in_launch ? &F->dense : nullptr, F->ahead, true,
-                               F->claim.on && prm->use_refinement ? refine_flag_words(F->d_refine_ws) : nullptr);
+                               F->claim.on && prm->use_refinement ? refine_flag_words(F->d_refine_ws) : nullptr, F->dense_winner);
     return RSDSFM_OK;
 }
 
@@ -264,7 +275,7 @@
         rc = ransac_begin(c, F->d_q, F->d_u, F->d_a, F->d_ak, n, prm->use_acceleration_mode, prm->ransac_trials, prm->ransac_tol, nullptr, J.seed,
                           prm->depth_mode, prm->k_sign_mode, &F->ro, prm->use_refinement ? &F->spec_tail : nullptr, &F->refinement_enqueued, &F->ransac, nullptr, nullptr,
                           nullptr, F->ahead, true,
-                               F->claim.on && prm->use_refinement ? refine_flag_words(F->d_refine_ws) : nullptr);
+                               F->claim.on && prm->use_refinement ? refine_flag_words(F->d_refine_ws) : nullptr, F->dense_winner);
         if (rc == RSDSFM_OK) rc = ransac_finish(c, &F->ransac);
         counted = rc == RSDSFM_OK;
     }
@@ -283,11 +294,16 @@
     double* d_final = F->d_inl;
     int flipped = 0;
     F->m_known = ro.num_inliers;
+    if (F->ransac.final_dense && ransac_winner_is_dense(F->ransac.h_best, n)) c->frame_dense_runs += 1;
     if (prm->use_refinement) {
         bool exact = false;
         if (F->refinement_enqueued) {
             rc = refine_poll(c, &F->refine, v, w, &k, &res->refine_summary);
             exact = rc == kRcRefineRestartExact;
+        }
+        if (!F->refinement_enqueued || exact) {
+            rc = ransac_compact_if_skipped(c, &F->ransac);
+            if (rc != RSDSFM_OK) return rc;
         }
         if (!F->refinement_enqueued || exact)
             rc = refine_device(c, F->d_u, n, ro.num_inliers, F->d_inl, F->d_in_a, F->d_in_ak, F->d_idx, v, w, k, prm->use_acceleration_mode,
@@ -389,6 +405,21 @@
     return RSDSFM_OK;
 }
 
+int rsdsfm_set_frame_dense_winner(rsdsfm_ctx* ctx, int on) {
+    if (!ctx) return RSDSFM_ERR_INVALID;
+    if (on < 0 || on > 1) return fail(&ctx->c, RSDSFM_ERR_INVALID, "on must be 0 (always the dense rho / mask and the compaction) or 1 (skip them for a winner that keeps every point)");
+    ctx->c.frame_dense_winner = on;
+    return RSDSFM_OK;
+}
+
+int rsdsfm_frame_dense_winner_runs(rsdsfm_ctx* ctx, int64_t* runs) {
+    if (!ctx || !runs) return RSDSFM_ERR_INVALID;
+    int64_t total = ctx->c.frame_dense_runs;
+    for (rsdsfm_ctx* lane : ctx->c.lanes) total += lane->c.frame_dense_runs;
+    *runs = total;
+    return RSDSFM_OK;
+}
+
 int rsdsfm_set_frame_side_flatten(rsdsfm_ctx* ctx, int mode) {
     if (!ctx) return RSDSFM_ERR_INVALID;
     if (mode < 0 || mode > 3) return fail(&ctx->c, RSDSFM_ERR_INVALID, "mode must be 0 (flatten first), 1 (flatten on a second stream), 2 (flatten behind the minimal solver) or 3 (flatten inside the solver's launch)");
@@ -424,6 +455,7 @@
         lc->lma_count_only_force = c->lma_count_only_force;
         lc->frame_side_flatten = c->frame_side_flatten;
         lc->frame_tail = c->frame_tail;
+        lc->frame_dense_winner = c->frame_dense_winner;
         lc->refine_stage_mode = c->refine_stage_mode;
     }
     for (int l = 0; l < L; ++l) lane_ctx(l)->refine_stage_separate = L > 1;
diff --git a/rs-aware-differential-sfm_amd/csrc/lm_common.hpp b/rs-aware-differential-sfm_amd/csrc/lm_common.hpp
--- a/rs-aware-differential-sfm_amd/csrc/lm_common.hpp
+++ b/rs-aware-differential-sfm_amd/csrc/lm_common.hpp
@@ -137,6 +137,15 @@
     double inv_hist[kMaxIter];
     double inv_cand[KMAX];
     __device__ __forceinline__ double inv_hist_at(int h) const { return inv_hist[h]; }
+    __device__ __forceinline__ void set_replay(int n) { n_hist = n, K = 0, write_which = 0; }
+};
+struct LmPlanReplayLds {
+    static constexpr int K = 0, write_which = 0;
+    int n_hist;
+    double inv_hist[kMaxIter];
+    double inv_cand[KMAX];
+    __device__ __forceinline__ double inv_hist_at(int h) const { return inv_hist[h]; }
+    __device__ __forceinline__ void set_replay(int n) { n_hist = n; }
 };
 
 struct LmPlanReg {
@@ -252,6 +261,20 @@
     return lm_pixel_t<false>(x, y, ux, uy, al, ak, pose, two_over, plan, acc, hook, model_out);
 }
 
+template <class Plan>
+__device__ __forceinline__ double hyp_rho(double x, double y, double ux, double uy, double al, double ak, const Pose& pose,
+                                          double two_over, int depth_mode, const Plan& plan) {
+    if (depth_mode == RSDSFM_DEPTH_CLOSED_FORM) return closed_form_rho(x, y, ux, uy, al, ak, pose, two_over);
+    double dummy[NS];
+    return lm_pixel(x, y, ux, uy, al, ak, pose, two_over, plan, dummy);
+}
+
+template <class Plan>
+__device__ __forceinline__ void lm_plan_replay_setup(Plan& plan, const LmState& st, int tid) {
+    if (tid == 0) plan.set_replay(st.n_hist);
+    if (tid < kMaxIter) plan.inv_hist[tid] = 1.0 / st.hist[tid];
+}
+
 __device__ __forceinline__ bool is_max_slot(int s) { return s == 2 || (s >= 3 && ((s - 3) % 5) == 4); }
 
 
diff --git a/rs-aware-differential-sfm_amd/csrc/ransac_host.hip b/rs-aware-differential-sfm_amd/csrc/ransac_host.hip
--- a/rs-aware-differential-sfm_amd/csrc/ransac_host.hip
+++ b/rs-aware-differential-sfm_amd/csrc/ransac_host.hip
@@ -181,8 +181,10 @@
                                             nullptr, 0, 0, nullptr, R.tie_margin, lazy);
                     if (rc != RSDSFM_OK) return rc;
                     flags_via_pick = true;
+                    R.final_dense = R.dense_winner && R.spec_tail && R.tail_ahead;
                     rc = ransac_final_launch(c, R.d_q, R.d_u, R.d_a, R.d_ak, n, R.d_best, R.d_states, depth_mode, tol, R.d_rho, R.d_mask, R.d_bcounts,
-                                             R.d_boffs, out->inlier_idx, out->inliers, out->alpha, out->alpha_k, R.h_best, R.refine_flag_words);
+                                             R.d_boffs, out->inlier_idx, out->inliers, out->alpha, out->alpha_k, R.h_best, R.refine_flag_words,
+                                             R.final_dense ? 1 : 0);
                     if (rc != RSDSFM_OK) return rc;
                     R.final_done = true;
                     R.spec_final = true;
@@ -268,8 +270,10 @@
                     rc = ransac_pick_launch(c, R.d_tcount, R.d_terr, T, R.d_hyp, R.d_best, R.h_best, nullptr, nullptr, 0, nullptr, 0, 0, nullptr, R.tie_margin,
                                             R.count_only ? PickLazy{R.d_scored, R.d_unscored, R.d_flags + 1} : PickLazy());
                     if (rc != RSDSFM_OK) return rc;
+                    R.final_dense = R.dense_winner && R.spec_tail;
                     rc = ransac_final_launch(c, R.d_q, R.d_u, R.d_a, R.d_ak, n, R.d_best, R.d_states, depth_mode, tol, R.d_rho, R.d_mask, R.d_bcounts,
-                                             R.d_boffs, out->inlier_idx, out->inliers, out->alpha, out->alpha_k, R.h_best, R.refine_flag_words);
+                                             R.d_boffs, out->inlier_idx, out->inliers, out->alpha, out->alpha_k, R.h_best, R.refine_flag_words,
+                                             R.final_dense ? 1 : 0);
                     if (rc != RSDSFM_OK) return rc;
                 }
                 if (R.spec_tail && !R.tail_enqueued) {
@@ -371,10 +375,12 @@
 int ransac_begin(Ctx* c, const double* d_q, const double* d_u, const double* d_a, const double* d_ak, int64_t n, int use_alpha_k, int T,
                  double tol, const int32_t* h_samples, uint64_t seed, int depth_mode, int k_sign_mode, rsdsfm_ransac_out* out,
                  const RansacSpecTail* spec_tail, bool* spec_tail_held, RansacRun* run, const Minimal9Direct* direct,
-                 const std::function<int()>* after_minimal9, const DenseFlatten* dense, bool tail_ahead, bool count_only, int* refine_flag_words) {
+                 const std::function<int()>* after_minimal9, const DenseFlatten* dense, bool tail_ahead, bool count_only, int* refine_flag_words,
+                 bool dense_winner) {
     RansacRun& R = *run;
     R = RansacRun();
     R.tail_ahead = tail_ahead;
+    R.dense_winner = dense_winner && spec_tail != nullptr;
     R.core_math = c->ransac_math_mode == 0 && c->ransac_standard_math == 0;
     R.analytic = depth_mode == RSDSFM_DEPTH_CERES_LM && T > 0 && c->lm_arithmetic == 0 && c->lma_hold == 0;
     R.tie_margin = depth_mode != RSDSFM_DEPTH_CERES_LM || c->lm_arithmetic != 0 ? 0.0 : (R.analytic ? kLmaTie : -kLmaTie);
@@ -451,6 +457,15 @@
 }
 
 int ransac_finish(Ctx* c, RansacRun* run) { return ransac_advance(c, *run, false); }
+
+int ransac_compact_if_skipped(Ctx* c, RansacRun* run) {
+    RansacRun& R = *run;
+    if (R.pc != kPcDone || !R.final_dense || !ransac_winner_is_dense(R.h_best, R.n)) return RSDSFM_OK;
+    R.final_dense = false;
+    const rsdsfm_ransac_out* out = R.out;
+    return ransac_final_launch(c, R.d_q, R.d_u, R.d_a, R.d_ak, R.n, R.d_best, R.d_states, R.depth_mode, R.tol, R.d_rho, R.d_mask, R.d_bcounts, R.d_boffs,
+                               out->inlier_idx, out->inliers, out->alpha, out->alpha_k, R.h_best, nullptr, 0);
+}
 
 int ransac_device(Ctx* c, const double* d_q, const double* d_u, const double* d_a, const double* d_ak, int64_t n,
                   int use_alpha_k, int T, double tol, const int32_t* h_samples, uint64_t seed, int depth_mode,
diff --git a/rs-aware-differential-sfm_amd/csrc/ransac_kernels.hip b/rs-aware-differential-sfm_amd/csrc/ransac_kernels.hip
--- a/rs-aware-differential-sfm_amd/csrc/ransac_kernels.hip
+++ b/rs-aware-differential-sfm_amd/csrc/ransac_kernels.hip
@@ -363,13 +363,6 @@
         if (s_fused_score && tid < nblocks)
             cnt_rt[(int64_t)tid * cnt_stride + t] = partials[((int64_t)tid * (rank_stride2 ? rank_stride2 : T * (NSR / 2)) + (int64_t)t * (NSR / 2)) * 2 + NS];
     }
-}
-
-__device__ __forceinline__ double hyp_rho(double x, double y, double ux, double uy, double al, double ak, const Pose& pose,
-                                          double two_over, int depth_mode, const LmPlanLds& plan) {
-    if (depth_mode == RSDSFM_DEPTH_CLOSED_FORM) return closed_form_rho(x, y, ux, uy, al, ak, pose, two_over);
-    double dummy[NS];
-    return lm_pixel(x, y, ux, uy, al, ak, pose, two_over, plan, dummy);
 }
 
 __device__ __forceinline__ double score_error(const PixelModel& m, double x, double y, double ux, double uy, double al, double ak,
@@ -705,24 +698,18 @@
                                                           const RansacBest* __restrict__ best,
                                                           const LmState* __restrict__ states, int depth_mode, double tol,
                                                           double* __restrict__ rho_out, uint8_t* __restrict__ mask_out,
-                                                          int64_t* __restrict__ block_counts) {
+                                                          int64_t* __restrict__ block_counts, int dense_skip) {
     __shared__ LmPlanLds plan;
     __shared__ int s_cnt[kRB / 64];
     const int tid = threadIdx.x, lane = tid & 63, wv = tid >> 6;
     if (best->undecided) return;
+    if (dense_skip && ransac_winner_is_dense(best, n)) return;
     const int bt = best->best_trial;
     Pose pose;
     pose.w[0] = best->hyp[0], pose.w[1] = best->hyp[1], pose.w[2] = best->hyp[2];
     pose.v[0] = best->hyp[3], pose.v[1] = best->hyp[4], pose.v[2] = best->hyp[5];
     pose.k = best->hyp[6];
-    if (depth_mode == RSDSFM_DEPTH_CERES_LM && bt >= 0) {
-        if (tid == 0) {
-            plan.n_hist = states[bt].n_hist;
-            plan.K = 0;
-            plan.write_which = 0;
-        }
-        if (tid < kMaxIter) plan.inv_hist[tid] = 1.0 / states[bt].hist[tid];
-    }
+    if (depth_mode == RSDSFM_DEPTH_CERES_LM && bt >= 0) lm_plan_replay_setup(plan, states[bt], tid);
     __syncthreads();
     const double two_over = 2.0 / (2.0 + pose.k);
     const int64_t i0 = (int64_t)blockIdx.x * chunk;
@@ -790,10 +777,11 @@
                                                             const int64_t* __restrict__ block_counts, RansacBest* best,
                                                             RansacBest* best_host, int64_t* __restrict__ inlier_idx, double* __restrict__ inliers,
                                                             double* __restrict__ out_alpha, double* __restrict__ out_alpha_k,
-                                                            int* __restrict__ zero_words = nullptr) {
+                                                            int* __restrict__ zero_words = nullptr, int dense_skip = 0) {
     __shared__ int s_wave[kRB / 64];
     __shared__ int64_t s_base;
     if (zero_words && blockIdx.x == 0 && threadIdx.x < (int)(kRefineStateBlockTail / sizeof(int))) zero_words[threadIdx.x] = 0;
+    if (dense_skip && ransac_winner_is_dense(best, n)) return;
     __shared__ int64_t s_pre[kRB / 64], s_all[kRB / 64];
     const int tid = threadIdx.x, lane = tid & 63, wv = tid >> 6;
     const int undecided = best->undecided;
@@ -1019,7 +1007,8 @@
 int ransac_final_launch(Ctx* c, const double* q, const double* u, const double* a, const double* ak, int64_t n,
                         RansacBest* best, const LmState* states, int depth_mode, double tol, double* rho, uint8_t* mask,
                         int64_t* block_counts, int64_t* block_offsets, int64_t* inlier_idx, double* inliers,
-                        double* out_alpha, double* out_alpha_k, RansacBest* best_host, int* zero_words) {
+                        double* out_alpha, double* out_alpha_k, RansacBest* best_host, int* zero_words, int dense_skip) {
+    if (dense_skip && !(inlier_idx || inliers || out_alpha || out_alpha_k)) dense_skip = 0;
     int64_t blocks = (n + kRB - 1) / kRB;
     if (blocks < 1) blocks = 1;
     const int64_t cap = 2048;
@@ -1030,11 +1019,11 @@
     }
     hipLaunchKernelGGL(ransac_final_kernel, dim3((int)blocks), dim3(kRB), 0, c->stream, reinterpret_cast<const double2*>(q),
                        reinterpret_cast<const double2*>(u), a, ak, n, chunk, best, states, depth_mode, tol, rho, mask,
-                       block_counts);
+                       block_counts, dense_skip);
     RSDSFM_HIP_CHECK(c, hipGetLastError());
     if (inlier_idx || inliers || out_alpha || out_alpha_k) {
         hipLaunchKernelGGL(ransac_scatter_kernel, dim3((int)blocks), dim3(kRB), 0, c->stream, reinterpret_cast<const double2*>(q),
-                           a, ak, n, chunk, rho, mask, block_counts, best, best_host, inlier_idx, inliers, out_alpha, out_alpha_k, zero_words);
+                           a, ak, n, chunk, rho, mask, block_counts, best, best_host, inlier_idx, inliers, out_alpha, out_alpha_k, zero_words, dense_skip);
     } else {
         if (zero_words) RSDSFM_HIP_CHECK(c, hipMemsetAsync(zero_words, 0, kRefineStateBlockTail, c->stream));
         hipLaunchKernelGGL(ransac_scan_kernel, dim3(1), dim3(256), 0, c->stream, block_counts, (int)blocks, block_offsets, best, best_host);
diff --git a/rs-aware-differential-sfm_amd/csrc/refine_host.hip b/rs-aware-differential-sfm_amd/csrc/refine_host.hip
--- a/rs-aware-differential-sfm_amd/csrc/refine_host.hip
+++ b/rs-aware-differential-sfm_amd/csrc/refine_host.hip
@@ -9,7 +9,8 @@
 int refine_begin(Ctx* c, const double* d_flow, int64_t n_flow, int64_t m, const double* d_inl, const double* d_alpha,
                  const double* d_alpha_k, const int64_t* d_inlier_idx, const double v_in[3], const double w_in[3], double k_in,
                  int const_acceleration, int flow_index_mode, double* d_inl_out, const RefineTail* tail, const RansacBest* d_best,
-                 void* ws_base, RefineRun* run, RefineState* hs_prefetch, double* d_zpartials, bool exact, const FinishClaim* claim) {
+                 void* ws_base, RefineRun* run, RefineState* hs_prefetch, double* d_zpartials, bool exact, const FinishClaim* claim,
+                 const RefineDense* dense) {
     if (m < 0 || n_flow < 0 || (!d_best && (!v_in || !w_in))) return fail(c, RSDSFM_ERR_INVALID, "bad arguments");
     if (flow_index_mode != RSDSFM_FLOW_COMPAT_RANK && flow_index_mode != RSDSFM_FLOW_GATHERED) return fail(c, RSDSFM_ERR_INVALID, "unknown flow_index_mode");
     if (flow_index_mode == RSDSFM_FLOW_GATHERED && m > 0 && !d_inlier_idx) return fail(c, RSDSFM_ERR_INVALID, "gathered mode needs inlier_idx");
@@ -52,6 +53,12 @@
     run->np = np;
     run->rf = !exact && c->lm_arithmetic == 0 && c->refine_arithmetic == 0;
     if (run->rf) c->refine_rf_runs += 1;
+    if (dense && dense->on) {
+        if (!run->rf || !d_best || !B.claim.on || !dense->q || !dense->alpha || !dense->alpha_k || !dense->best || !dense->best_host || !dense->idx_out ||
+            !dense->alpha_out || !dense->alpha_k_out || dense->n != m || n_flow < m)
+            return fail(c, RSDSFM_ERR_INVALID, "dense-winner path: not the radius-factorised refinement of a frame solve's short tail");
+        B.dense = *dense;
+    }
     run->d_inl_out = d_inl_out;
     run->tail = tail;
     run->launched = 0;
diff --git a/rs-aware-differential-sfm_amd/csrc/refine_kernels.hip b/rs-aware-differential-sfm_amd/csrc/refine_kernels.hip
--- a/rs-aware-differential-sfm_amd/csrc/refine_kernels.hip
+++ b/rs-aware-differential-sfm_amd/csrc/refine_kernels.hip
@@ -462,8 +462,13 @@
                                                                  double* __restrict__ inl_out, double* __restrict__ zpartials,
                                                                  RefineState* __restrict__ state_host, const int* __restrict__ bad_index,
                                                                  double fx, double fy, double cx, double cy, int rows, int ncols,
-                                                                 unsigned* __restrict__ owner, unsigned tag, int32_t* __restrict__ ys) {
+                                                                 unsigned* __restrict__ owner, unsigned tag, int32_t* __restrict__ ys,
+                                                                 const RansacBest* __restrict__ dense_best, int64_t dense_n,
+                                                                 const double* __restrict__ dense_q) {
     __shared__ double s_red[kFB / 64];
+    const bool dense = dense_best && ransac_winner_is_dense(dense_best, dense_n);
+    const double* __restrict__ xy = dense ? dense_q : inl;
+    const int xy_stride = dense ? 2 : 3;
     if (state_host && blockIdx.x == 0) {
         for (int i = threadIdx.x; i < (int)(sizeof(RefineState) / 8); i += kFB)
             reinterpret_cast<double*>(state_host)[i] = reinterpret_cast<const double*>(st)[i];
@@ -474,7 +479,7 @@
     const int64_t stride = (int64_t)gridDim.x * kFB;
     double acc = 0.0;
     for (int64_t i = (int64_t)blockIdx.x * kFB + threadIdx.x; i < m; i += stride) {
-        const double xn = inl[3 * i], yn = inl[3 * i + 1];
+        const double xn = xy[xy_stride * i], yn = xy[xy_stride * i + 1];
         inl_out[3 * i] = xn;
         inl_out[3 * i + 1] = yn;
         const double z = 1.0 / rho[i];
@@ -496,7 +501,7 @@
 }
 
 __global__ void refine_state_from_best_kernel(const RansacBest* __restrict__ best, RefineState* __restrict__ st, int np, int cap,
-                                              int* __restrict__ bad_index) {
+                                              int* __restrict__ bad_index, int dense_skip, int64_t dense_n) {
     if (threadIdx.x != 0 || blockIdx.x != 0) return;
     RefineState z;
     memset(&z, 0, sizeof(z));
@@ -509,7 +514,7 @@
     z.termination = -1;
     z.radius = kInitialRadius;
     z.need_schur = 1;
-    const int64_t m = best->undecided ? 0 : best->num_inliers_scan;
+    const int64_t m = best->undecided ? 0 : ((dense_skip && ransac_winner_is_dense(best, dense_n)) ? dense_n : best->num_inliers_scan);
     z.m = m;
     int64_t b = (m + kFB - 1) / kFB;
     if (b < 1) b = 1;
@@ -519,7 +524,7 @@
     }
     z.grid = (int)b;
     *st = z;
-    bad_index[0] = 0;
+    bad_index[0] = bad_index[1] = 0;
     bad_index[4] = bad_index[5] = bad_index[6] = 0;
 }
 
@@ -548,7 +553,8 @@
 static inline const RefineState* slot_state_in(const Ctx* c, const RefineBuffers& B, int j) { return j == 0 ? B.state : chunk_state(c, B, j - 1); }
 
 int refine_state_from_best_launch(Ctx* c, const RansacBest* d_best, const RefineBuffers& B, int np) {
-    hipLaunchKernelGGL(refine_state_from_best_kernel, dim3(1), dim3(64), 0, c->stream, d_best, B.state, np, refine_grid_cap(c), B.bad_index);
+    hipLaunchKernelGGL(refine_state_from_best_kernel, dim3(1), dim3(64), 0, c->stream, d_best, B.state, np, refine_grid_cap(c), B.bad_index,
+                       B.dense.on ? 1 : 0, B.dense.n);
     RSDSFM_HIP_CHECK(c, hipGetLastError());
     return RSDSFM_OK;
 }
@@ -898,7 +904,8 @@
     if (B.claim.on) {
         hipLaunchKernelGGL(refine_finish_claim_kernel, dim3(refine_finish_grid(c, B)), dim3(kFB), 0, c->stream, B.m_on_device ? (int64_t)-1 : B.m, B.inl,
                            B.rho_a, B.rho_b, B.state, inl_out, B.zpartials, B.state_host, B.bad_index, B.claim.fx, B.claim.fy, B.claim.cx, B.claim.cy,
-                           B.claim.rows, B.claim.cols, B.claim.owner, B.claim.tag, B.claim.ys);
+                           B.claim.rows, B.claim.cols, B.claim.owner, B.claim.tag, B.claim.ys,
+                           static_cast<const RansacBest*>(B.dense.on ? B.dense.best : nullptr), B.dense.n, B.dense.q);
         RSDSFM_HIP_CHECK(c, hipGetLastError());
         return RSDSFM_OK;
     }
diff --git a/rs-aware-differential-sfm_amd/csrc/refine_rf_kernels.hip b/rs-aware-differential-sfm_amd/csrc/refine_rf_kernels.hip
--- a/rs-aware-differential-sfm_amd/csrc/refine_rf_kernels.hip
+++ b/rs-aware-differential-sfm_amd/csrc/refine_rf_kernels.hip
@@ -1,3 +1,4 @@
+#include "lm_common.hpp"
 #include "refine_common.hpp"
 
 #ifndef RF_LOADS_ONLY
@@ -35,7 +36,8 @@
 
 enum RfGuard : int {
     kRfGuardNonFinite = 1, kRfGuardGradient = 2, kRfGuardModel = 3, kRfGuardParameter = 4, kRfGuardFunction = 5, kRfGuardQuality = 6,
-    kRfGuardPivot = 7, kRfGuardList = 8, kRfGuardRadius = 9
+    kRfGuardPivot = 7, kRfGuardList = 8, kRfGuardRadius = 9,
+    kRfGuardDenseCount = 10
 };
 constexpr double kBandGradient = 1e-4, kBandParameter = 1e-2, kBandFunction = 1e-4, kBandQuality = 1e-4, kBandModel = 1e-12, kBandPivot = 1e-9;
 
@@ -619,6 +621,10 @@
     int grid_cap;
     unsigned long long* stamps;
 };
+struct RfDenseArgs {
+    RefineDense dn;
+    int* miss;
+};
 
 struct RfLoad {
     double4 c4;
@@ -640,10 +646,9 @@
     return l;
 }
 
-}
-
-template <int NP, bool FIRST, bool ZSUM>
-__global__ __launch_bounds__(kFB) void refine_rf_pass_kernel(const RfPassArgs A) {
+template <int NP, bool FIRST, bool ZSUM, bool DENSE, bool PUBLISH>
+__device__ __forceinline__ void rf_pass_body(const RfPassArgs A, const RfDenseArgs* D) {
+    static_assert((FIRST || !DENSE) && !(FIRST && PUBLISH), "the dense source is the first pass's, the count is published by the pass behind it");
     using RR = RfRow<NP>;
     __shared__ RfStageLds<NP> s_stage;
     __shared__ double s_red[kFB / 64][RR::NW];
@@ -660,6 +665,12 @@
         for (int i = 0; i < 8; ++i) tk[i] = 0;
     }
     if (stamp) tk[0] = wall_clock64();
+    __shared__ LmPlanReplayLds s_plan;
+    bool dense = false;
+    if constexpr (DENSE) {
+        dense = ransac_winner_is_dense(D->dn.best, D->dn.n);
+        if (dense && D->dn.depth_mode == RSDSFM_DEPTH_CERES_LM) lm_plan_replay_setup(s_plan, D->dn.states[D->dn.best->best_trial], (int)threadIdx.x);
+    }
     if (FIRST && A.best) {
         if (threadIdx.x < sizeof(RefineState) / 8) reinterpret_cast<unsigned long long*>(&s_state)[threadIdx.x] = 0ull;
         __syncthreads();
@@ -674,7 +685,7 @@
             z.termination = -1;
             z.radius = kInitialRadius;
             z.need_schur = 1;
-            const int64_t mb = A.best->undecided ? 0 : A.best->num_inliers_scan;
+            const int64_t mb = A.best->undecided ? 0 : (dense ? D->dn.n : A.best->num_inliers_scan);
             z.m = mb;
             int64_t b = (mb + kFB - 1) / kFB;
             if (b < 1) b = 1;
@@ -687,6 +698,18 @@
         __syncthreads();
     } else {
         state_to_lds(&s_state, A.st_in);
+        if constexpr (PUBLISH) if (ransac_winner_is_dense(D->dn.best, D->dn.n)) {
+            const int miss = *D->miss;
+            if (blockIdx.x == 0 && threadIdx.x == 0) {
+                const int64_t scan = miss ? (int64_t)-1 : D->dn.n;
+                D->dn.best->num_inliers_scan = scan;
+                D->dn.best_host->num_inliers_scan = scan;
+            }
+            if (miss) {
+                if (threadIdx.x == 0 && s_state.termination < 0) s_state.termination = kTermRestartExact, s_state.rf_guard = kRfGuardDenseCount;
+                __syncthreads();
+            }
+        }
     }
     RefineState* st = &s_state;
     if (stamp) tk[1] = wall_clock64();
@@ -733,16 +756,7 @@
     if (FIRST) {
         RfPoint Pq = rf_point(st->p);
         const RfPoint P = rf_point_uniform(Pq);
-        for (int64_t i = i0; i < m; i += stride) {
-            int64_t fi = (A.flow_index_mode == RSDSFM_FLOW_GATHERED) ? A.inlier_idx[i] : i;
-            if (fi < 0 || fi >= A.n_flow) {
-                *A.bad_index = 1;
-                fi = 0;
-            }
-            const double2 f = A.flow[fi];
-            const double x = A.inl[3 * i], y = A.inl[3 * i + 1];
-            const double rho = 1.0 / A.inl[3 * i + 2];
-            const double al = A.alpha[i], ak = A.alpha_k[i];
+        auto first_body = [&](int64_t i, double x, double y, const double2 f, double rho, double al, double ak) {
             A.xyuv_out[i] = make_double4(x, y, f.x, f.y);
             const double ab = NP == 6 ? P.c1 * __builtin_fma(P.k, ak, al) : al;
             if (NP == 6) A.beta[i] = ab;
@@ -761,6 +775,45 @@
             const double ihm = flagged ? 0.0 : rcp_core(flagged ? 1.0 : o.h);
             rf_schur_accumulate<NP>(o, ihm, acc);
             if (flagged) rf_list_append(A.list_count, A.list_entries, x, y, f.x, f.y, ab, ak, rho, i);
+        };
+        if constexpr (DENSE) if (dense) {
+            Pose pose;
+            pose.w[0] = D->dn.best->hyp[0], pose.w[1] = D->dn.best->hyp[1], pose.w[2] = D->dn.best->hyp[2];
+            pose.v[0] = D->dn.best->hyp[3], pose.v[1] = D->dn.best->hyp[4], pose.v[2] = D->dn.best->hyp[5];
+            pose.k = D->dn.best->hyp[6];
+            const double two_over = 2.0 / (2.0 + pose.k);
+            const double2* __restrict__ q2 = reinterpret_cast<const double2*>(D->dn.q);
+            for (int64_t i = i0; i < m; i += stride) {
+                int64_t fi = i;
+                if (fi < 0 || fi >= A.n_flow) {
+                    *A.bad_index = 1;
+                    fi = 0;
+                }
+                const double2 f = A.flow[fi];
+                const double2 qq = q2[i];
+                const double al = D->dn.alpha[i], ak = D->dn.alpha_k[i];
+                const double rho_r = hyp_rho(qq.x, qq.y, f.x, f.y, al, ak, pose, two_over, D->dn.depth_mode, s_plan);
+                const bool in = point_error(qq.x, qq.y, f.x, f.y, al, ak, pose, two_over, rho_r) < D->dn.tol;
+                if (!in) *D->miss = 1;
+                const double z = 1.0 / rho_r;
+                const double rho = 1.0 / z;
+                D->dn.idx_out[i] = i;
+                if (NP == 7) D->dn.alpha_out[i] = al, D->dn.alpha_k_out[i] = ak;
+                first_body(i, qq.x, qq.y, f, rho, al, ak);
+            }
+        }
+        if (!DENSE || !dense) {
+            for (int64_t i = i0; i < m; i += stride) {
+                int64_t fi = (A.flow_index_mode == RSDSFM_FLOW_GATHERED) ? A.inlier_idx[i] : i;
+                if (fi < 0 || fi >= A.n_flow) {
+                    *A.bad_index = 1;
+                    fi = 0;
+                }
+                const double2 f = A.flow[fi];
+                const double x = A.inl[3 * i], y = A.inl[3 * i + 1];
+                const double rho = 1.0 / A.inl[3 * i + 2];
+                first_body(i, x, y, f, rho, A.alpha[i], A.alpha_k[i]);
+            }
         }
     } else {
         RfPoint Pq = rf_point(st->p), Pcq = rf_point(st->pc);
@@ -880,6 +933,21 @@
     }
 }
 
+}
+
+template <int NP, bool FIRST, bool ZSUM>
+__global__ __launch_bounds__(kFB) void refine_rf_pass_kernel(const RfPassArgs A) {
+    rf_pass_body<NP, FIRST, ZSUM, false, false>(A, nullptr);
+}
+template <int NP, bool ZSUM>
+__global__ __launch_bounds__(kFB) void refine_rf_pass_dense_kernel(const RfPassArgs A, const RfDenseArgs D) {
+    rf_pass_body<NP, true, ZSUM, true, false>(A, &D);
+}
+template <int NP, bool ZSUM>
+__global__ __launch_bounds__(kFB) void refine_rf_pass_publish_kernel(const RfPassArgs A, const RfDenseArgs D) {
+    rf_pass_body<NP, false, ZSUM, false, true>(A, &D);
+}
+
 template <int NP>
 __global__ __launch_bounds__(kFB) void refine_rf_apply_kernel(const double* __restrict__ rows, int nrows, int row_stride, RfLists lists,
                                                              const RefineState* __restrict__ st_in, RefineState* __restrict__ st_out,
@@ -1015,8 +1083,12 @@
     return buf;
 }
 template <int NP, bool ZSUM>
-void rf_pass_launch_t(Ctx* c, const RfPassArgs& A, bool first, int grid) {
-    if (first)
+void rf_pass_launch_t(Ctx* c, const RfPassArgs& A, bool first, int grid, const RfDenseArgs* D, int g) {
+    if (D && first)
+        hipLaunchKernelGGL((refine_rf_pass_dense_kernel<NP, ZSUM>), dim3(grid), dim3(kFB), 0, c->stream, A, *D);
+    else if (D && g == 1)
+        hipLaunchKernelGGL((refine_rf_pass_publish_kernel<NP, ZSUM>), dim3(grid), dim3(kFB), 0, c->stream, A, *D);
+    else if (first)
         hipLaunchKernelGGL((refine_rf_pass_kernel<NP, true, ZSUM>), dim3(grid), dim3(kFB), 0, c->stream, A);
     else
         hipLaunchKernelGGL((refine_rf_pass_kernel<NP, false, ZSUM>), dim3(grid), dim3(kFB), 0, c->stream, A);
@@ -1066,10 +1138,13 @@
     A.beat = rf_beat(c);
     A.slot = g;
     const bool first = g == 0;
+    RfDenseArgs Dn;
+    Dn.dn = B.dense, Dn.miss = B.bad_index + 1;
+    const RfDenseArgs* D = B.dense.on && B.m_on_device && g <= 1 ? &Dn : nullptr;
     if (np == 7) {
-        if (B.want_zsum) rf_pass_launch_t<7, true>(c, A, first, grid); else rf_pass_launch_t<7, false>(c, A, first, grid);
+        if (B.want_zsum) rf_pass_launch_t<7, true>(c, A, first, grid, D, g); else rf_pass_launch_t<7, false>(c, A, first, grid, D, g);
     } else {
-        if (B.want_zsum) rf_pass_launch_t<6, true>(c, A, first, grid); else rf_pass_launch_t<6, false>(c, A, first, grid);
+        if (B.want_zsum) rf_pass_launch_t<6, true>(c, A, first, grid, D, g); else rf_pass_launch_t<6, false>(c, A, first, grid, D, g);
     }
     RSDSFM_HIP_CHECK(c, hipGetLastError());
     return RSDSFM_OK;
diff --git a/rs-aware-differential-sfm_amd/csrc/rsdsfm_internal.hpp b/rs-aware-differential-sfm_amd/csrc/rsdsfm_internal.hpp
--- a/rs-aware-differential-sfm_amd/csrc/rsdsfm_internal.hpp
+++ b/rs-aware-differential-sfm_amd/csrc/rsdsfm_internal.hpp
@@ -73,6 +73,9 @@
     int32_t _pad_shared;
     int32_t lazy_pending;
 };
+__host__ __device__ __forceinline__ bool ransac_winner_is_dense(const RansacBest* best, int64_t n) {
+    return !best->undecided && best->best_trial >= 0 && best->num_inliers == n;
+}
 struct PickLazy {
     int* scored = nullptr;
     int* list = nullptr;
@@ -155,6 +158,8 @@
     hipEvent_t ev_fork = nullptr, ev_join = nullptr, ev_seq = nullptr;
     int frame_side_flatten = 3;
     int frame_tail = 0;
+    int frame_dense_winner = 1;
+    int64_t frame_dense_runs = 0;
     unsigned long long* d_flat_counters = nullptr;
     int seq_lanes = 0;
     int refine_stage_mode = 0;
@@ -343,7 +348,7 @@
 int ransac_final_launch(Ctx* c, const double* q, const double* u, const double* a, const double* ak, int64_t n,
                         RansacBest* best, const LmState* states, int depth_mode, double tol, double* rho, uint8_t* mask,
                         int64_t* block_counts, int64_t* block_offsets, int64_t* inlier_idx, double* inliers,
-                        double* out_alpha, double* out_alpha_k, RansacBest* best_host = nullptr, int* zero_words = nullptr);
+                        double* out_alpha, double* out_alpha_k, RansacBest* best_host = nullptr, int* zero_words = nullptr, int dense_skip = 0);
 int ransac_rows_doubles();
 int ransac_lm_rows_launch(Ctx* c, const double* q, const double* u, const double* a, const double* ak, int64_t n,
                           const double* hyp, int T, const LmState* states, double* partials, int round, double tol, double* rows,
@@ -399,6 +404,21 @@
     unsigned* owner = nullptr;
     unsigned tag = 0, mask = 0;
 };
+struct RefineDense {
+    bool on = false;
+    const double* q = nullptr;
+    const double* alpha = nullptr;
+    const double* alpha_k = nullptr;
+    const LmState* states = nullptr;
+    RansacBest* best = nullptr;
+    RansacBest* best_host = nullptr;
+    int64_t n = 0;
+    int depth_mode = 0;
+    double tol = 0.0;
+    int64_t* idx_out = nullptr;
+    double* alpha_out = nullptr;
+    double* alpha_k_out = nullptr;
+};
 struct RefineBuffers {
     const double* flow;
     int64_t n_flow, m;
@@ -420,6 +440,7 @@
     double* zpartials = nullptr;
     const RansacBest* best_dev = nullptr;
     FinishClaim claim;
+    RefineDense dense;
     bool want_zsum = false;
 };
 size_t ransac_pinned_bytes(int T);
@@ -448,6 +469,7 @@
     int lma_cand[2] = {2, 1}, lma_cand_next[2] = {0, 0};
     int *d_irr_count = nullptr, *d_irr_list = nullptr;
     bool restarted = false;
+    bool dense_winner = false, final_dense = false;
     bool tail_ahead = true;
     const Minimal9Direct* direct = nullptr;
     const DenseFlatten* dense = nullptr;
@@ -475,8 +497,9 @@
                  double tol, const int32_t* h_samples, uint64_t seed, int depth_mode, int k_sign_mode, rsdsfm_ransac_out* out,
                  const RansacSpecTail* spec_tail, bool* spec_tail_held, RansacRun* run, const Minimal9Direct* direct,
                  const std::function<int()>* after_minimal9, const DenseFlatten* dense = nullptr, bool tail_ahead = true, bool count_only = false,
-                 int* refine_flag_words = nullptr);
+                 int* refine_flag_words = nullptr, bool dense_winner = false);
 int ransac_finish(Ctx* c, RansacRun* run);
+int ransac_compact_if_skipped(Ctx* c, RansacRun* run);
 void ransac_commit_hints(Ctx* c, const RansacRun& run);
 int flatten_enqueue(Ctx* c, const double* d_img, int32_t rows, int32_t cols, double fx, double fy, double cx, double cy, double gamma,
                     double thr, double* d_q, double* d_u, double* d_alpha, double* d_alpha_k, int64_t* h_total);
@@ -500,7 +523,7 @@
                  const double* d_alpha_k, const int64_t* d_inlier_idx, const double v_in[3], const double w_in[3], double k_in,
                  int const_acceleration, int flow_index_mode, double* d_inl_out, const RefineTail* tail, const RansacBest* d_best,
                  void* ws_base, RefineRun* run, RefineState* hs_prefetch, double* d_zpartials, bool exact = false,
-                 const FinishClaim* claim = nullptr);
+                 const FinishClaim* claim = nullptr, const RefineDense* dense = nullptr);
 constexpr int kRcRefineRestartExact = 1;
 int refine_device(Ctx* c, const double* d_flow, int64_t n_flow, int64_t m, const double* d_inl, const double* d_alpha,
                   const double* d_alpha_k, const int64_t* d_inlier_idx, const double v_in[3], const double w_in[3], double k_in,
```

New measurement: 1802 (median of 6 runs). 2.9% higher.
